# Luolin0826/band

Measured on AMD Instinct MI355X. Metric: multi-DNN inferences/sec + p99 job latency, 4-model int8 mix @1/2/4/8 GPU, higher is better.
Workload: dtype int8

## Files before the change

### band_amd/_abi.py

```python
import ctypes
import os

_HERE = os.path.dirname(os.path.abspath(__file__))
LIB_PATH = os.path.join(_HERE, "libband_hip%s.so" % (
    "_" + os.environ["BAND_HIP_LIB_VARIANT"] if os.environ.get("BAND_HIP_LIB_VARIANT") else ""))

c_int, c_int32, c_void_p, c_size_t = ctypes.c_int, ctypes.c_int32, ctypes.c_void_p, ctypes.c_size_t


class ConvParams(ctypes.Structure):
    _fields_ = [(n, c_int) for n in (
        "batch", "in_h", "in_w", "in_c", "out_h", "out_w", "out_c", "k_h", "k_w",
        "stride_h", "stride_w", "dil_h", "dil_w", "pad_h", "pad_w", "k_pad", "n_pad", "in_xor")] + [
        (n, c_int32) for n in ("in_zp", "w_zp", "out_zp", "act_min", "act_max")] + [
        (n, c_void_p) for n in ("input", "output", "weights", "bias_eff", "mult", "shift", "residual")] + [
        (n, c_int32) for n in ("add_y_off", "add_r_off", "add_o_off", "add_left_shift", "add_y_mult",
                               "add_y_shift", "add_r_mult", "add_r_shift", "add_o_mult", "add_o_shift",
                               "add_act_min", "add_act_max")] + [("out_table", c_void_p), ("requant_fast", c_int32),
                                                                  ("kernel_hint", c_int32),
                                                                  ("out_img_stride", ctypes.c_int64)]


class ConvGroupedParams(ctypes.Structure):
    _fields_ = [("conv", ConvParams), ("groups", c_int32)]


class ConvGroup(ctypes.Structure):
    _fields_ = [("n", c_int), ("blocks", c_int), ("is1x1", c_int), ("table", c_void_p)]


class DwConvParams(ctypes.Structure):
    _fields_ = [(n, c_int) for n in (
        "batch", "in_h", "in_w", "in_c", "out_h", "out_w", "out_c", "depth_multiplier",
        "k_h", "k_w", "stride_h", "stride_w", "dil_h", "dil_w", "pad_h", "pad_w", "in_xor")] + [
        (n, c_int32) for n in ("in_zp", "w_zp", "out_zp", "act_min", "act_max")] + [
        (n, c_void_p) for n in ("input", "output", "weights", "bias", "mult", "shift", "out_table", "taps")] + [
        ("requant_fast", c_int32), ("kernel_hint", c_int32)]


class FcParams(ctypes.Structure):
    _fields_ = [(n, c_int) for n in ("rows", "depth", "depth_pad", "units", "in_xor")] + [
        (n, c_int32) for n in ("in_zp", "w_zp", "out_zp", "act_min", "act_max")] + [
        (n, c_void_p) for n in ("input", "output", "weights", "bias_eff", "mult", "shift", "out_table")]


class EltwiseParams(ctypes.Structure):
    _fields_ = [("kind", c_int), ("in_signed", c_int), ("shape_a", c_int * 4),
                ("shape_b", c_int * 4), ("shape_o", c_int * 4)] + [
        (n, c_int32) for n in ("a_off", "b_off", "o_off", "left_shift", "a_mult", "a_shift",
                               "b_mult", "b_shift", "o_mult", "o_shift", "act_min", "act_max")] + [
        (n, c_void_p) for n in ("a", "b", "out")]


class PoolParams(ctypes.Structure):
    _fields_ = [(n, c_int) for n in (
        "kind", "in_signed", "batch", "in_h", "in_w", "channels", "out_h", "out_w",
        "f_h", "f_w", "stride_h", "stride_w", "pad_h", "pad_w")] + [
        (n, c_int32) for n in ("act_min", "act_max")] + [
        (n, c_void_p) for n in ("input", "output")]


class IrbParams(ctypes.Structure):
    _fields_ = [(n, c_int) for n in (
        "batch", "in_h", "in_w", "in_c", "exp_c", "out_h", "out_w", "out_c", "stride", "pad_h", "pad_w",
        "has_expand", "tile_h", "tile_w")] + [
        ("exp_w", c_void_p), ("exp_k_pad", c_int), ("exp_bias_eff", c_void_p), ("exp_mult", c_void_p),
        ("exp_shift", c_void_p)] + [(n, c_int32) for n in ("x_zp", "e_zp", "e_act_min", "e_act_max")] + [
        ("dw_w", c_void_p), ("dw_bias", c_void_p), ("dw_mult", c_void_p), ("dw_shift", c_void_p)] + [
        (n, c_int32) for n in ("d_zp", "d_act_min", "d_act_max")] + [
        ("proj_w", c_void_p), ("proj_k_pad", c_int), ("proj_bias_eff", c_void_p), ("proj_mult", c_void_p),
        ("proj_shift", c_void_p)] + [(n, c_int32) for n in ("p_zp", "p_act_min", "p_act_max")] + [
        ("has_residual", c_int)] + [(n, c_int32) for n in (
            "add_p_off", "add_x_off", "add_o_off", "add_left_shift", "add_p_mult", "add_p_shift", "add_x_mult",
            "add_x_shift", "add_o_mult", "add_o_shift", "add_act_min", "add_act_max")] + [
        ("input", c_void_p), ("output", c_void_p), ("debug_stamps", c_void_p), ("requant_fast", c_int32)]


class MeanParams(ctypes.Structure):
    _fields_ = [(n, ctypes.c_long) for n in ("outer", "reduce", "inner")] + [("type", c_int)] + [
        (n, c_int32) for n in ("multiplier", "shift", "bias")] + [("input", c_void_p), ("output", c_void_p)]


class MeanRowsParams(ctypes.Structure):
    _fields_ = [("rows", ctypes.c_long), ("depth", c_int), ("type", c_int), ("exact", c_int),
                ("scale", ctypes.c_float), ("bias", ctypes.c_float), ("out_zp", c_int32),
                ("input", c_void_p), ("output", c_void_p)]


class LayerNormParams(ctypes.Structure):
    _fields_ = [("rows", ctypes.c_long), ("depth", c_int), ("mean_x", MeanRowsParams), ("mean_d", MeanRowsParams)] + [
        (n, EltwiseParams) for n in ("sqdiff", "add_eps", "mul_gamma", "mul_x", "mul_m", "sub_beta", "add_out")] + [
        ("eps_q", c_int32)] + [(n, c_void_p) for n in ("rsqrt_table", "input", "gamma", "beta", "output")]


class DetectionParams(ctypes.Structure):
    _fields_ = [(n, c_int) for n in ("batch", "num_boxes", "num_classes", "num_classes_with_background",
                                     "max_detections")] + [
        (n, ctypes.c_float) for n in ("score_threshold", "iou_threshold", "scale_y", "scale_x", "scale_h",
                                      "scale_w")] + [
        ("box_type", c_int), ("score_type", c_int), ("box_scale", ctypes.c_float), ("score_scale", ctypes.c_float),
        ("box_zp", c_int32), ("score_zp", c_int32)] + [
        (n, c_void_p) for n in ("box_encodings", "class_scores", "anchors", "out_boxes", "out_classes",
                                "out_scores", "out_num", "scratch")]


class ChainParams(ctypes.Structure):
    _fields_ = [("dw", DwConvParams), ("pw1", ConvParams), ("pw2", ConvParams), ("has_pw2", c_int),
                ("px_blocks", c_int), ("waves", c_int), ("persist", c_int), ("tile", c_int),
                ("tile_blob", c_void_p), ("debug_stamps", c_void_p), ("deep", c_int), ("c_split", c_int),
                ("stage", c_int), ("dense", c_int)]


CONCAT_MAX_INPUTS = 16


class ConcatParams(ctypes.Structure):
    _fields_ = [("n_inputs", c_int), ("outer", ctypes.c_long),
                ("row", ctypes.c_long * CONCAT_MAX_INPUTS), ("input", c_void_p * CONCAT_MAX_INPUTS),
                ("table", c_void_p * CONCAT_MAX_INPUTS), ("output", c_void_p)]

# ... 55 lines not shown
class SoftmaxParams(ctypes.Structure):
    _fields_ = [("rows", ctypes.c_long), ("depth", c_int), ("is_signed", c_int), ("table", c_void_p),
                ("out_scale", ctypes.c_float), ("out_zp", c_int32), ("input", c_void_p), ("output", c_void_p)]


class ZeroInsertParams(ctypes.Structure):
    _fields_ = [(n, c_int) for n in ("batch", "in_h", "in_w", "channels", "stride_h", "stride_w", "out_h",
                                     "out_w")] + [("fill", ctypes.c_uint32), ("input", c_void_p), ("output", c_void_p)]


class ConvF32Params(ctypes.Structure):
    _fields_ = [(n, c_int) for n in (
        "batch", "in_h", "in_w", "in_c", "out_h", "out_w", "out_c", "k_h", "k_w", "stride_h", "stride_w",
        "dil_h", "dil_w", "pad_h", "pad_w", "depthwise", "depth_multiplier")] + [
        ("act_min", ctypes.c_float), ("act_max", ctypes.c_float)] + [
        (n, c_void_p) for n in ("input", "output", "weights", "bias")]


class FcF32Params(ctypes.Structure):
    _fields_ = [(n, c_int) for n in ("rows", "depth", "units")] + [
        ("act_min", ctypes.c_float), ("act_max", ctypes.c_float)] + [
        (n, c_void_p) for n in ("input", "output", "weights", "bias")]


class EltwiseF32Params(ctypes.Structure):
    _fields_ = [("kind", c_int), ("shape_a", c_int * 4), ("shape_b", c_int * 4), ("shape_o", c_int * 4),
                ("act_min", ctypes.c_float), ("act_max", ctypes.c_float)] + [(n, c_void_p) for n in ("a", "b", "out")]


class PoolF32Params(ctypes.Structure):
    _fields_ = [(n, c_int) for n in (
        "kind", "batch", "in_h", "in_w", "channels", "out_h", "out_w", "f_h", "f_w", "stride_h", "stride_w",
        "pad_h", "pad_w")] + [("act_min", ctypes.c_float), ("act_max", ctypes.c_float)] + [
        (n, c_void_p) for n in ("input", "output")]


KERNEL_SYMBOLS = {
    "bh_device_count": (c_int, [ctypes.POINTER(c_int)]),
    "bh_set_device": (c_int, [c_int]),
    "bh_get_device": (c_int, [ctypes.POINTER(c_int)]),
    "bh_device_arch": (c_int, [c_int, ctypes.c_char_p, c_size_t]),
    "bh_device_pci_bus_id": (c_int, [c_int, ctypes.c_char_p, c_int]),
    "bh_stream_create": (c_int, [ctypes.POINTER(c_void_p)]),
    "bh_stream_destroy": (c_int, [c_void_p]),
    "bh_stream_sync": (c_int, [c_void_p]),
    "bh_stream_query": (c_int, [c_void_p]),
    "bh_malloc": (c_int, [ctypes.POINTER(c_void_p), c_size_t]),
    "bh_free": (c_int, [c_void_p]),
    "bh_host_alloc": (c_int, [ctypes.POINTER(c_void_p), c_size_t]),
    "bh_host_free": (c_int, [c_void_p]),
    "bh_memcpy_h2d_async": (c_int, [c_void_p, c_void_p, c_size_t, c_void_p]),
    "bh_memcpy_d2h_async": (c_int, [c_void_p, c_void_p, c_size_t, c_void_p]),
    "bh_memcpy_d2d_async": (c_int, [c_void_p, c_void_p, c_size_t, c_void_p]),
    "bh_copy_d2d": (c_int, [c_void_p, c_void_p, c_size_t, c_void_p]),
    "bh_memset_async": (c_int, [c_void_p, c_int, c_size_t, c_void_p]),
    "bh_memcpy_h2d": (c_int, [c_void_p, c_void_p, c_size_t]),
    "bh_memcpy_d2h": (c_int, [c_void_p, c_void_p, c_size_t]),
    "bh_capture_begin": (c_int, [c_void_p]),
    "bh_capture_end": (c_int, [c_void_p, ctypes.POINTER(c_void_p)]),
    "bh_graph_launch": (c_int, [c_void_p, c_void_p]),
    "bh_graph_destroy": (c_int, [c_void_p]),
    "bh_event_create": (c_int, [ctypes.POINTER(c_void_p)]),
    "bh_event_create_blocking": (c_int, [ctypes.POINTER(c_void_p)]),
    "bh_capture_end_keep": (c_int, [c_void_p, ctypes.POINTER(c_void_p), ctypes.POINTER(c_void_p)]),
    "bh_graph_free": (c_int, [c_void_p]),
    "bh_graph_memcpy_nodes": (c_int, [c_void_p, ctypes.POINTER(c_void_p), ctypes.POINTER(c_void_p),
                                      ctypes.POINTER(c_void_p), ctypes.POINTER(c_size_t), c_int,
                                      ctypes.POINTER(c_int)]),
    "bh_graph_exec_set_memcpy": (c_int, [c_void_p, c_void_p, c_void_p, c_void_p, c_size_t, c_int]),
    "bh_event_destroy": (c_int, [c_void_p]),
    "bh_event_record": (c_int, [c_void_p, c_void_p]),
    "bh_event_sync": (c_int, [c_void_p]),
    "bh_event_query": (c_int, [c_void_p]),
    "bh_event_create_untimed": (c_int, [ctypes.POINTER(c_void_p)]),
    "bh_event_elapsed_ms": (c_int, [c_void_p, c_void_p, ctypes.POINTER(ctypes.c_float)]),
    "bh_spin_us": (c_int, [c_void_p, c_int]),
    "bh_empty_launch": (c_int, [c_void_p]),
    "bh_profile_events": (c_int, [c_void_p, c_void_p]),
    "bh_pack_conv_weights": (c_int, [c_void_p, c_int, c_int, c_int, c_int, c_int, c_void_p,
                                     c_int32, c_int32, c_void_p, c_void_p]),
    "bh_conv_packed_geometry": (c_int, [c_int, c_int, ctypes.POINTER(c_int), ctypes.POINTER(c_int)]),
    "bh_pack_dw_taps": (c_int, [c_void_p, c_int, c_void_p, c_int32, c_int32, c_void_p]),
    "bh_conv_requant_fast_ok": (c_int, [c_void_p, c_void_p, c_int, c_int, ctypes.c_int64]),
    "bh_conv2d_i8": (c_int, [ctypes.POINTER(ConvParams), c_void_p]),
    "bh_conv_group_ok": (c_int, [ctypes.POINTER(ConvParams)]),
    "bh_conv_group_table_bytes": (ctypes.c_size_t, [c_int]),
    "bh_conv_group_plan": (c_int, [ctypes.POINTER(ConvParams), c_int, c_void_p, ctypes.POINTER(ConvGroup)]),
    "bh_conv_group_i8": (c_int, [ctypes.POINTER(ConvGroup), c_void_p]),
    "bh_conv2d_i8_kernel": (ctypes.c_char_p, [ctypes.POINTER(ConvParams)]),
    "bh_conv2d_grouped_i8": (c_int, [ctypes.POINTER(ConvGroupedParams), c_void_p]),
    "bh_conv2d_grouped_i8_kernel": (ctypes.c_char_p, [ctypes.POINTER(ConvGroupedParams)]),
    "bh_conv_gemm_big_config": (ctypes.c_int, [ctypes.c_long, ctypes.c_int]),
    "bh_dwconv2d_i8_kernel": (ctypes.c_char_p, [ctypes.POINTER(DwConvParams)]),
    "bh_lut_u8": (c_int, [c_void_p, c_void_p, ctypes.c_long, c_void_p, c_void_p]),
    "bh_lut_f32": (c_int, [c_void_p, c_void_p, ctypes.c_long, c_void_p, c_void_p]),
    "bh_quantize_f32": (c_int, [c_void_p, c_void_p, ctypes.c_long, ctypes.c_float, c_int32, c_int, c_void_p]),
    "bh_concat": (c_int, [ctypes.POINTER(ConcatParams), c_void_p]),
    "bh_pad": (c_int, [ctypes.POINTER(PadParams), c_void_p]),
    "bh_resize_nearest": (c_int, [ctypes.POINTER(ResizeNearestParams), c_void_p]),
    "bh_resize_bilinear_i8": (c_int, [ctypes.POINTER(ResizeBilinearParams), c_void_p]),
    "bh_resize_bilinear_u8": (c_int, [ctypes.POINTER(ResizeBilinearU8Params), c_void_p]),
    "bh_argminmax": (c_int, [ctypes.POINTER(ArgMinMaxParams), c_void_p]),
    "bh_argminmax_kernel": (ctypes.c_char_p, [ctypes.POINTER(ArgMinMaxParams)]),
    "bh_resize_bilinear_argminmax_i8": (c_int, [ctypes.POINTER(ResizeArgMinMaxParams), c_void_p]),
    "bh_resize_bilinear_argminmax_i8_ok": (c_int, [ctypes.POINTER(ResizeArgMinMaxParams)]),
    "bh_reindex": (c_int, [ctypes.POINTER(ReindexParams), c_void_p]),
    "bh_reindex_as": (c_int, [ctypes.POINTER(ReindexParams), c_int, c_void_p]),
    "bh_reindex_kernel": (ctypes.c_char_p, [ctypes.POINTER(ReindexParams)]),
    "bh_reindex_canonical": (c_int, [ctypes.POINTER(ReindexParams), ctypes.POINTER(ReindexParams)]),
    "bh_batch_matmul_i8": (c_int, [ctypes.POINTER(BatchMatMulParams), c_void_p]),
    "bh_batch_matmul_i8_kernel": (ctypes.c_char_p, [ctypes.POINTER(BatchMatMulParams)]),
    "bh_batch_matmul_f32": (c_int, [ctypes.POINTER(BatchMatMulParams), c_void_p]),
    "bh_batch_matmul_check": (c_int, [ctypes.POINTER(BatchMatMulParams), c_int]),
    "bh_softmax_i8": (c_int, [ctypes.POINTER(SoftmaxParams), c_void_p]),
    "bh_zero_insert": (c_int, [ctypes.POINTER(ZeroInsertParams), c_void_p]),
    "bh_conv2d_f32": (c_int, [ctypes.POINTER(ConvF32Params), c_void_p]),
    "bh_conv2d_f32_split": (c_int, [ctypes.POINTER(ConvF32Params)]),
    "bh_fc_f32": (c_int, [ctypes.POINTER(FcF32Params), c_void_p]),
    "bh_eltwise_f32": (c_int, [ctypes.POINTER(EltwiseF32Params), c_void_p]),
    "bh_pool_f32": (c_int, [ctypes.POINTER(PoolF32Params), c_void_p]),
    "bh_unary_f32": (c_int, [c_int, c_void_p, c_void_p, ctypes.c_long, ctypes.c_float, ctypes.c_float, c_void_p]),
    "bh_softmax_f32": (c_int, [c_void_p, c_void_p, ctypes.c_long, c_int, ctypes.c_float, c_void_p]),
    "bh_dwconv2d_i8": (c_int, [ctypes.POINTER(DwConvParams), c_void_p]),
    "bh_fc_i8": (c_int, [ctypes.POINTER(FcParams), c_void_p]),
    "bh_eltwise_i8": (c_int, [ctypes.POINTER(EltwiseParams), c_void_p]),
    "bh_pool_i8": (c_int, [ctypes.POINTER(PoolParams), c_void_p]),
    "bh_irb_i8": (c_int, [ctypes.POINTER(IrbParams), c_void_p]),
    "bh_irb_lds_bytes": (c_size_t, [ctypes.POINTER(IrbParams)]),
    "bh_chain_i8": (c_int, [ctypes.POINTER(ChainParams), c_void_p]),
    "bh_mean": (c_int, [ctypes.POINTER(MeanParams), c_void_p]),
    "bh_mean_rows": (c_int, [ctypes.POINTER(MeanRowsParams), c_void_p]),
    "bh_mean_rows_kernel": (ctypes.c_char_p, [ctypes.POINTER(MeanRowsParams)]),
    "bh_mean_rows_check": (c_int, [ctypes.POINTER(MeanRowsParams)]),
    "bh_layernorm_i8": (c_int, [ctypes.POINTER(LayerNormParams), c_void_p]),
    "bh_layernorm_i8_kernel": (ctypes.c_char_p, [ctypes.POINTER(LayerNormParams)]),
    "bh_layernorm_i8_check": (c_int, [ctypes.POINTER(LayerNormParams)]),
    "bh_detection_scratch_bytes": (c_size_t, [c_int, c_int]),
    "bh_detection_postprocess": (c_int, [ctypes.POINTER(DetectionParams), c_void_p]),
    "bh_chain_lds_bytes": (c_size_t, [ctypes.POINTER(ChainParams)]),
    "bh_chain_tile_lds_bytes": (c_size_t, [ctypes.POINTER(ChainParams)]),
    "bh_chain_tile_launch": (c_int, [ctypes.POINTER(ChainParams), c_void_p]),
    "bh_chain_tile_blob_bytes": (c_size_t, [ctypes.POINTER(ChainParams)]),
    "bh_chain_tile_pack": (c_int, [ctypes.POINTER(ChainParams), c_void_p, c_void_p]),
    "bh_chain_stage_lds_bytes": (c_size_t, [ctypes.POINTER(ChainParams)]),
    "bh_chain_stage_launch": (c_int, [ctypes.POINTER(ChainParams), c_void_p]),
    "bh_chain_dense_lds_bytes": (c_size_t, [ctypes.POINTER(ChainParams)]),
    "bh_chain_dense_launch": (c_int, [ctypes.POINTER(ChainParams), c_void_p]),
    "bh_last_error": (ctypes.c_char_p, []),
}

BACKEND_SYMBOLS = {}

_lib = None
_configured = set()


class BandHipError(RuntimeError):
    pass


def load():
    global _lib
    if _lib is None:
        if not os.path.exists(LIB_PATH):
            raise BandHipError(
                "libband_hip.so not built (%s); run __graft_entry__.build() / make -C band_amd/csrc" % LIB_PATH)
# ... 17 lines not shown
```

### band_amd/csrc/backend/hip/lower.cc

```cpp
#include "backend/hip/executor_internal.h"

namespace band {
namespace hip {

using namespace ex;

namespace {

struct ConvQuant {
  std::vector<int32_t> mult, shift;
  int32_t amin, amax, in_zp, w_zp;
  const int32_t* bias;
};

ConvQuant QuantOf(const TflModel& d, const ConvGeometry& g, const TflTensor& out) {
  const TflTensor& in = d.tensors[g.input];
  const TflTensor& w = d.tensors[g.filter];
  const bool i8 = in.type == DataType::kInt8;
  ConvQuant q;
  ConvMultipliers(Scale(in), w.scale, g.out_c, Scale(out), !i8, &q.mult, &q.shift);
  ActivationRangeQuantized(g.act, Scale(out), Zp(out), i8, &q.amin, &q.amax);
  q.in_zp = Dom(in);
  q.w_zp = i8 ? 0 : Dom(w);
  q.bias = g.bias >= 0 ? reinterpret_cast<const int32_t*>(d.tensors[g.bias].data) : nullptr;
// ... 14 lines not shown
  f.in_xor = c.in_xor; f.in_zp = c.in_zp; f.w_zp = c.w_zp; f.out_zp = c.out_zp;
  f.act_min = c.act_min; f.act_max = c.act_max; f.input = c.input; f.output = c.output;
  f.weights = c.weights; f.bias_eff = c.bias_eff; f.mult = c.mult; f.shift = c.shift;
  F.kernel = "fc_kernel";
  F.alg_bytes = L->alg_bytes;
  F.alg_ops = L->alg_ops;
  *L = F;
  return true;
}

template <class Params>
void SetGeometry(const ConvGeometry& g, Params* p) {
  p->batch = g.batch; p->in_h = g.in_h; p->in_w = g.in_w; p->in_c = g.in_c;
  p->out_h = g.out_h; p->out_w = g.out_w; p->out_c = g.out_c; p->k_h = g.k_h; p->k_w = g.k_w;
  p->stride_h = g.stride_h; p->stride_w = g.stride_w; p->dil_h = g.dil_h; p->dil_w = g.dil_w;
  p->pad_h = g.pad_h; p->pad_w = g.pad_w;
}
template <class Params>
void SetGeometry(const PoolGeometry& g, Params* p) {
  p->batch = g.batch; p->in_h = g.in_h; p->in_w = g.in_w; p->channels = g.channels;
  p->out_h = g.out_h; p->out_w = g.out_w; p->f_h = g.f_h; p->f_w = g.f_w;
  p->stride_h = g.stride_h; p->stride_w = g.stride_w; p->pad_h = g.pad_h; p->pad_w = g.pad_w;
}

absl::Status Refused(const TflOperator& op, const char* why) {
  return absl::InternalError(std::string("unsupported ") + TflBuiltinName(op.builtin) + ": " + why);
}

}

absl::Status HipModelExecutor::ConstBlob(const std::string& key, size_t bytes, PreparedSubgraph* sg,
                                         const std::function<absl::Status(uint8_t*)>& fill,
                                         std::shared_ptr<DeviceBlob>* out) {
  auto blob = DeviceRegistry::Get().FindConst(ordinal_, key);
  if (!blob) {
    std::vector<uint8_t> host(bytes, 0);
    RETURN_STATUS_IF(fill(host.data()));
    blob = std::make_shared<DeviceBlob>(ordinal_, bytes);
    if (!blob->ok() || !blob->Upload(0, host.data(), bytes)) return HipErr(1, ("upload constant " + key).c_str());
    DeviceRegistry::Get().PutConst(ordinal_, key, blob);
  }
  sg->consts.push_back(blob);
  *out = blob;
  return absl::OkStatus();
}

absl::Status HipModelExecutor::UploadConst(const std::string& key, const void* data, size_t bytes,
                                           PreparedSubgraph* sg, const void** dev) {
  std::shared_ptr<DeviceBlob> blob;
  RETURN_STATUS_IF(ConstBlob(key, bytes, sg, [&](uint8_t* host) {
    if (bytes) std::memcpy(host, data, bytes);
    return absl::OkStatus();
  }, &blob));
  *dev = blob->ptr();
  return absl::OkStatus();
}

absl::Status HipModelExecutor::DevicePtr(const HipModel& model, int t, PreparedSubgraph* sg, void** ptr) {
  const TflTensor& tt = model.desc().tensors[t];
  if (!tt.is_const()) {
    auto it = sg->offset.find(t);
    if (it == sg->offset.end()) return absl::InternalError("tensor without arena slot");
    *ptr = static_cast<char*>(sg->arena->ptr()) + it->second;
    return absl::OkStatus();
  }
  const void* dev = nullptr;
  RETURN_STATUS_IF(UploadConst("m" + Hex(model.serial()) + "/t" + std::to_string(t), tt.data, tt.data_size, sg, &dev));
  *ptr = const_cast<void*>(dev);
  return absl::OkStatus();
}

absl::Status HipModelExecutor::PackedConv(const HipModel& model, int oi, const ConvGeometry& g, bool flip,
                                          const void* in_ptr, void* out_ptr, const std::string& ckey,
                                          PreparedSubgraph* sg, Launch* L) {
  const TflModel& d = model.desc();
  const TflTensor& w = d.tensors[g.filter];
  const TflTensor& out = d.tensors[d.ops[oi].outputs[0]];
  const bool i8 = w.type == DataType::kInt8;
  const ConvQuant q = QuantOf(d, g, out);
  const int oc = g.out_c, kh = g.k_h, kw = g.k_w, icg = g.in_c / g.groups, K = kh * kw * icg;
  int kp = 0, np = 0;
  bh_conv_packed_geometry(oc, K, &kp, &np);
  const size_t wbytes = static_cast<size_t>(kp) * np;
  std::shared_ptr<DeviceBlob> blob;
  RETURN_STATUS_IF(ConstBlob(ckey, wbytes + 12ull * oc, sg, [&](uint8_t* host) {
    std::vector<uint8_t> flipped(flip ? static_cast<size_t>(oc) * K : 0);
    for (size_t i = 0; i < flipped.size(); ++i) {
      const size_t ci = i % icg, fx = i / icg % kw, fy = i / icg / kw % kh, co = i / K;
      flipped[i] = w.data[((co * kh + (kh - 1 - fy)) * kw + (kw - 1 - fx)) * icg + ci];
    }
    int32_t* tables = reinterpret_cast<int32_t*>(host + wbytes);
    if (bh_pack_conv_weights(flip ? flipped.data() : w.data, i8 ? 1 : 0, oc, K, kp, np, q.bias, q.in_zp, q.w_zp,
                             reinterpret_cast<int8_t*>(host), tables) != 0)
      return absl::InternalError("weight packing failed");
    std::copy(q.mult.begin(), q.mult.end(), tables + oc);
    std::copy(q.shift.begin(), q.shift.end(), tables + 2 * oc);
    return absl::OkStatus();
  }, &blob));
  const int32_t* tab = reinterpret_cast<const int32_t*>(static_cast<char*>(blob->ptr()) + wbytes);
  bh_conv_params& p = L->conv;
  p = bh_conv_params{};
  SetGeometry(g, &p);
  p.k_pad = kp; p.n_pad = np; p.in_xor = i8 ? 0 : 0x80;
  p.in_zp = q.in_zp; p.w_zp = q.w_zp; p.out_zp = Zp(out); p.act_min = q.amin; p.act_max = q.amax;
  p.input = in_ptr; p.output = out_ptr;
  p.weights = static_cast<const int8_t*>(blob->ptr());
  p.bias_eff = tab; p.mult = tab + oc; p.shift = tab + 2 * oc;
  p.requant_fast = bh_conv_requant_fast_ok(q.mult.data(), q.shift.data(), oc, K, MaxAbs(q.bias, oc));
  const double M = static_cast<double>(g.batch) * g.out_h * g.out_w;
  L->alg_ops = 2.0 * M * oc * K;
  L->alg_bytes = static_cast<double>(g.batch) * g.in_h * g.in_w * g.in_c + M * oc + static_cast<double>(oc) * K +
                 12.0 * oc;
  if (g.groups == 1) {
    L->kind = Launch::kConv;
    L->kernel = bh_conv2d_i8_kernel(&p);
    if (GemvAsFc(L)) return absl::OkStatus();
  } else {
    L->kind = Launch::kConvGrouped;
    L->conv_groups = g.groups;
    const bh_conv_grouped_params gp{p, g.groups};
    L->kernel = device_flag_ == DeviceFlag::kCPU ? "conv_grouped_host" : bh_conv2d_grouped_i8_kernel(&gp);
  }
  TryFuseResidualAdd(model, oi, sg, L);
  return absl::OkStatus();
}

absl::Status HipModelExecutor::LowerConv(const HipModel& model, int oi, void* in_ptr, void* out_ptr,
                                         const std::string& ckey, PreparedSubgraph* sg, Launch* L) {
  ConvGeometry g;
  const char* why = "";
  if (!ConvArgs(model.desc(), model.desc().ops[oi], &g, &why)) return Refused(model.desc().ops[oi], why);
  return PackedConv(model, oi, g, false, in_ptr, out_ptr, ckey, sg, L);
}

absl::Status HipModelExecutor::LowerTransposeConv(const HipModel& model, int oi, void* out_ptr,
                                                  const std::string& ckey, PreparedSubgraph* sg, Launch* L) {
  const TflModel& d = model.desc();
  ConvGeometry g;
  const char* why = "";
  if (!ConvArgs(d, d.ops[oi], &g, &why)) return Refused(d.ops[oi], why);
  const TflTensor& x = d.tensors[g.input];
  void* x_ptr = nullptr;
  RETURN_STATUS_IF(DevicePtr(model, g.input, sg, &x_ptr));
  const int uh = (g.in_h - 1) * g.stride_h + 1, uw = (g.in_w - 1) * g.stride_w + 1;
  const size_t ubytes = static_cast<size_t>(g.batch) * uh * uw * g.in_c;
  auto scratch = std::make_shared<DeviceBlob>(ordinal_, ubytes);
  if (!scratch->ok()) return absl::InternalError("HBM scratch allocation failed");
  sg->consts.push_back(scratch);
  Launch Z;
  Z.kind = Launch::kZeroInsert;
  Z.op_index = oi;
  Z.kernel = "zero_insert_kernel";
  Z.zi = bh_zero_insert_params{};
  Z.zi.batch = g.batch; Z.zi.in_h = g.in_h; Z.zi.in_w = g.in_w; Z.zi.channels = g.in_c;
  Z.zi.stride_h = g.stride_h; Z.zi.stride_w = g.stride_w; Z.zi.out_h = uh; Z.zi.out_w = uw;
  Z.zi.fill = static_cast<uint32_t>(Zp(x)) & 0xffu;
  Z.zi.input = x_ptr;
  Z.zi.output = scratch->ptr();
  Z.alg_bytes = static_cast<double>(x.num_elements()) + static_cast<double>(ubytes);
  sg->launches.push_back(Z);
  ConvGeometry u = g;
  u.in_h = uh; u.in_w = uw;
  u.stride_h = u.stride_w = 1;
  u.pad_h = g.k_h - 1 - g.pad_h; u.pad_w = g.k_w - 1 - g.pad_w;
  return PackedConv(model, oi, u, true, scratch->ptr(), out_ptr, ckey, sg, L);
}

absl::Status HipModelExecutor::LowerGlue(const HipModel& model, int oi, void* in_ptr, void* out_ptr,
                                         const std::string& ckey, PreparedSubgraph* sg, Launch* L) {
  const TflModel& d = model.desc();
  const TflOperator& op = d.ops[oi];
  auto T = [&](int i) -> const TflTensor& { return d.tensors[i]; };
  const TflTensor& in = T(op.inputs[0]);
  const TflTensor& out = T(op.outputs[0]);
  const bool i8 = in.type == DataType::kInt8;
  const double in_bytes = static_cast<double>(meta_[op.inputs[0]]->bytes);
  const double out_bytes = static_cast<double>(meta_[op.outputs[0]]->bytes);
  L->alg_bytes = in_bytes + out_bytes;
  switch (op.builtin) {
    case kTflQuantize:
    case kTflRelu:
    case kTflRelu6:
    case kTflReluN1To1:
    case kTflLogistic:
    case kTflHardSwish:
    case kTflRsqrt:
    case kTflGelu: {
      L->src = in_ptr;
      L->dst = out_ptr;
      L->count = static_cast<long>(out.num_elements());
      if (op.builtin == kTflQuantize && in.type == DataType::kFloat32) {
// ... 499 lines not shown
  L->alg_bytes = bytes;
  return absl::OkStatus();
}

absl::Status HipModelExecutor::LowerReindex(const HipModel& model, int oi, PreparedSubgraph* sg) {
  const TflModel& d = model.desc();
  const TflOperator& op = d.ops[oi];
  void* in_ptr = nullptr;
  RETURN_STATUS_IF(DevicePtr(model, op.inputs[op.builtin == kTflSplit ? 1 : 0], sg, &in_ptr));
  for (int k = 0; k < static_cast<int>(op.outputs.size()); ++k) {
    Launch L;
    L.op_index = oi;
    L.out_tensor = op.outputs[k];
    const char* why = "";
    if (!ReindexArgs(d, op, k, &L.reindex, &why))
      return absl::InternalError(std::string("unsupported ") + TflBuiltinName(op.builtin) + ": " + why);
    void* out_ptr = nullptr;
    RETURN_STATUS_IF(DevicePtr(model, op.outputs[k], sg, &out_ptr));
    L.reindex.input = in_ptr;
    L.reindex.output = out_ptr;
    bh_reindex_params c;
    if (bh_reindex_canonical(&L.reindex, &c) != 0)
      return absl::InternalError(std::string(TflBuiltinName(op.builtin)) + ": " + bh_last_error());
    const size_t bytes = meta_[op.outputs[k]]->bytes;
    L.alg_bytes = 2.0 * bytes;
    if (c.rank == 1 && c.in_stride[0] == 1 && c.in_offset == 0) {
      L.kind = Launch::kCopy;
      L.kernel = "copy";
      L.src = in_ptr;
      L.dst = out_ptr;
      L.bytes = bytes;
      if (L.src == L.dst) continue;
    } else {
      L.kind = Launch::kReindex;
      L.kernel = device_flag_ == DeviceFlag::kCPU ? "reindex_host" : bh_reindex_kernel(&L.reindex);
    }
    sg->launches.push_back(L);
  }
  return absl::OkStatus();
}

absl::Status HipModelExecutor::LowerBatchMatMul(const HipModel& model, int oi, void* lhs_ptr, void* out_ptr,
                                                PreparedSubgraph* sg, Launch* L) {
  const TflModel& d = model.desc();
  const TflOperator& op = d.ops[oi];
  const char* why = "";
  bh_batch_matmul_params& p = L->bmm;
  if (!BatchMatMulArgs(d, op, &p, &why)) return absl::InternalError(std::string("unsupported BATCH_MATMUL: ") + why);
  void* rhs_ptr = nullptr;
  RETURN_STATUS_IF(DevicePtr(model, op.inputs[1], sg, &rhs_ptr));
  p.lhs = lhs_ptr;
  p.rhs = rhs_ptr;
  p.out = out_ptr;
  const bool f32 = d.tensors[op.inputs[0]].type == DataType::kFloat32;
  if (bh_batch_matmul_check(&p, f32 ? 4 : 1) != 0) return absl::InternalError(std::string("BATCH_MATMUL: ") + bh_last_error());
  const bool cpu = device_flag_ == DeviceFlag::kCPU;
  L->kind = f32 ? Launch::kBatchMatMulF32 : Launch::kBatchMatMul;
  L->kernel = f32 ? (cpu ? "batch_matmul_f32_host" : "bmm_f32_kernel")
                  : (cpu ? "batch_matmul_host" : bh_batch_matmul_i8_kernel(&p));
  L->alg_ops = 2.0 * p.batch[0] * p.batch[1] * p.m * p.n * p.k;
  L->alg_bytes = static_cast<double>(meta_[op.inputs[0]]->bytes + meta_[op.outputs[0]]->bytes) +
                 static_cast<double>(GetDataTypeBytes(d.tensors[op.inputs[1]].type) * d.tensors[op.inputs[1]].num_elements());
  return absl::OkStatus();
}

absl::Status HipModelExecutor::LowerDepthwise(const HipModel& model, int oi, void* in_ptr, void* out_ptr,
                                              const std::string& ckey, PreparedSubgraph* sg, Launch* L) {
  const TflModel& d = model.desc();
  const TflOperator& op = d.ops[oi];
  ConvGeometry g;
  const char* why = "";
  if (!ConvArgs(d, op, &g, &why)) return Refused(op, why);
  const TflTensor& in = d.tensors[g.input];
  const TflTensor& w = d.tensors[g.filter];
  const TflTensor& out = d.tensors[op.outputs[0]];
  const bool i8 = in.type == DataType::kInt8;
  const ConvQuant q = QuantOf(d, g, out);
  const int oc = g.out_c, kh = g.k_h, kw = g.k_w;
  const size_t wbytes = static_cast<size_t>(kh) * kw * oc;
  const size_t wpad = (wbytes + 15) / 16 * 16;
  const size_t tbytes = 12ull * oc;
  const bool dot = kh == 3 && kw == 3 && g.depth_multiplier == 1 && oc % 4 == 0;
  const size_t pbytes = dot ? 16ull * oc : 0;
  std::shared_ptr<DeviceBlob> blob;
  RETURN_STATUS_IF(ConstBlob(ckey, wpad + tbytes + pbytes, sg, [&](uint8_t* host) {
    for (size_t i = 0; i < wbytes; ++i) host[i] = i8 ? w.data[i] : static_cast<uint8_t>(w.data[i] ^ 0x80);
    int32_t* tables = reinterpret_cast<int32_t*>(host + wpad);
    for (int c = 0; c < oc; ++c) tables[c] = q.bias ? q.bias[c] : 0;
    std::copy(q.mult.begin(), q.mult.end(), tables + oc);
    std::copy(q.shift.begin(), q.shift.end(), tables + 2 * oc);
    if (dot && bh_pack_dw_taps(reinterpret_cast<const int8_t*>(host), oc, tables, q.in_zp, q.w_zp, tables + 3 * oc) != 0)
      return absl::InternalError("depthwise tap packing failed");
    return absl::OkStatus();
  }, &blob));
  const int32_t* tab = reinterpret_cast<const int32_t*>(static_cast<char*>(blob->ptr()) + wpad);
  bh_dwconv_params& p = L->dw;
  p = bh_dwconv_params{};
  SetGeometry(g, &p);
  p.depth_multiplier = g.depth_multiplier;
  p.in_xor = i8 ? 0 : 0x80; p.in_zp = q.in_zp; p.w_zp = q.w_zp; p.out_zp = Zp(out);
  p.act_min = q.amin; p.act_max = q.amax; p.input = in_ptr; p.output = out_ptr;
  p.weights = static_cast<const int8_t*>(blob->ptr());
  p.bias = tab; p.mult = tab + oc; p.shift = tab + 2 * oc;
  if (dot && !blob->host()) p.taps = tab + 3 * oc;
  p.requant_fast = bh_conv_requant_fast_ok(q.mult.data(), q.shift.data(), oc, kh * kw, MaxAbs(q.bias, oc));
  L->kind = Launch::kDwConv;
  L->kernel = bh_dwconv2d_i8_kernel(&p);
  const double M = static_cast<double>(g.batch) * g.out_h * g.out_w;
  L->alg_ops = 2.0 * M * oc * kh * kw;
  L->alg_bytes = static_cast<double>(in.num_elements()) + M * oc + static_cast<double>(wbytes) + 12.0 * oc;
  return absl::OkStatus();
}

absl::Status HipModelExecutor::LowerFc(const HipModel& model, int oi, void* in_ptr, void* out_ptr,
                                       const std::string& ckey, PreparedSubgraph* sg, Launch* L) {
  const TflModel& d = model.desc();
  const TflOperator& op = d.ops[oi];
  FcGeometry g;
  const char* why = "";
  if (!FcArgs(d, op, &g, &why)) return Refused(op, why);
  const TflTensor& in = d.tensors[op.inputs[0]];
  const TflTensor& w = d.tensors[g.filter];
  const TflTensor& out = d.tensors[op.outputs[0]];
  const bool i8 = in.type == DataType::kInt8;
  const int32_t* bias = g.bias >= 0 ? reinterpret_cast<const int32_t*>(d.tensors[g.bias].data) : nullptr;
  const int units = g.units, depth = g.depth, rows = g.rows;
  const int depth_pad = (depth + 15) / 16 * 16;
  int32_t mult, shift, amin, amax;
  FullyConnectedMultiplier(Scale(in), Scale(w), Scale(out), &mult, &shift);
  ActivationRangeQuantized(g.act, Scale(out), Zp(out), i8, &amin, &amax);
  const int32_t in_zp = Dom(in), w_zp = Dom(w);
  const size_t wbytes = static_cast<size_t>(units) * depth_pad;
  std::shared_ptr<DeviceBlob> blob;
  RETURN_STATUS_IF(ConstBlob(ckey, wbytes + 12ull * units, sg, [&](uint8_t* host) {
    int8_t* packed = reinterpret_cast<int8_t*>(host);
    int32_t* tables = reinterpret_cast<int32_t*>(host + wbytes);
    for (int u = 0; u < units; ++u) {
      int64_t s = 0;
      for (int k = 0; k < depth; ++k) {
        const uint8_t raw = w.data[static_cast<size_t>(u) * depth + k];
        const int v = i8 ? static_cast<int>(static_cast<int8_t>(raw)) : static_cast<int>(raw) - 128;
        packed[static_cast<size_t>(u) * depth_pad + k] = static_cast<int8_t>(v);
        s += v;
      }
      tables[u] = static_cast<int32_t>((bias ? bias[u] : 0) - static_cast<int64_t>(in_zp) * s +
                                       static_cast<int64_t>(depth) * in_zp * w_zp);
      tables[units + u] = mult;
      tables[2 * units + u] = shift;
    }
    return absl::OkStatus();
  }, &blob));
  const int32_t* tab = reinterpret_cast<const int32_t*>(static_cast<char*>(blob->ptr()) + wbytes);
  bh_fc_params& p = L->fc;
  p = bh_fc_params{};
  p.rows = rows; p.depth = depth; p.depth_pad = depth_pad; p.units = units;
  p.in_xor = i8 ? 0 : 0x80; p.in_zp = in_zp; p.w_zp = w_zp; p.out_zp = Zp(out);
  p.act_min = amin; p.act_max = amax; p.input = in_ptr; p.output = out_ptr;
  p.weights = static_cast<const int8_t*>(blob->ptr());
  p.bias_eff = tab; p.mult = tab + units; p.shift = tab + 2 * units;
  L->kind = Launch::kFc;
  L->kernel = "fc_kernel";
  L->alg_ops = 2.0 * rows * units * depth;
  L->alg_bytes = static_cast<double>(rows) * depth + static_cast<double>(rows) * units +
                 static_cast<double>(units) * depth + 12.0 * units;
  return absl::OkStatus();
}

absl::Status HipModelExecutor::LowerEltwise(const HipModel& model, int oi, void* in_ptr, void* out_ptr,
                                            PreparedSubgraph* sg, Launch* L) {
  const TflModel& d = model.desc();
  const TflOperator& op = d.ops[oi];
  BroadcastShapes s;
  const char* why = "";
  if (!BroadcastArgs(d, op, &s, &why)) return Refused(op, why);
  const TflTensor& in = d.tensors[op.inputs[0]];
  const TflTensor& b = d.tensors[op.inputs[1]];
  const TflTensor& out = d.tensors[op.outputs[0]];
  const bool i8 = in.type == DataType::kInt8;
  void* b_ptr = nullptr;
  RETURN_STATUS_IF(DevicePtr(model, op.inputs[1], sg, &b_ptr));
  bh_eltwise_params& p = L->elt;
  p = bh_eltwise_params{};
  p.in_signed = i8 ? 1 : 0;
  std::copy_n(s.a, 4, p.shape_a); std::copy_n(s.b, 4, p.shape_b); std::copy_n(s.o, 4, p.shape_o);
  p.a_off = -Zp(in); p.b_off = -Zp(b); p.o_off = Zp(out);
  ActivationRangeQuantized(op.options.Int8(0, 0), Scale(out), Zp(out), i8, &p.act_min, &p.act_max);
  if (op.builtin == kTflSquaredDifference) {
    AddParams ap;
// ... 190 lines not shown
```

### band_amd/csrc/kernels/chain_dense.hip

```cpp
#include <algorithm>
#include <climits>

#include "chain_dw.hpp"
#include "common.hpp"

namespace bh {

struct DenseLds {
  int S1, S2, slab, off_pl, off_add;
  size_t bytes;
};

static DenseLds dense_lds(const bh_chain_params& p) {
  DenseLds L;
  L.S1 = p.pw1.k_pad + 32;
  L.S2 = (p.has_pw2 ? p.pw2.k_pad : (p.pw1.out_c + 15) / 16 * 16) + 32;
  const int dl_row = std::max(L.S1, p.has_pw2 ? (p.pw2.out_c + 15) / 16 * 16 : 0);
  L.off_pl = 16 * dl_row;
  L.slab = L.off_pl + 16 * L.S2;
  L.off_add = 4 * L.slab;
  L.bytes = (size_t)L.off_add + (p.pw1.residual ? 512 * sizeof(int) : 0);
  return L;
}

__device__ __forceinline__ void dense_copy_rows(const unsigned char* src, int stride, uint8_t* dst, int N, int rows,
                                                int lane) {
  const bool v16 = (N & 15) == 0;
  const int u = v16 ? N >> 4 : N >> 2;
  const float rcp = 1.0f / (float)u;
  for (int i = lane; i < rows * u; i += 64) {
    const int r = (int)(((float)i + 0.5f) * rcp);
    const int k = i - r * u;
    if (v16) *(v4i*)(dst + (long)r * N + k * 16) = *(const v4i*)(src + r * stride + k * 16);
    else *(uint32_t*)(dst + (long)r * N + k * 4) = *(const uint32_t*)(src + r * stride + k * 4);
  }
}

struct DenseConv {
  __amdgpu_buffer_rsrc_t w, be, mu, sh;
  int wv, cv;
  int tile_w;
};
__device__ __forceinline__ DenseConv dense_conv(const bh_conv_params& c, int r16, int g) {
  DenseConv d;
  d.w = __builtin_amdgcn_make_buffer_rsrc((void*)c.weights, (short)0, c.n_pad * c.k_pad, 0x00020000);
  d.be = __builtin_amdgcn_make_buffer_rsrc((void*)c.bias_eff, (short)0, c.out_c * 4, 0x00020000);
  d.mu = __builtin_amdgcn_make_buffer_rsrc((void*)c.mult, (short)0, c.out_c * 4, 0x00020000);
  d.sh = __builtin_amdgcn_make_buffer_rsrc((void*)c.shift, (short)0, c.out_c * 4, 0x00020000);
  d.wv = r16 * c.k_pad + g * 16;
  d.cv = r16 * 4;
  d.tile_w = 16 * c.k_pad;
  return d;
}
template <int KX>
struct DenseTile {
  v4i w[KX];
  int be, mu, sh;
};
template <int KX>
__device__ __forceinline__ void dense_filter_load(const DenseConv& c, int t, int k0, int KS, v4i (&w)[KX]) {
  typedef unsigned int v4u __attribute__((ext_vector_type(4)));
#pragma unroll
  for (int u = 0; u < KX; ++u) {
    if (k0 + u < KS) {
      const v4u v = __builtin_amdgcn_raw_buffer_load_b128(c.w, c.wv, t * c.tile_w + (k0 + u) * 64, 0);
      w[u] = (v4i){(int)v.x, (int)v.y, (int)v.z, (int)v.w};
    } else {
      w[u] = (v4i){0, 0, 0, 0};
    }
  }
}
template <int KX>
__device__ __forceinline__ void dense_tile_load(const DenseConv& c, int t, int k0, int KS, DenseTile<KX>& d) {
  dense_filter_load<KX>(c, t, k0, KS, d.w);
  d.be = (int)__builtin_amdgcn_raw_buffer_load_b32(c.be, c.cv, t * 64, 0);
  d.mu = (int)__builtin_amdgcn_raw_buffer_load_b32(c.mu, c.cv, t * 64, 0);
  d.sh = (int)__builtin_amdgcn_raw_buffer_load_b32(c.sh, c.cv, t * 64, 0);
}

template <bool FAST, bool INTERIOR>
__device__ __forceinline__ void dense_dw_groups(const bh_dwconv_params& d, const __amdgpu_buffer_rsrc_t rsrc,
                                                const int (&off)[3], const bool (&ok)[3], bool need, int src4, int r16,
                                                int g, unsigned char* dl, int S1) {
  typedef unsigned int v4u __attribute__((ext_vector_type(4)));
  const int zfill = (int)splat_byte(d.in_zp);
  const int dsel = r16 >> 2;
  const int bsh = 8 * (r16 & 3);
  const int tsel1 = g == 0 ? 0 : 1, tbit1 = g == 0 ? 24 : 8 * (g - 1);
  const int tbit2 = g < 2 ? 8 * (2 + g) : bsh;
  const int G = d.out_c >> 4;
  for (int cg = 0; cg < G; ++cg) {
    const int c0 = cg * 16;
    v4u v[3];
#pragma unroll
    for (int s = 0; s < 3; ++s) asm volatile("" : "=v"(v[s].x), "=v"(v[s].y), "=v"(v[s].z), "=v"(v[s].w));
    if (need) {
#pragma unroll
      for (int s = 0; s < 3; ++s) v[s] = __builtin_amdgcn_raw_buffer_load_b128(rsrc, off[s] + c0, 0, 0);
    }
    const int c = c0 + r16;
    const v4i tw = *(const v4i*)(d.taps + 4 * c);
    const int32_t mu = d.mult[c], sh = d.shift[c];
    v4i xf[3];
#pragma unroll
    for (int s = 0; s < 3; ++s) {
      if (INTERIOR) xf[s] = (v4i){(int)v[s].x, (int)v[s].y, (int)v[s].z, (int)v[s].w};
      else xf[s] = (v4i){ok[s] ? (int)v[s].x : zfill, ok[s] ? (int)v[s].y : zfill, ok[s] ? (int)v[s].z : zfill,
                         ok[s] ? (int)v[s].w : zfill};
#pragma unroll
      for (int j = 0; j < 4; ++j) xf[s][j] = __builtin_amdgcn_ds_bpermute(src4, xf[s][j]);
    }
    const uint32_t t0 = (uint32_t)tw.x, t1 = (uint32_t)tw.y, t2 = (uint32_t)tw.z;
    uint32_t wb[3];
    wb[0] = (t0 >> (8 * g)) & 0xffu;
    wb[1] = ((tsel1 ? t1 : t0) >> tbit1) & 0xffu;
    wb[2] = ((g < 2 ? t1 : t2) >> tbit2) & 0xffu;
    v4i acc = (v4i){tw.w, tw.w, tw.w, tw.w};
#pragma unroll
    for (int s = 0; s < 3; ++s) {
      const int w = g < 3 ? (int)(wb[s] << bsh) : 0;
      const v4i wf = (v4i){dsel == 0 ? w : 0, dsel == 1 ? w : 0, dsel == 2 ? w : 0, dsel == 3 ? w : 0};
      acc = __builtin_amdgcn_mfma_i32_16x16x64_i8(xf[s], wf, acc, 0, 0, 0);
    }
    const ChanQ q = chan_q(mu, sh, d.out_zp);
    int32_t o[4];
#pragma unroll
    for (int r = 0; r < 4; ++r) o[r] = requant_out<FAST>(acc[r], q, d.out_zp, d.act_min, d.act_max);
    stage4(dl, S1, 4 * g, c, o);
  }
}

template <bool FAST>
__device__ __forceinline__ void dense_dw(const bh_dwconv_params& d, const ChainDivs& dv, int m, bool mval, int lane,
                                         int r16, int g, unsigned char* dl, int S1) {
  const int C = d.out_c;
  const int mm = mval ? m : 0;
  const int t = dv.out_w.div(mm);
  const int ox = mm - t * d.out_w;
  const int n = dv.out_h.div(t);
  const int oy = t - n * d.out_h;
  const int iy = oy * d.stride_h, ix = ox * d.stride_w, row0 = n * d.in_h;
  const int gx = g * d.dil_w;
  const int dd = (g == 1 || g == 2) && gx % d.stride_w == 0 ? gx / d.stride_w : 0;
  const bool borrow = dd > 0 && r16 + dd < 16 && ox + dd < d.out_w;
  const bool need = g < 3 && !borrow;
  const int src4 = (borrow ? r16 + dd : lane) << 2;
  int off[3];
  bool ok[3];
#pragma unroll
  for (int s = 0; s < 3; ++s) {
    const int y = iy + s * d.dil_h - d.pad_h, x = ix + gx - d.pad_w;
    ok[s] = mval && g < 3 && y >= 0 && y < d.in_h && x >= 0 && x < d.in_w;
    off[s] = ok[s] ? ((row0 + y) * d.in_w + x) * C : 0;
  }
  const __amdgpu_buffer_rsrc_t rsrc =
      __builtin_amdgcn_make_buffer_rsrc((void*)d.input, (short)0, d.batch * d.in_h * d.in_w * C, 0x00020000);
  const bool interior = __builtin_amdgcn_ballot_w64(g < 3 && !(ok[0] && ok[1] && ok[2])) == 0;
  if (interior) dense_dw_groups<FAST, true>(d, rsrc, off, ok, need, src4, r16, g, dl, S1);
  else dense_dw_groups<FAST, false>(d, rsrc, off, ok, need, src4, r16, g, dl, S1);
}

__device__ __forceinline__ void dense_wave_sync() {
  __builtin_amdgcn_fence(__ATOMIC_RELEASE, "wavefront");
  __builtin_amdgcn_wave_barrier();
  __builtin_amdgcn_fence(__ATOMIC_ACQUIRE, "wavefront");
}

template <bool FAST, int KX, int WPE>
__global__ __launch_bounds__(256, WPE) void chain_dense_kernel(bh_chain_params cp, int P, DenseLds L, ChainDivs dv) {
  extern __shared__ __attribute__((aligned(16))) unsigned char smem[];
  const int lane = threadIdx.x & 63;
  const int pb = threadIdx.x >> 6;
  const int r16 = lane & 15;
  const int g = lane >> 4;
  const int mw = xcd_block(blockIdx.x, gridDim.x) * 64 + pb * 16;
  unsigned char* dl = smem + pb * L.slab;
  unsigned char* pl = dl + L.off_pl;
  const int* add_tab = (const int*)(smem + L.off_add);
  if (cp.pw1.residual) {
    const bh_conv_params& a = cp.pw1;
    int* tab = (int*)(smem + L.off_add);
    for (int i = threadIdx.x; i < 512; i += 256) {
      const int q = (i & 255) - 128;
      tab[i] = i < 256 ? requant_lt1((q + a.add_y_off) * (1 << a.add_left_shift), a.add_y_mult, a.add_y_shift)
                       : requant_lt1((q + a.add_r_off) * (1 << a.add_left_shift), a.add_r_mult, a.add_r_shift);
    }
    __syncthreads();
  }
  if (mw >= P) return;
  const int rows = min(16, P - mw);
  const int orow = 4 * g;

  dense_dw<FAST>(cp.dw, dv, mw + r16, mw + r16 < P, lane, r16, g, dl, L.S1);
  dense_wave_sync();

  {
    const bh_conv_params& a = cp.pw1;
    const int N1 = a.out_c;
    const int T1 = (N1 + 15) >> 4;
    const int KS1 = a.k_pad >> 6;
    const unsigned char* xrow = dl + r16 * L.S1 + g * 16;
    const uint8_t* res = (const uint8_t*)a.residual;
    const DenseConv ac = dense_conv(a, r16, g);
    for (int t = 0; t < T1; ++t) {
      DenseTile<2> cur;
      dense_tile_load<2>(ac, t, 0, KS1, cur);
      v4i acc = (v4i){cur.be, cur.be, cur.be, cur.be};
      const int mu = cur.mu, sh = cur.sh;
      for (int k = 0;;) {
        acc = __builtin_amdgcn_mfma_i32_16x16x64_i8(*(const v4i*)(xrow + k * 64), cur.w[0], acc, 0, 0, 0);
        if (k + 1 < KS1)
          acc = __builtin_amdgcn_mfma_i32_16x16x64_i8(*(const v4i*)(xrow + (k + 1) * 64), cur.w[1], acc, 0, 0, 0);
        k += 2;
        if (k >= KS1) break;
        dense_filter_load<2>(ac, t, k, KS1, cur.w);
      }
      const int n = t * 16 + r16;
      if (n < N1) {
        const ChanQ q = chan_q(mu, sh, a.out_zp);
        int32_t v[4];
#pragma unroll
        for (int r = 0; r < 4; ++r) v[r] = requant_out<FAST>(acc[r], q, a.out_zp, a.act_min, a.act_max);
        if (res) {
          int32_t rq[4];
#pragma unroll
          for (int r = 0; r < 4; ++r)
            rq[r] = (int32_t)(int8_t)res[(uint32_t)(min(mw + orow + r, P - 1) * N1 + n)];
#pragma unroll
          for (int r = 0; r < 4; ++r) {
            const int32_t sy = add_tab[v[r] + 128];
            const int32_t sr = add_tab[256 + rq[r] + 128];
            v[r] = clamp_i32(requant_lt1(sy + sr, a.add_o_mult, a.add_o_shift) + a.add_o_off, a.add_act_min,
                             a.add_act_max);
          }
        }
        stage4(pl, L.S2, orow, n, v);
      }
    }
    dense_wave_sync();
    if (a.output) dense_copy_rows(pl, L.S2, (uint8_t*)a.output + (long)mw * N1, N1, rows, lane);
  }
  if (!cp.has_pw2) return;

  {
    const bh_conv_params& b = cp.pw2;
    const int N2 = b.out_c;
    const int T2 = (N2 + 15) >> 4;
    const int KS2 = b.k_pad >> 6;
    v4i x[KX];
#pragma unroll
    for (int k = 0; k < KX; ++k) x[k] = k < KS2 ? *(const v4i*)(pl + r16 * L.S2 + g * 16 + k * 64) : (v4i){0, 0, 0, 0};
    constexpr bool PF = KX <= 2;
    const DenseConv bc = dense_conv(b, r16, g);
    DenseTile<KX> cur, nxt;
    if (PF) dense_tile_load<KX>(bc, 0, 0, KS2, cur);
    for (int t = 0; t < T2; ++t) {
      if (!PF) dense_tile_load<KX>(bc, t, 0, KS2, cur);
      else if (t + 1 < T2) dense_tile_load<KX>(bc, t + 1, 0, KS2, nxt);
      v4i acc = (v4i){cur.be, cur.be, cur.be, cur.be};
#pragma unroll
      for (int k = 0; k < KX; ++k)
        if (k < KS2) acc = __builtin_amdgcn_mfma_i32_16x16x64_i8(x[k], cur.w[k], acc, 0, 0, 0);
      const int n = t * 16 + r16;
      if (n < N2) {
        const ChanQ q = chan_q(cur.mu, cur.sh, b.out_zp);
        int32_t v[4];
#pragma unroll
        for (int r = 0; r < 4; ++r) v[r] = requant_out<FAST>(acc[r], q, b.out_zp, b.act_min, b.act_max);
        stage4(dl, N2, orow, n, v);
      }
      if (PF && t + 1 < T2) cur = nxt;
    }
    dense_wave_sync();
    dense_copy_rows(dl, N2, (uint8_t*)b.output + (long)mw * N2, N2, rows, lane);
  }
}

#ifndef BH_DENSE_WPE
#define BH_DENSE_WPE 8
#endif

template <bool FAST, int KX, int WPE>
static void launch_dense(const bh_chain_params& p, int P, const DenseLds& L, hipStream_t s) {
  ChainDivs dv;
  dv.out_w = FastDiv(p.dw.out_w);
  dv.out_h = FastDiv(p.dw.out_h);
  BH_LAUNCH((chain_dense_kernel<FAST, KX, WPE>), dim3((P + 63) / 64), dim3(256), L.bytes, s, p, P, L, dv);
}

}

extern "C" size_t bh_chain_dense_lds_bytes(const bh_chain_params* pp) {
  const bh_chain_params& p = *pp;
  if (p.dense != 1 || p.px_blocks != 4 || (p.waves != 0 && p.waves != 4)) return 0;
  if (p.tile || p.persist || p.deep || p.stage || p.c_split > 1) return 0;
  if ((long)p.pw1.n_pad * p.pw1.k_pad >= INT32_MAX || (p.has_pw2 && (long)p.pw2.n_pad * p.pw2.k_pad >= INT32_MAX)) return 0;
  const bh::DenseLds L = bh::dense_lds(p);
  return L.bytes <= 64 * 1024 ? L.bytes : 0;
}

extern "C" int bh_chain_dense_launch(const bh_chain_params* pp, bh_stream_t stream) {
  const bh_chain_params& p = *pp;
  const int P = p.dw.batch * p.dw.out_h * p.dw.out_w;
  const bh::DenseLds L = bh::dense_lds(p);
  const bool fast = p.dw.requant_fast && p.pw1.requant_fast && (!p.has_pw2 || p.pw2.requant_fast);
  hipStream_t s = (hipStream_t)stream;
  const int ks2 = p.has_pw2 ? p.pw2.k_pad >> 6 : 1;
  if (ks2 <= 1) {
    if (fast) bh::launch_dense<true, 1, BH_DENSE_WPE>(p, P, L, s);
    else bh::launch_dense<false, 1, BH_DENSE_WPE>(p, P, L, s);
  } else if (ks2 <= 2) {
    if (fast) bh::launch_dense<true, 2, BH_DENSE_WPE>(p, P, L, s);
    else bh::launch_dense<false, 2, BH_DENSE_WPE>(p, P, L, s);
  } else {
    if (fast) bh::launch_dense<true, 5, BH_DENSE_WPE>(p, P, L, s);
    else bh::launch_dense<false, 5, BH_DENSE_WPE>(p, P, L, s);
  }
  return bh_check_launch("chain_dense_kernel");
}
```

### band_amd/csrc/kernels/chain_dw.hpp

```cpp
#pragma once

#include "common.hpp"

namespace bh {

struct ChainDivs {
  FastDiv out_w, out_h;
};

template <bool FAST, int DA, int WPB>
__device__ __forceinline__ void chain_dw_mfma(const bh_dwconv_params& d, const ChainDivs& dv, int m, bool mval,
                                              int lane, int r16, int g, int wsub, unsigned char* dl, int S1,
                                              int orow) {
  typedef unsigned int v4u __attribute__((ext_vector_type(4)));
  const int C = d.out_c;
  const int mm = mval ? m : 0;
  const int t = dv.out_w.div(mm);
  const int ox = mm - t * d.out_w;
  const int n = dv.out_h.div(t);
  const int oy = t - n * d.out_h;
  const int iy = oy * d.stride_h, ix = ox * d.stride_w, row0 = n * d.in_h;
  const int gx = g * d.dil_w;
  const int dd = (g == 1 || g == 2) && gx % d.stride_w == 0 ? gx / d.stride_w : 0;
  const bool borrow = dd > 0 && r16 + dd < 16 && ox + dd < d.out_w;
  const bool need = g < 3 && !borrow;
  const int src4 = (borrow ? r16 + dd : lane) << 2;
  int off[3];
  bool ok[3];
#pragma unroll
  for (int s = 0; s < 3; ++s) {
    const int y = iy + s * d.dil_h - d.pad_h, x = ix + gx - d.pad_w;
    ok[s] = mval && g < 3 && y >= 0 && y < d.in_h && x >= 0 && x < d.in_w;
    off[s] = ok[s] ? ((row0 + y) * d.in_w + x) * C : 0;
  }
  const __amdgpu_buffer_rsrc_t rsrc =
      __builtin_amdgcn_make_buffer_rsrc((void*)d.input, (short)0, d.batch * d.in_h * d.in_w * C, 0x00020000);
  const int zfill = (int)splat_byte(d.in_zp);
  const int dsel = r16 >> 2;
  const int bsh = 8 * (r16 & 3);
  const int tsel1 = g == 0 ? 0 : 1, tbit1 = g == 0 ? 24 : 8 * (g - 1);
  const int tbit2 = g < 2 ? 8 * (2 + g) : bsh;
  struct DwItem {
    v4i xf[3];
    v4i tw;
    int32_t mu, sh;
  };
  auto dw_load = [&](int cg, DwItem& it) {
    const int c0 = cg * 16;
    v4u v[3] = {};
    if (need) {
#pragma unroll
      for (int s = 0; s < 3; ++s) v[s] = __builtin_amdgcn_raw_buffer_load_b128(rsrc, off[s] + c0, 0, 0);
    }
#pragma unroll
    for (int s = 0; s < 3; ++s)
      it.xf[s] = (v4i){ok[s] ? (int)v[s].x : zfill, ok[s] ? (int)v[s].y : zfill, ok[s] ? (int)v[s].z : zfill,
                       ok[s] ? (int)v[s].w : zfill};
    const int c = c0 + r16;
    it.tw = *(const v4i*)(d.taps + 4 * c);
    it.mu = d.mult[c];
    it.sh = d.shift[c];
  };
  auto dw_finish = [&](int cg, DwItem& it) {
#pragma unroll
    for (int s = 0; s < 3; ++s)
#pragma unroll
      for (int j = 0; j < 4; ++j) it.xf[s][j] = __builtin_amdgcn_ds_bpermute(src4, it.xf[s][j]);
    const uint32_t t0 = (uint32_t)it.tw.x, t1 = (uint32_t)it.tw.y, t2 = (uint32_t)it.tw.z;
    uint32_t wb[3];
    wb[0] = (t0 >> (8 * g)) & 0xffu;
    wb[1] = ((tsel1 ? t1 : t0) >> tbit1) & 0xffu;
    wb[2] = ((g < 2 ? t1 : t2) >> tbit2) & 0xffu;
    v4i acc = (v4i){it.tw.w, it.tw.w, it.tw.w, it.tw.w};
#pragma unroll
    for (int s = 0; s < 3; ++s) {
      const int w = g < 3 ? (int)(wb[s] << bsh) : 0;
      const v4i wf = (v4i){dsel == 0 ? w : 0, dsel == 1 ? w : 0, dsel == 2 ? w : 0, dsel == 3 ? w : 0};
      acc = __builtin_amdgcn_mfma_i32_16x16x64_i8(it.xf[s], wf, acc, 0, 0, 0);
    }
    const ChanQ q = chan_q(it.mu, it.sh, d.out_zp);
    int32_t v[4];
#pragma unroll
    for (int r = 0; r < 4; ++r) v[r] = requant_out<FAST>(acc[r], q, d.out_zp, d.act_min, d.act_max);
    stage4(dl, S1, orow, cg * 16 + r16, v);
  };
  const int G = C >> 4;
  for (int cg = wsub; cg < G; cg += DA * WPB) {
    DwItem it[DA];
#pragma unroll
    for (int u = 0; u < DA; ++u) dw_load(cg + u * WPB < G ? cg + u * WPB : cg, it[u]);
#pragma unroll
    for (int u = 0; u < DA; ++u)
      if (u == 0 || cg + u * WPB < G) dw_finish(cg + u * WPB, it[u]);
  }
}

template <bool FAST, int NB, int NW>
__device__ __forceinline__ void chain_dw_mfma_wg(const bh_dwconv_params& d, const ChainDivs& dv, int m0, int P,
                                                 int lane, int r16, int g, int wave, unsigned char* dl, int S1) {
  typedef unsigned int v4u __attribute__((ext_vector_type(4)));
  const int C = d.out_c;
  const int gx = g * d.dil_w;
  const int dd = (g == 1 || g == 2) && gx % d.stride_w == 0 ? gx / d.stride_w : 0;
  int off[NB][3], src4[NB];
  bool ok[NB][3], need[NB];
#pragma unroll
  for (int b = 0; b < NB; ++b) {
    const int m = m0 + 16 * b + r16;
    const bool mval = m < P;
    const int mm = mval ? m : 0;
    const int t = dv.out_w.div(mm);
    const int ox = mm - t * d.out_w;
    const int n = dv.out_h.div(t);
    const int oy = t - n * d.out_h;
    const int iy = oy * d.stride_h, ix = ox * d.stride_w, row0 = n * d.in_h;
    const bool borrow = dd > 0 && r16 + dd < 16 && ox + dd < d.out_w;
    need[b] = g < 3 && !borrow;
    src4[b] = (borrow ? r16 + dd : lane) << 2;
#pragma unroll
    for (int s = 0; s < 3; ++s) {
      const int y = iy + s * d.dil_h - d.pad_h, x = ix + gx - d.pad_w;
      ok[b][s] = mval && g < 3 && y >= 0 && y < d.in_h && x >= 0 && x < d.in_w;
      off[b][s] = ok[b][s] ? ((row0 + y) * d.in_w + x) * C : 0;
    }
  }
  const __amdgpu_buffer_rsrc_t rsrc =
      __builtin_amdgcn_make_buffer_rsrc((void*)d.input, (short)0, d.batch * d.in_h * d.in_w * C, 0x00020000);
  const int zfill = (int)splat_byte(d.in_zp);
  const int dsel = r16 >> 2;
  const int bsh = 8 * (r16 & 3);
  const int tsel1 = g == 0 ? 0 : 1, tbit1 = g == 0 ? 24 : 8 * (g - 1);
  const int tbit2 = g < 2 ? 8 * (2 + g) : bsh;
  const int G = C >> 4;
  for (int cg = wave; cg < G; cg += NW) {
    const int c0 = cg * 16;
    const int c = c0 + r16;
    v4i xf[NB][3];
#pragma unroll
    for (int b = 0; b < NB; ++b) {
      v4u v[3] = {};
      if (need[b]) {
#pragma unroll
        for (int s = 0; s < 3; ++s) v[s] = __builtin_amdgcn_raw_buffer_load_b128(rsrc, off[b][s] + c0, 0, 0);
      }
#pragma unroll
      for (int s = 0; s < 3; ++s)
        xf[b][s] = (v4i){ok[b][s] ? (int)v[s].x : zfill, ok[b][s] ? (int)v[s].y : zfill,
                         ok[b][s] ? (int)v[s].z : zfill, ok[b][s] ? (int)v[s].w : zfill};
    }
    const v4i tw = *(const v4i*)(d.taps + 4 * c);
    const int32_t mu = d.mult[c], sh = d.shift[c];
    const uint32_t t0 = (uint32_t)tw.x, t1 = (uint32_t)tw.y, t2 = (uint32_t)tw.z;
    uint32_t wb[3];
    wb[0] = (t0 >> (8 * g)) & 0xffu;
    wb[1] = ((tsel1 ? t1 : t0) >> tbit1) & 0xffu;
    wb[2] = ((g < 2 ? t1 : t2) >> tbit2) & 0xffu;
    v4i wf[3];
#pragma unroll
    for (int s = 0; s < 3; ++s) {
      const int w = g < 3 ? (int)(wb[s] << bsh) : 0;
      wf[s] = (v4i){dsel == 0 ? w : 0, dsel == 1 ? w : 0, dsel == 2 ? w : 0, dsel == 3 ? w : 0};
    }
    const ChanQ q = chan_q(mu, sh, d.out_zp);
#pragma unroll
    for (int b = 0; b < NB; ++b) {
#pragma unroll
      for (int s = 0; s < 3; ++s)
#pragma unroll
        for (int j = 0; j < 4; ++j) xf[b][s][j] = __builtin_amdgcn_ds_bpermute(src4[b], xf[b][s][j]);
      v4i acc = (v4i){tw.w, tw.w, tw.w, tw.w};
#pragma unroll
      for (int s = 0; s < 3; ++s) acc = __builtin_amdgcn_mfma_i32_16x16x64_i8(xf[b][s], wf[s], acc, 0, 0, 0);
      int32_t v[4];
#pragma unroll
      for (int r = 0; r < 4; ++r) v[r] = requant_out<FAST>(acc[r], q, d.out_zp, d.act_min, d.act_max);
      stage4(dl, S1, 16 * b + 4 * g, c, v);
    }
  }
}

}
```

### band_amd/csrc/kernels/chain_stage.hip

```cpp
#include <algorithm>

#include "chain_blob.hpp"
#include "chain_dw.hpp"
#include "common.hpp"

namespace bh {

struct StageGeom {
  int S1, S2;
  int TS;
  int w1_bytes;
  int blob_w2, blob_b2, blob_m2, blob_s2;
  int off_w2, off_t2, off_dl, off_pl, off_o1, off_res, off_add, off_out;
  int out_pitch;
  size_t bytes;
};

static size_t up16(size_t v) { return (v + 15) / 16 * 16; }

static StageGeom stage_geom(const bh_chain_params& p) {
  StageGeom G{};
  const TileBlob B = tile_blob(p);
  const int rows = p.px_blocks * 16;
  const int N1 = p.pw1.out_c, N2 = p.pw2.out_c;
  const int T2 = (N2 + 15) / 16;
  const int S = std::max(1, p.c_split);
  G.TS = (T2 + S - 1) / S;
  G.S1 = p.pw1.k_pad + 32;
  G.S2 = p.pw2.k_pad + 32;
  G.w1_bytes = B.w2;
  G.blob_w2 = B.w2;
  G.blob_b2 = B.b2;
  G.blob_m2 = B.m2;
  G.blob_s2 = B.s2;
  size_t o = B.w2;
  G.off_w2 = (int)o;
  o += (size_t)G.TS * 16 * p.pw2.k_pad;
  G.off_t2 = (int)o;
  o += 3 * (size_t)G.TS * 64;
  G.off_dl = (int)o;
  o += (size_t)rows * G.S1;
  G.off_pl = (int)o;
  o += (size_t)rows * G.S2;
  G.off_o1 = (int)o;
  o += p.pw1.output ? up16((size_t)rows * N1) : 0;
  G.off_res = (int)o;
  o += p.pw1.residual ? up16((size_t)rows * N1) : 0;
  G.off_add = (int)o;
  o += p.pw1.residual ? 512 * 4 : 0;
  const int cw = G.TS * 16;
  G.out_pitch = cw % 32 == 0 ? cw + 16 : cw;
  if ((size_t)rows * G.out_pitch <= (size_t)rows * G.S1) {
    G.off_out = G.off_dl;
  } else {
    G.off_out = (int)o;
    o += (size_t)rows * G.out_pitch;
  }
  G.bytes = up16(o);
  return G;
}

__device__ __forceinline__ void stage_copy_rows(const unsigned char* src, uint8_t* dst, int bytes, int tid,
                                                int nthreads) {
  const int n16 = bytes >> 4;
  for (int i = tid; i < n16; i += nthreads) *(v4i*)(dst + i * 16) = *(const v4i*)(src + i * 16);
  const int rem = (bytes - (n16 << 4)) >> 2;
  if (tid < rem) *(uint32_t*)(dst + n16 * 16 + tid * 4) = *(const uint32_t*)(src + n16 * 16 + tid * 4);
}

__device__ __forceinline__ void stage_copy_out(const unsigned char* src, int pitch, uint8_t* dst, int Nc, int c0,
                                               int cw, int rows, int tid, int nthreads) {
  const bool v16 = ((c0 | cw | Nc) & 15) == 0;
  const int u = v16 ? cw >> 4 : cw >> 2;
  const float rcp = 1.0f / (float)u;
  for (int i = tid; i < rows * u; i += nthreads) {
    const int r = (int)(((float)i + 0.5f) * rcp);
    const int k = i - r * u;
    if (v16) *(v4i*)(dst + (long)r * Nc + c0 + k * 16) = *(const v4i*)(src + r * pitch + k * 16);
    else *(uint32_t*)(dst + (long)r * Nc + c0 + k * 4) = *(const uint32_t*)(src + r * pitch + k * 4);
  }
}

template <int RB, bool FAST, int KX, int NW, int LW>
__global__ __launch_bounds__(NW * 64) void chain_stage_kernel(bh_chain_params cp, int P, StageGeom G, ChainDivs dv) {
  extern __shared__ __attribute__((aligned(16))) unsigned char smem[];
  constexpr int WPB = NW / RB;
  constexpr int NA = NW - LW;
  constexpr int NL = LW ? LW : NW;
  static_assert(NA % RB == 0, "phase-A waves cover every pixel block");
  const int tid = threadIdx.x;
  const int lane = tid & 63;
  const int wave = tid >> 6;
  const int r16 = lane & 15;
  const int g = lane >> 4;
  const int pb = wave % RB;
  const int wsub = wave / RB;
  const int blk = xcd_block(blockIdx.x, gridDim.x);
  const int m0 = blk * RB * 16;
  const int rows = min(RB * 16, P - m0);
  const int m = m0 + pb * 16 + r16;
  const int orow = pb * 16 + 4 * g;
  const bh_conv_params& a = cp.pw1;
  const bh_conv_params& b = cp.pw2;
  const int N1 = a.out_c, N2 = b.out_c;
  const int T1 = (N1 + 15) >> 4, T2 = (N2 + 15) >> 4;
  const int t_lo = (int)blockIdx.y * T2 / (int)gridDim.y;
  const int t_hi = ((int)blockIdx.y + 1) * T2 / (int)gridDim.y;
  const int nt = t_hi - t_lo;
  unsigned char* dl = smem + G.off_dl;
  unsigned char* pl = smem + G.off_pl;
  unsigned char* o1 = smem + G.off_o1;
  unsigned char* ol = smem + G.off_out;
  const unsigned char* resl = smem + G.off_res;

  if (LW == 0 || wave >= NA) {
    const int lw = LW ? wave - NA : wave;
    const unsigned char* blob = (const unsigned char*)cp.tile_blob;
    auto run16 = [&](const unsigned char* src, unsigned char* dst, int units) {
      for (int base = lw * 64; base < units; base += NL * 64)
        if (base + lane < units) dma16(src + (base + lane) * 16, dst + base * 16);
    };
    run16(blob, smem, G.w1_bytes >> 4);
    run16(blob + G.blob_w2 + (long)t_lo * 16 * b.k_pad, smem + G.off_w2, nt * b.k_pad);
    run16(blob + G.blob_b2 + 64 * t_lo, smem + G.off_t2, 4 * nt);
    run16(blob + G.blob_m2 + 64 * t_lo, smem + G.off_t2 + G.TS * 64, 4 * nt);
    run16(blob + G.blob_s2 + 64 * t_lo, smem + G.off_t2 + 2 * G.TS * 64, 4 * nt);
    if (a.residual) {
      const uint8_t* res = (const uint8_t*)a.residual + (long)m0 * N1;
      const int units = (rows * N1) >> 2;
      for (int base = lw * 64; base < units; base += NL * 64)
        if (base + lane < units) dma4(res + (base + lane) * 4, smem + G.off_res + base * 4);
    }
  }
  int* add_tab = (int*)(smem + G.off_add);
  if (a.residual) {
    for (int i = tid; i < 512; i += NW * 64) {
      const int q = (i & 255) - 128;
      add_tab[i] = i < 256 ? requant_lt1((q + a.add_y_off) * (1 << a.add_left_shift), a.add_y_mult, a.add_y_shift)
                           : requant_lt1((q + a.add_r_off) * (1 << a.add_left_shift), a.add_r_mult, a.add_r_shift);
    }
  }

  if (LW == 0 || wave < NA) chain_dw_mfma<FAST, 2, NA / RB>(cp.dw, dv, m, m < P, lane, r16, g, wsub, dl, G.S1, orow);
  asm volatile("s_waitcnt vmcnt(0)" ::: "memory");
  __syncthreads();

  {
    const int k1 = a.k_pad;
    const int KS1 = k1 >> 6;
    const int sx1 = swz_mask(r16, k1 >> 4);
    const int* b1 = (const int*)(smem + T1 * 16 * k1);
    const int* m1 = b1 + N1;
    const int* s1 = m1 + N1;
    const unsigned char* xrow = dl + (pb * 16 + r16) * G.S1 + g * 16;
    const bool out1 = a.output != nullptr && blockIdx.y == 0;
    auto epi = [&](int nch, v4i acc) {
      if (nch >= N1) return;
      const ChanQ q = chan_q(m1[nch], s1[nch], a.out_zp);
      int32_t v[4];
#pragma unroll
      for (int r = 0; r < 4; ++r) v[r] = requant_out<FAST>(acc[r], q, a.out_zp, a.act_min, a.act_max);
      if (a.residual) {
#pragma unroll
        for (int r = 0; r < 4; ++r) {
          const int32_t rq = (int32_t)(int8_t)resl[(orow + r) * N1 + nch];
          v[r] = clamp_i32(requant_lt1(add_tab[v[r] + 128] + add_tab[256 + rq + 128], a.add_o_mult, a.add_o_shift) +
                               a.add_o_off,
                           a.add_act_min, a.add_act_max);
        }
      }
      if (out1) stage4(o1, N1, orow, nch, v);
      stage4(pl, G.S2, orow, nch, v);
    };
    for (int t = wsub; t < T1; t += 2 * WPB) {
      const bool two = t + WPB < T1;
      const int ra = t * 16 + r16, rb = (two ? t + WPB : t) * 16 + r16;
      const unsigned char* wa = smem + ra * k1;
      const unsigned char* wb = smem + rb * k1;
      const int ba = b1[ra < N1 ? ra : 0], bb = b1[rb < N1 ? rb : 0];
      v4i acca = (v4i){ba, ba, ba, ba}, accb = (v4i){bb, bb, bb, bb};
      for (int k = 0; k < KS1; ++k) {
        const v4i xv = *(const v4i*)(xrow + k * 64);
        const v4i w0 = *(const v4i*)(wa + 16 * ((4 * k + g) ^ sx1));
        const v4i w1 = *(const v4i*)(wb + 16 * ((4 * k + g) ^ sx1));
        acca = __builtin_amdgcn_mfma_i32_16x16x64_i8(xv, w0, acca, 0, 0, 0);
        accb = __builtin_amdgcn_mfma_i32_16x16x64_i8(xv, w1, accb, 0, 0, 0);
      }
      epi(ra, acca);
      if (two) epi(rb, accb);
    }
  }
  __syncthreads();
  if (a.output && blockIdx.y == 0) stage_copy_rows(o1, (uint8_t*)a.output + (long)m0 * N1, rows * N1, tid, NW * 64);

  {
    const int k2 = b.k_pad;
    const int KS2 = k2 >> 6;
    const int sx2 = swz_mask(r16, k2 >> 4);
    const unsigned char* W2 = smem + G.off_w2;
    const int* b2 = (const int*)(smem + G.off_t2);
    const int* m2 = b2 + G.TS * 16;
    const int* s2 = m2 + G.TS * 16;
    const unsigned char* xrow = pl + (pb * 16 + r16) * G.S2 + g * 16;
    v4i x[KX];
#pragma unroll
    for (int k = 0; k < KX; ++k) x[k] = k < KS2 ? *(const v4i*)(xrow + k * 64) : (v4i){0, 0, 0, 0};
    auto epi = [&](int lc, v4i acc) {
      if (t_lo * 16 + lc >= N2) return;
      const ChanQ q = chan_q(m2[lc], s2[lc], b.out_zp);
      int32_t v[4];
#pragma unroll
      for (int r = 0; r < 4; ++r) v[r] = requant_out<FAST>(acc[r], q, b.out_zp, b.act_min, b.act_max);
      stage4(ol, G.out_pitch, orow, lc, v);
    };
    for (int t = wsub; t < nt; t += 2 * WPB) {
      const bool two = t + WPB < nt;
      const int ra = t * 16 + r16, rb = (two ? t + WPB : t) * 16 + r16;
      const unsigned char* wa = W2 + ra * k2;
      const unsigned char* wb = W2 + rb * k2;
      const int ba = t_lo * 16 + ra < N2 ? b2[ra] : 0, bb = t_lo * 16 + rb < N2 ? b2[rb] : 0;
      v4i acca = (v4i){ba, ba, ba, ba}, accb = (v4i){bb, bb, bb, bb};
#pragma unroll
      for (int k = 0; k < KX; ++k)
        if (k < KS2) {
          const v4i w0 = *(const v4i*)(wa + 16 * ((4 * k + g) ^ sx2));
          const v4i w1 = *(const v4i*)(wb + 16 * ((4 * k + g) ^ sx2));
          acca = __builtin_amdgcn_mfma_i32_16x16x64_i8(x[k], w0, acca, 0, 0, 0);
          accb = __builtin_amdgcn_mfma_i32_16x16x64_i8(x[k], w1, accb, 0, 0, 0);
        }
      epi(ra, acca);
      if (two) epi(rb, accb);
    }
  }
  __syncthreads();
  const int c_lo = t_lo * 16, c_hi = min(N2, t_hi * 16);
  if (c_hi > c_lo)
    stage_copy_out(ol, G.out_pitch, (uint8_t*)b.output + (long)m0 * N2, N2, c_lo, c_hi - c_lo, rows, tid, NW * 64);
}

template <int RB, bool FAST, int KX, int NW, int LW>
static void launch_stage(const bh_chain_params& p, int P, const StageGeom& G, hipStream_t s) {
  if (G.bytes > 64 * 1024) {
    static thread_local int opted_device = -1;
    int dev = 0;
    (void)hipGetDevice(&dev);
    if (opted_device != dev) {
      (void)hipFuncSetAttribute((const void*)chain_stage_kernel<RB, FAST, KX, NW, LW>,
                                hipFuncAttributeMaxDynamicSharedMemorySize, 160 * 1024);
      opted_device = dev;
    }
  }
  ChainDivs dv;
  dv.out_w = FastDiv(p.dw.out_w);
  dv.out_h = FastDiv(p.dw.out_h);
  const int blocks = (P + RB * 16 - 1) / (RB * 16);
  BH_LAUNCH((chain_stage_kernel<RB, FAST, KX, NW, LW>), dim3(blocks, std::max(1, p.c_split)), dim3(NW * 64), G.bytes, s,
            p, P, G, dv);
}

template <bool FAST, int KX>
static void launch_stage_form(const bh_chain_params& p, int P, const StageGeom& G, hipStream_t s) {
  const int nw = p.waves == 8 ? 8 : 4;
  if (p.stage == 2) {
    if (p.px_blocks == 2) {
      if (nw == 8) launch_stage<2, FAST, KX, 8, 4>(p, P, G, s);
      else launch_stage<2, FAST, KX, 4, 2>(p, P, G, s);
    } else {
      if (nw == 8) launch_stage<1, FAST, KX, 8, 4>(p, P, G, s);
      else launch_stage<1, FAST, KX, 4, 2>(p, P, G, s);
    }
    return;
  }
  if (p.px_blocks == 2) {
    if (nw == 8) launch_stage<2, FAST, KX, 8, 0>(p, P, G, s);
    else launch_stage<2, FAST, KX, 4, 0>(p, P, G, s);
  } else {
    if (nw == 8) launch_stage<1, FAST, KX, 8, 0>(p, P, G, s);
    else launch_stage<1, FAST, KX, 4, 0>(p, P, G, s);
  }
}

}

extern "C" size_t bh_chain_stage_lds_bytes(const bh_chain_params* pp) {
  const bh_chain_params& p = *pp;
  if (!p.has_pw2 || p.pw2.k_pad > 64 * 5) return 0;
  if (p.px_blocks != 1 && p.px_blocks != 2) return 0;
  if (p.waves != 0 && p.waves != 4 && p.waves != 8) return 0;
  if (p.tile || p.persist || p.deep || p.stage < 0 || p.stage > 2) return 0;
  if (p.c_split < 0 || p.c_split > 8 || (p.pw2.out_c + 15) / 16 < std::max(1, p.c_split)) return 0;
  const bh::StageGeom G = bh::stage_geom(p);
  return G.bytes <= 160 * 1024 ? G.bytes : 0;
}

extern "C" int bh_chain_stage_launch(const bh_chain_params* pp, bh_stream_t stream) {
  const bh_chain_params& p = *pp;
  if (!p.tile_blob) {
    bh_set_last_error("bh_chain_i8: the stage form needs tile_blob (bh_chain_tile_pack)");
    return BH_EINVAL;
  }
  const int P = p.dw.batch * p.dw.out_h * p.dw.out_w;
  const bh::StageGeom G = bh::stage_geom(p);
  const bool fast = p.dw.requant_fast && p.pw1.requant_fast && p.pw2.requant_fast;
  const bool k2 = p.pw2.k_pad <= 128;
  hipStream_t s = (hipStream_t)stream;
  if (k2) {
    if (fast) bh::launch_stage_form<true, 2>(p, P, G, s);
    else bh::launch_stage_form<false, 2>(p, P, G, s);
  } else {
    if (fast) bh::launch_stage_form<true, 5>(p, P, G, s);
    else bh::launch_stage_form<false, 5>(p, P, G, s);
  }
  return bh_check_launch("chain_stage_kernel");
}
```

### band_amd/csrc/kernels/common.hpp

```cpp
#pragma once

#include <hip/hip_ext.h>
#include <hip/hip_runtime.h>
#include <stdint.h>

#include "band_hip_kernels.h"

namespace bh {

struct ProfEvents {
  hipEvent_t start = nullptr;
  hipEvent_t stop = nullptr;
  int launched = 0;
};
extern thread_local ProfEvents g_prof;

#define BH_LAUNCH(kern, grid, block, shmem, stream, ...)                                            \
  do {                                                                                              \
    if (::bh::g_prof.stop) {                                                                        \
      hipExtLaunchKernelGGL(kern, grid, block, shmem, stream, ::bh::g_prof.start, ::bh::g_prof.stop, 0, \
                            __VA_ARGS__);                                                           \
      ::bh::g_prof.start = nullptr;                                                                 \
      ++::bh::g_prof.launched;                                                                      \
    } else {                                                                                        \
// ... 9 lines not shown
__device__ __forceinline__ int32_t srdhm(int32_t a, int32_t b) {
  return (int32_t)(((int64_t)a * (int64_t)b + (1ll << 30)) >> 31);
}

__device__ __forceinline__ int32_t rdbypot(int32_t x, int e) {
  const int32_t mask = (int32_t)((1u << e) - 1u);
  const int32_t rem = x & mask;
  const int32_t thr = (mask >> 1) + (x < 0 ? 1 : 0);
  return (x >> e) + (rem > thr ? 1 : 0);
}

__device__ __forceinline__ int32_t requant(int32_t x, int32_t m, int32_t shift) {
  const int left = shift > 0 ? shift : 0;
  const int right = shift > 0 ? 0 : -shift;
  return rdbypot(srdhm((int32_t)((uint32_t)x << left), m), right);
}

__device__ __forceinline__ int32_t requant_lt1(int32_t x, int32_t m, int32_t left_shift) {
  return rdbypot(srdhm(x, m), -left_shift);
}

__device__ __forceinline__ int32_t clamp_i32(int32_t v, int32_t lo, int32_t hi) {
  return v < lo ? lo : (v > hi ? hi : v);
}

__device__ __forceinline__ int32_t sbyte(uint32_t w, int b) {
  return (int32_t)(int8_t)((w >> (8 * b)) & 0xff);
}

__device__ __forceinline__ uint32_t splat_byte(int32_t v) {
  return ((uint32_t)v & 0xffu) * 0x01010101u;
}

__device__ __forceinline__ uint32_t pack4_bytes(const int32_t v[4]) {
  const uint32_t lo = __builtin_amdgcn_perm((uint32_t)v[1], (uint32_t)v[0], 0x0c0c0400u);
  const uint32_t hi = __builtin_amdgcn_perm((uint32_t)v[3], (uint32_t)v[2], 0x04000c0cu);
  return lo | hi;
}

__device__ __forceinline__ uint32_t quad_transpose8(uint32_t p) {
  const int i = (int)(threadIdx.x & 3);
  const uint32_t x = (uint32_t)__builtin_amdgcn_mov_dpp((int)p, 0x4e, 0xf, 0xf, false);
  const uint32_t n = __builtin_amdgcn_perm(x, p, (i & 2) ? 0x03020706u : 0x05040100u);
  const uint32_t y = (uint32_t)__builtin_amdgcn_mov_dpp((int)n, 0xb1, 0xf, 0xf, false);
  return __builtin_amdgcn_perm(y, n, (i & 1) ? 0x03070105u : 0x06020400u);
}

__device__ __forceinline__ void stage4(unsigned char* tile, int stride, int row0, int col, const int32_t v[4]) {
  const int r16 = col & 15;
  *(uint32_t*)(tile + (row0 + (r16 & 3)) * stride + col - r16 + (r16 & ~3)) = quad_transpose8(pack4_bytes(v));
}

struct FastDiv {
  uint32_t d = 1, m = 0, s = 0;
  FastDiv() = default;
  __host__ __device__ explicit FastDiv(uint32_t div) : d(div ? div : 1) {
    if (d > 1) {
      uint32_t l = 0;
      while ((1u << l) < d) ++l;
      const uint64_t p = 31 + l;
      m = (uint32_t)(((1ull << p) + d - 1) / d);
      s = (uint32_t)(p - 32);
    }
  }
  __device__ __forceinline__ uint32_t div(uint32_t n) const { return d == 1 ? n : (__umulhi(n, m) >> s); }
  __device__ __forceinline__ uint32_t mod(uint32_t n) const { return n - div(n) * d; }
};

struct ChanQ {
  int32_t mu, sh;
  int32_t e, emask, zpe;
  int64_t c0;
};

__device__ __forceinline__ ChanQ chan_q(int32_t mu, int32_t sh, int32_t zp) {
  ChanQ q;
  q.mu = mu;
  q.sh = sh;
  q.e = -sh;
  q.emask = q.e > 0 ? -1 : 0;
  q.zpe = (int32_t)((uint32_t)zp << (q.e & 31));
  q.c0 = (1ll << 30) + (q.e > 0 ? (1ll << (30 + q.e)) : 0ll);
  return q;
}

__device__ __forceinline__ int32_t med3_clamp(int32_t v, int32_t lo, int32_t hi) {
  int32_t r;
  asm("v_med3_i32 %0, %1, %2, %3" : "=v"(r) : "v"(v), "s"(lo), "v"(hi));
  return r;
}

template <bool FAST>
__device__ __forceinline__ int32_t requant_out(int32_t acc, const ChanQ& q, int32_t zp, int32_t lo, int32_t hi) {
  int32_t v;
  if constexpr (FAST) {
    const int64_t z = (int64_t)acc * q.mu + q.c0;
    const int32_t u = (int32_t)(z >> 31);
    v = (u + ((acc >> 31) & q.emask) + q.zpe) >> q.e;
  } else {
    v = requant(acc, q.mu, q.sh) + zp;
  }
  return med3_clamp(v, lo, hi);
}

__device__ __forceinline__ int32_t requant_clamp(int32_t acc, int32_t mu, int32_t sh, int32_t zp, int32_t lo,
                                                 int32_t hi, bool fast) {
  return fast ? requant_out<true>(acc, chan_q(mu, sh, zp), zp, lo, hi) : clamp_i32(requant(acc, mu, sh) + zp, lo, hi);
}

template <typename T>
using cst_ptr = const T __attribute__((address_space(4)))*;
template <typename T>
__device__ __forceinline__ cst_ptr<T> as_const(const T* p) {
  return (cst_ptr<T>)(uintptr_t)p;
}

__device__ __forceinline__ int xcd_block(int hw, int total) {
  const int per = total >> 3;
  return hw < (per << 3) ? (hw & 7) * per + (hw >> 3) : hw;
}

struct XcdSplit {
  int xb, sub_m, sub_n;
};
__device__ __forceinline__ void xcd_tile(int hw, int total, const XcdSplit& x, int gm, int gn, int& bm, int& bn) {
  if (x.xb == 0) {
    const int l = xcd_block(hw, total);
    bm = l / gn;
    bn = l - bm * gn;
    return;
  }
  const int a = 8 / x.xb;
  const int xcd = hw & 7, j = hw >> 3;
  const int pa = xcd / x.xb, pb = xcd - pa * x.xb;
  const int m_lo = pa * gm / a, sm = (pa + 1) * gm / a - m_lo;
  const int n_lo = pb * gn / x.xb, sn = (pb + 1) * gn / x.xb - n_lo;
  if (j >= sm * sn) {
    bm = gm;
    bn = 0;
    return;
  }
  const int jm = j / sn;
  bm = m_lo + jm;
  bn = n_lo + (j - jm * sn);
}
inline XcdSplit xcd_split(long in_bytes, long w_bytes, int gm, int gn) {
  XcdSplit best{0, gm, gn};
  long cost = -1;
  const long blocks = (long)gm * gn;
  for (int xb = 1; xb <= 8; xb *= 2) {
    const int a = 8 / xb;
    if (xb > gn || a > gm) continue;
    const int sub_m = (gm + a - 1) / a, sub_n = (gn + xb - 1) / xb;
    if (8L * sub_m * sub_n * 8 > blocks * 9) continue;
    const long c = xb * in_bytes + a * w_bytes;
    if (cost < 0 || c < cost) {
      cost = c;
      best = {xb, sub_m, sub_n};
    }
  }
  return best;
}
inline int xcd_grid(const XcdSplit& x) { return x.xb ? 8 * x.sub_m * x.sub_n : x.sub_m * x.sub_n; }

}

// ... 3 lines not shown
```

### band_amd/csrc/kernels/fused_chain.hip

```cpp
#include <algorithm>

#include "chain_dw.hpp"
#include "common.hpp"

namespace bh {

__device__ __forceinline__ uint32_t pack4(const int32_t v[4]) {
  const uint32_t lo = __builtin_amdgcn_perm((uint32_t)v[1], (uint32_t)v[0], 0x0c0c0400u);
  const uint32_t hi = __builtin_amdgcn_perm((uint32_t)v[3], (uint32_t)v[2], 0x04000c0cu);
  return lo | hi;
}

__device__ __forceinline__ v4i gemm_tile(const bh_conv_params& c, const unsigned char* xrow, int t, int KS, int r16,
                                         int g) {
  const int8_t* wrow = c.weights + (long)(t * 16 + r16) * c.k_pad + g * 16;
  const int nb = t * 16 + 4 * g;
  const int nl = nb < c.out_c ? nb : 0;
  v4i acc = *(const v4i*)(c.bias_eff + nl);
  int k = 0;
  for (; k + 8 <= KS; k += 8) {
    v4i w[8], x[8];
#pragma unroll
    for (int u = 0; u < 8; ++u) {
      w[u] = *(const v4i*)(wrow + (k + u) * 64);
// ... 18 lines not shown
    acc = __builtin_amdgcn_mfma_i32_16x16x64_i8(w, x, acc, 0, 0, 0);
  }
  return acc;
}

template <bool FAST>
__device__ __forceinline__ void requant4(const bh_conv_params& c, int nb, v4i acc, int32_t v[4]) {
  const v4i vm = *(const v4i*)(c.mult + nb);
  const v4i vs = *(const v4i*)(c.shift + nb);
#pragma unroll
  for (int r = 0; r < 4; ++r)
    v[r] = requant_out<FAST>(acc[r], chan_q(vm[r], vs[r], c.out_zp), c.out_zp, c.act_min, c.act_max);
}

template <int KMAX, typename Epi>
__device__ __forceinline__ void gemm_xs(const bh_conv_params& c, const unsigned char* xrow, int KS, int t0, int tstep,
                                        int r16, int g, Epi&& epi) {
  v4i x[KMAX];
#pragma unroll
  for (int k = 0; k < KMAX; ++k) x[k] = k < KS ? *(const v4i*)(xrow + k * 64) : (v4i){0, 0, 0, 0};
  const int T = (c.out_c + 15) >> 4;
  for (int t = t0; t < T; t += 2 * tstep) {
    const int tb = t + tstep < T ? t + tstep : t;
    const int8_t* ra = c.weights + (long)(t * 16 + r16) * c.k_pad + g * 16;
    const int8_t* rb = c.weights + (long)(tb * 16 + r16) * c.k_pad + g * 16;
    v4i wa[KMAX], wb[KMAX];
#pragma unroll
    for (int k = 0; k < KMAX; ++k)
      if (k < KS) {
        wa[k] = *(const v4i*)(ra + k * 64);
        wb[k] = *(const v4i*)(rb + k * 64);
      }
    const int na = t * 16 + 4 * g, nb = tb * 16 + 4 * g;
    const int la = na < c.out_c ? na : 0, lb = nb < c.out_c ? nb : 0;
    v4i acca = *(const v4i*)(c.bias_eff + la);
    v4i accb = *(const v4i*)(c.bias_eff + lb);
    const v4i ma = *(const v4i*)(c.mult + la), sa = *(const v4i*)(c.shift + la);
    const v4i mb = *(const v4i*)(c.mult + lb), sb = *(const v4i*)(c.shift + lb);
#pragma unroll
    for (int k = 0; k < KMAX; ++k)
      if (k < KS) {
        acca = __builtin_amdgcn_mfma_i32_16x16x64_i8(wa[k], x[k], acca, 0, 0, 0);
        accb = __builtin_amdgcn_mfma_i32_16x16x64_i8(wb[k], x[k], accb, 0, 0, 0);
      }
    epi(t, na, acca, ma, sa);
    if (tb != t) epi(tb, nb, accb, mb, sb);
  }
}

template <bool FAST>
__device__ __forceinline__ void requant4m(const bh_conv_params& c, v4i acc, v4i vm, v4i vs, int32_t v[4]) {
#pragma unroll
  for (int r = 0; r < 4; ++r)
    v[r] = requant_out<FAST>(acc[r], chan_q(vm[r], vs[r], c.out_zp), c.out_zp, c.act_min, c.act_max);
}

constexpr int kXsMax = 5;

__device__ __forceinline__ void copy_out(const unsigned char* src, uint8_t* dst, int bytes) {
  const int n16 = bytes >> 4;
  for (int i = threadIdx.x; i < n16; i += blockDim.x) *(v4i*)(dst + i * 16) = *(const v4i*)(src + i * 16);
  const int rem = (bytes - (n16 << 4)) >> 2;
  if ((int)threadIdx.x < rem)
    *(uint32_t*)(dst + n16 * 16 + threadIdx.x * 4) = *(const uint32_t*)(src + n16 * 16 + threadIdx.x * 4);
}

__device__ __forceinline__ void copy_out_slice(const unsigned char* src, uint8_t* dst, int Nc, int c0, int cw,
                                               int rows) {
  const bool v16 = ((c0 | cw | Nc) & 15) == 0;
  const int u = v16 ? cw >> 4 : cw >> 2;
  const float rcp = 1.0f / (float)u;
  for (int i = threadIdx.x; i < rows * u; i += blockDim.x) {
    const int r = (int)(((float)i + 0.5f) * rcp);
    const int k = i - r * u;
    const long o = (long)r * Nc + c0;
    if (v16) *(v4i*)(dst + o + k * 16) = *(const v4i*)(src + o + k * 16);
    else *(uint32_t*)(dst + o + k * 4) = *(const uint32_t*)(src + o + k * 4);
  }
}

template <int KB>
struct TileHead {
  v4i w[KB];
  int be, mu, sh;
};
template <int KB>
__device__ __forceinline__ void tile_head_load(const bh_conv_params& c, int t, int KS, int r16, int g,
                                               TileHead<KB>& h) {
  const int8_t* wrow = c.weights + (long)(t * 16 + r16) * c.k_pad + g * 16;
#pragma unroll
  for (int u = 0; u < KB; ++u)
    if (u < KS) h.w[u] = *(const v4i*)(wrow + u * 64);
  const int n = t * 16 + r16;
  const int nl = n < c.out_c ? n : 0;
  h.be = c.bias_eff[nl];
  h.mu = c.mult[nl];
  h.sh = c.shift[nl];
}
template <int KB = 4>
__device__ __forceinline__ v4i gemm_tile_nt(const bh_conv_params& c, const unsigned char* xrow, int t, int KS,
                                            int r16, int g, const TileHead<KB>& h) {
  const int8_t* wrow = c.weights + (long)(t * 16 + r16) * c.k_pad + g * 16;
  v4i acc = (v4i){h.be, h.be, h.be, h.be};
  {
    v4i x[KB];
#pragma unroll
    for (int u = 0; u < KB; ++u)
      if (u < KS) x[u] = *(const v4i*)(xrow + u * 64);
#pragma unroll
    for (int u = 0; u < KB; ++u)
      if (u < KS) acc = __builtin_amdgcn_mfma_i32_16x16x64_i8(x[u], h.w[u], acc, 0, 0, 0);
  }
  for (int k = KB; k < KS; k += KB) {
    v4i w[KB], x[KB];
#pragma unroll
    for (int u = 0; u < KB; ++u)
      if (k + u < KS) {
        w[u] = *(const v4i*)(wrow + (k + u) * 64);
        x[u] = *(const v4i*)(xrow + (k + u) * 64);
      }
#pragma unroll
    for (int u = 0; u < KB; ++u)
      if (k + u < KS) acc = __builtin_amdgcn_mfma_i32_16x16x64_i8(x[u], w[u], acc, 0, 0, 0);
  }
  return acc;
}

template <int KMAX, int TT>
struct XsRound {
  int tt[TT], be[TT], mu[TT], sh[TT];
  v4i w[TT][KMAX];
};
template <int KMAX, int TT>
__device__ __forceinline__ void xs_round_load(const bh_conv_params& c, int KS, int t, int tstep, int T, int r16,
                                              int g, XsRound<KMAX, TT>& rd) {
#pragma unroll
  for (int u = 0; u < TT; ++u) {
    rd.tt[u] = t + u * tstep < T ? t + u * tstep : t;
    const int8_t* r = c.weights + (long)(rd.tt[u] * 16 + r16) * c.k_pad + g * 16;
#pragma unroll
    for (int k = 0; k < KMAX; ++k)
      if (k < KS) rd.w[u][k] = *(const v4i*)(r + k * 64);
    const int n = rd.tt[u] * 16 + r16;
    const int l = n < c.out_c ? n : 0;
    rd.be[u] = c.bias_eff[l];
    rd.mu[u] = c.mult[l];
    rd.sh[u] = c.shift[l];
  }
}
template <int KMAX, int TT, typename Epi>
__device__ __forceinline__ void gemm_xs_nt_from(const bh_conv_params& c, const unsigned char* xrow, int KS, int t0,
                                                int tstep, int T, int r16, int g, XsRound<KMAX, TT>& rd, Epi&& epi) {
  v4i x[KMAX];
#pragma unroll
  for (int k = 0; k < KMAX; ++k) x[k] = k < KS ? *(const v4i*)(xrow + k * 64) : (v4i){0, 0, 0, 0};
  for (int t = t0; t < T; t += TT * tstep) {
    if (t != t0) xs_round_load<KMAX, TT>(c, KS, t, tstep, T, r16, g, rd);
    v4i acc[TT];
#pragma unroll
    for (int u = 0; u < TT; ++u) acc[u] = (v4i){rd.be[u], rd.be[u], rd.be[u], rd.be[u]};
#pragma unroll
    for (int k = 0; k < KMAX; ++k)
      if (k < KS) {
#pragma unroll
        for (int u = 0; u < TT; ++u)
          acc[u] = __builtin_amdgcn_mfma_i32_16x16x64_i8(x[k], rd.w[u][k], acc[u], 0, 0, 0);
      }
#pragma unroll
    for (int u = 0; u < TT; ++u)
      if (u == 0 || rd.tt[u] != t) epi(rd.tt[u], rd.tt[u] * 16 + r16, acc[u], rd.mu[u], rd.sh[u]);
  }
}
template <int KMAX, int TT = 2, typename Epi>
__device__ __forceinline__ void gemm_xs_nt(const bh_conv_params& c, const unsigned char* xrow, int KS, int t0,
                                           int tstep, int r16, int g, Epi&& epi) {
  const int T = (c.out_c + 15) >> 4;
  XsRound<KMAX, TT> rd;
  if (t0 < T) xs_round_load<KMAX, TT>(c, KS, t0, tstep, T, r16, g, rd);
  gemm_xs_nt_from<KMAX, TT>(c, xrow, KS, t0, tstep, T, r16, g, rd, epi);
}

template <int KMAX, typename Epi>
__device__ __forceinline__ void gemm_xs4_nt(const bh_conv_params& c, const unsigned char* base, int stride, int KS,
                                            int wave, int r16, int g, Epi&& epi, int t_begin = 0, int t_end = -1) {
  v4i x[4][KMAX];
#pragma unroll
  for (int pb = 0; pb < 4; ++pb)
#pragma unroll
    for (int k = 0; k < KMAX; ++k)
      x[pb][k] = k < KS ? *(const v4i*)(base + (pb * 16 + r16) * stride + g * 16 + k * 64) : (v4i){0, 0, 0, 0};
  const int T = t_end >= 0 ? t_end : (c.out_c + 15) >> 4;
  for (int t = t_begin + wave; t < T; t += 4) {
    const int n = t * 16 + r16;
    const int nl = n < c.out_c ? n : 0;
    const int8_t* wrow = c.weights + (long)(t * 16 + r16) * c.k_pad + g * 16;
    v4i w[KMAX];
#pragma unroll
    for (int k = 0; k < KMAX; ++k)
      if (k < KS) w[k] = *(const v4i*)(wrow + k * 64);
    const int be = c.bias_eff[nl], mu = c.mult[nl], sh = c.shift[nl];
    v4i acc[4];
#pragma unroll
    for (int pb = 0; pb < 4; ++pb) acc[pb] = (v4i){be, be, be, be};
#pragma unroll
    for (int k = 0; k < KMAX; ++k)
      if (k < KS) {
#pragma unroll
        for (int pb = 0; pb < 4; ++pb) acc[pb] = __builtin_amdgcn_mfma_i32_16x16x64_i8(x[pb][k], w[k], acc[pb], 0, 0, 0);
      }
    epi(n, acc, mu, sh);
  }
}

template <int RB, bool FAST, int KX, int NW, bool AM, int DA = 2, int VAR = 0>
__global__ __launch_bounds__(NW * 64) void chain_kernel(bh_chain_params cp, int P, int S1, int S2, int off_pl, int off_o1,
                                                       int off_add, ChainDivs dv) {
  extern __shared__ __attribute__((aligned(16))) unsigned char smem[];
  const unsigned long long t_entry = __builtin_amdgcn_s_memtime();
  constexpr int WPB = NW / RB;
  constexpr int TTC = DA > 2 ? (KX <= 2 ? 6 : 3) : 2;
  const int lane = threadIdx.x & 63;
  const int wave = threadIdx.x >> 6;
  const int r16 = lane & 15;
  const int g = lane >> 4;
  const int pb = wave % RB;
  const int wsub = wave / RB;
  const int blk = xcd_block(blockIdx.x, gridDim.x);
  const int m0 = blk * RB * 16;
  const int rows = min(RB * 16, P - m0);
  const int m = m0 + pb * 16 + r16;
  unsigned char* dl = smem;
  unsigned char* pl = smem + off_pl;
  unsigned char* o1 = smem + off_o1;
  int* add_tab = (int*)(smem + off_add);
  if (cp.pw1.residual) {
    const bh_conv_params& a = cp.pw1;
    for (int i = threadIdx.x; i < 512; i += NW * 64) {
      const int q = (i & 255) - 128;
      add_tab[i] = i < 256 ? requant_lt1((q + a.add_y_off) * (1 << a.add_left_shift), a.add_y_mult, a.add_y_shift)
                           : requant_lt1((q + a.add_r_off) * (1 << a.add_left_shift), a.add_r_mult, a.add_r_shift);
    }
  }
  const int prow = pb * 16 + r16;
  const int orow = pb * 16 + 4 * g;
  unsigned long long* stamps =
      cp.debug_stamps ? (unsigned long long*)cp.debug_stamps + 8 * (long)blockIdx.x : nullptr;
#define CHAIN_STAMP(k) \
  if (stamps && threadIdx.x == 0) stamps[k] = __builtin_amdgcn_s_memtime();
  CHAIN_STAMP(0)
  if (stamps && threadIdx.x == 0) stamps[7] = t_entry;

  constexpr bool SPLIT = (VAR & 2) != 0;
  constexpr bool PFC = RB == 1 && DA == 2;
  constexpr bool PFB = PFC && NW == 16;
  constexpr int KBB = DA > 2 ? 8 : 4;
  TileHead<KBB> b_head;
  if constexpr (PFB) {
    const int KS1 = cp.pw1.k_pad >> 6;
    if (KS1 > KX && wsub < (cp.pw1.out_c + 15) >> 4) tile_head_load<KBB>(cp.pw1, wsub, KS1, r16, g, b_head);
  }

  if constexpr (RB == 2 && DA == 2) {
    chain_dw_mfma_wg<FAST, RB, NW>(cp.dw, dv, m0, P, lane, r16, g, wave, dl, S1);
  } else {
    chain_dw_mfma<FAST, DA, WPB>(cp.dw, dv, m, m < P, lane, r16, g, wsub, dl, S1, orow);
  }
  __syncthreads();
  CHAIN_STAMP(1)

  {
    const bh_conv_params& a = cp.pw1;
    const int N1 = a.out_c;
    const int T1 = (N1 + 15) >> 4;
    const int KS1 = a.k_pad >> 6;
    const unsigned char* xrow = dl + prow * S1 + g * 16;
    const uint8_t* res = (const uint8_t*)a.residual;
    const bool out1 = a.output != nullptr && (!SPLIT || blockIdx.y == 0);
    auto epi = [&](int t, int n, v4i acc, int mu, int sh) {
      if (n >= N1) return;
      const ChanQ q = chan_q(mu, sh, a.out_zp);
      int32_t v[4];
#pragma unroll
      for (int r = 0; r < 4; ++r) v[r] = requant_out<FAST>(acc[r], q, a.out_zp, a.act_min, a.act_max);
      if (res) {
        int32_t rq[4];
#pragma unroll
        for (int r = 0; r < 4; ++r) {
          const int mr = m0 + orow + r;
          rq[r] = mr < P ? (int32_t)(int8_t)res[(long)mr * N1 + n] : 0;
        }
#pragma unroll
        for (int r = 0; r < 4; ++r) {
          const int32_t sy = add_tab[v[r] + 128];
          const int32_t sr = add_tab[256 + rq[r] + 128];
          v[r] = clamp_i32(requant_lt1(sy + sr, a.add_o_mult, a.add_o_shift) + a.add_o_off, a.add_act_min,
                           a.add_act_max);
        }
      }
      if (out1) stage4(o1, N1, orow, n, v);
      if (cp.has_pw2) stage4(pl, S2, orow, n, v);
    };
    if (AM && KS1 <= KX) {
      gemm_xs4_nt<KX>(a, dl, S1, KS1, wave, r16, g, [&](int n, const v4i* acc, int mu, int sh) {
        if (n >= N1) return;
        const ChanQ q = chan_q(mu, sh, a.out_zp);
#pragma unroll
        for (int pb4 = 0; pb4 < 4; ++pb4) {
          const int rb = pb4 * 16 + 4 * g;
          int32_t v[4];
#pragma unroll
          for (int r = 0; r < 4; ++r) v[r] = requant_out<FAST>(acc[pb4][r], q, a.out_zp, a.act_min, a.act_max);
          if (res) {
#pragma unroll
            for (int r = 0; r < 4; ++r) {
              const int mr = m0 + rb + r;
              const int32_t rq = mr < P ? (int32_t)(int8_t)res[(long)mr * N1 + n] : 0;
              v[r] = clamp_i32(requant_lt1(add_tab[v[r] + 128] + add_tab[256 + rq + 128], a.add_o_mult, a.add_o_shift) +
                                   a.add_o_off,
                               a.add_act_min, a.add_act_max);
            }
          }
          if (out1) stage4(o1, N1, rb, n, v);
          if (cp.has_pw2) stage4(pl, S2, rb, n, v);
        }
      });
    } else if (KS1 <= KX) {
      gemm_xs_nt<KX, TTC>(a, xrow, KS1, wsub, WPB, r16, g, epi);
    } else {
      for (int t = wsub; t < T1; t += WPB) {
        if (!PFB || t != wsub) tile_head_load<KBB>(a, t, KS1, r16, g, b_head);
        const v4i acc = gemm_tile_nt<KBB>(a, xrow, t, KS1, r16, g, b_head);
        epi(t, t * 16 + r16, acc, b_head.mu, b_head.sh);
      }
    }
  }
  struct CTiles {
    int lo, hi;
  };
  auto c_tiles = [&]() {
    const int T2 = (cp.pw2.out_c + 15) >> 4;
    if constexpr (SPLIT)
      return CTiles{(int)blockIdx.y * T2 / (int)gridDim.y, ((int)blockIdx.y + 1) * T2 / (int)gridDim.y};
    else
      return CTiles{0, T2};
  };
  XsRound<KX, TTC> c_first;
  if constexpr (PFC) {
    if (cp.has_pw2) {
      const CTiles ct = c_tiles();
      if (ct.lo + wsub < ct.hi)
        xs_round_load<KX, TTC>(cp.pw2, cp.pw2.k_pad >> 6, ct.lo + wsub, WPB, ct.hi, r16, g, c_first);
    }
  }
  __syncthreads();
  CHAIN_STAMP(2)
  if (cp.pw1.output && (!SPLIT || blockIdx.y == 0))
    copy_out(o1, (uint8_t*)cp.pw1.output + (long)m0 * cp.pw1.out_c, rows * cp.pw1.out_c);
  CHAIN_STAMP(3)
  if (!cp.has_pw2) return;

  {
    const bh_conv_params& b = cp.pw2;
    const int N2 = b.out_c;
    const int KS2 = b.k_pad >> 6;
    const CTiles ct = c_tiles();
    const unsigned char* xrow = pl + prow * S2 + g * 16;
    auto epi4 = [&](int n, const v4i* acc, int mu, int sh) {
      if (n >= N2) return;
      const ChanQ q = chan_q(mu, sh, b.out_zp);
#pragma unroll
      for (int pb4 = 0; pb4 < 4; ++pb4) {
        int32_t v[4];
#pragma unroll
        for (int r = 0; r < 4; ++r) v[r] = requant_out<FAST>(acc[pb4][r], q, b.out_zp, b.act_min, b.act_max);
        stage4(dl, N2, pb4 * 16 + 4 * g, n, v);
      }
    };
    auto epi1 = [&](int t, int n, v4i acc, int mu, int sh) {
      if (n >= N2) return;
      const ChanQ q = chan_q(mu, sh, b.out_zp);
      int32_t v[4];
#pragma unroll
      for (int r = 0; r < 4; ++r) v[r] = requant_out<FAST>(acc[r], q, b.out_zp, b.act_min, b.act_max);
      stage4(dl, N2, orow, n, v);
    };
    if constexpr (AM) {
      gemm_xs4_nt<KX>(b, pl, S2, KS2, wave, r16, g, epi4, ct.lo, ct.hi);
    } else {
      const int tc0 = ct.lo + wsub;
      if (!PFC && tc0 < ct.hi) xs_round_load<KX, TTC>(b, KS2, tc0, WPB, ct.hi, r16, g, c_first);
      gemm_xs_nt_from<KX, TTC>(b, xrow, KS2, tc0, WPB, ct.hi, r16, g, c_first, epi1);
    }
  }
  __syncthreads();
  CHAIN_STAMP(4)
  if constexpr (!SPLIT) {
    copy_out(dl, (uint8_t*)cp.pw2.output + (long)m0 * cp.pw2.out_c, rows * cp.pw2.out_c);
  } else {
    const int N2 = cp.pw2.out_c;
    const int T2 = (N2 + 15) >> 4;
    const int c_lo = (int)blockIdx.y * T2 / (int)gridDim.y * 16;
    const int c_hi = min(N2, ((int)blockIdx.y + 1) * T2 / (int)gridDim.y * 16);
    if (c_hi > c_lo)
      copy_out_slice(dl, (uint8_t*)cp.pw2.output + (long)m0 * N2, N2, c_lo, c_hi - c_lo, rows);
  }
  CHAIN_STAMP(5)
#undef CHAIN_STAMP
}

struct ChainLds {
  int S1, S2, off_pl, off_o1, off_add;
  size_t bytes;
};
static ChainLds chain_lds(const bh_chain_params& p) {
  ChainLds L;
  const int rows = p.px_blocks * 16;
  L.S1 = p.pw1.k_pad + 32;
  L.S2 = p.has_pw2 ? p.pw2.k_pad + 32 : 0;
  const int dl_row = std::max(L.S1, p.has_pw2 ? (p.pw2.out_c + 15) / 16 * 16 : 0);
  L.off_pl = rows * dl_row;
  L.off_o1 = L.off_pl + rows * L.S2;
  L.off_add = L.off_o1 + (p.pw1.output ? rows * ((p.pw1.out_c + 15) / 16 * 16) : 0);
  L.bytes = (size_t)L.off_add + (p.pw1.residual ? 512 * sizeof(int) : 0);
  return L;
}


struct PersistLds {
  int ws1, ws2, S1, S2;
  int off_w2, off_t1, off_t2, off_dwt, off_dww, off_dl, off_pl, off_o1;
  size_t bytes;
};

__host__ __device__ inline PersistLds persist_lds(const bh_chain_params& p) {
  PersistLds L;
  const int T1 = (p.pw1.out_c + 15) / 16;
  const int T2 = p.has_pw2 ? (p.pw2.out_c + 15) / 16 : 0;
  const int C = p.dw.out_c;
  L.ws1 = p.pw1.k_pad + 16;
  L.ws2 = p.has_pw2 ? p.pw2.k_pad + 16 : 0;
  L.S1 = L.ws1;
  L.S2 = L.ws2;
  size_t o = (size_t)T1 * 16 * L.ws1;
  L.off_w2 = (int)o;
  o += (size_t)T2 * 16 * L.ws2;
  L.off_t1 = (int)o;
  o += 12 * (size_t)T1 * 16;
  L.off_t2 = (int)o;
  o += 12 * (size_t)T2 * 16;
  L.off_dwt = (int)o;
  o += 12 * (size_t)C;
  L.off_dww = (int)o;
  o += (9 * (size_t)C + 15) / 16 * 16;
  const int dl_row = L.S1 > (T2 * 16) ? L.S1 : T2 * 16;
  L.off_dl = (int)o;
  o += 64 * (size_t)dl_row;
  L.off_pl = (int)o;
  o += 64 * (size_t)L.S2;
  L.off_o1 = (int)o;
  o += p.pw1.output ? 64 * (size_t)T1 * 16 : 0;
  L.bytes = o;
  return L;
}

template <bool FAST, int KX>
__global__ __launch_bounds__(256) void chain_persist_kernel(bh_chain_params cp, int P, PersistLds L, ChainDivs dv) {
  typedef unsigned int v4u __attribute__((ext_vector_type(4)));
  extern __shared__ __attribute__((aligned(16))) unsigned char smem[];
  const int tid = threadIdx.x;
  const int lane = tid & 63;
  const int wave = tid >> 6;
  const int r16 = lane & 15;
  const int g = lane >> 4;
  const bh_dwconv_params& d = cp.dw;
// ... 138 lines not shown
        v4i acc[4] = {be, be, be, be};
        for (int k = 0; k < KS1; ++k) {
          const v4i w = *(const v4i*)(wrow + k * 64);
#pragma unroll
          for (int pb = 0; pb < 4; ++pb)
            acc[pb] = __builtin_amdgcn_mfma_i32_16x16x64_i8(
                w, *(const v4i*)(dl + (pb * 16 + r16) * L.S1 + g * 16 + k * 64), acc[pb], 0, 0, 0);
        }
        if (nb >= N1) continue;
        const v4i vm = *(const v4i*)(t1 + T1 * 16 + nb);
        const v4i vs = *(const v4i*)(t1 + 2 * T1 * 16 + nb);
        ChanQ q[4];
#pragma unroll
        for (int r = 0; r < 4; ++r) q[r] = chan_q(vm[r], vs[r], a.out_zp);
        uint32_t rq[4];
#pragma unroll
        for (int pb = 0; pb < 4; ++pb) rq[pb] = res && mv[pb] ? *(const uint32_t*)(res + (long)mp[pb] * N1 + nb) : 0u;
#pragma unroll
        for (int pb = 0; pb < 4; ++pb) {
          int32_t v[4];
#pragma unroll
          for (int r = 0; r < 4; ++r) v[r] = requant_out<FAST>(acc[pb][r], q[r], a.out_zp, a.act_min, a.act_max);
          if (res) {
#pragma unroll
            for (int r = 0; r < 4; ++r) {
              const int32_t qv = sbyte(rq[pb], r);
              const int32_t sy =
                  requant_lt1((v[r] + a.add_y_off) * (1 << a.add_left_shift), a.add_y_mult, a.add_y_shift);
              const int32_t sr =
                  requant_lt1((qv + a.add_r_off) * (1 << a.add_left_shift), a.add_r_mult, a.add_r_shift);
              v[r] = clamp_i32(requant_lt1(sy + sr, a.add_o_mult, a.add_o_shift) + a.add_o_off, a.add_act_min,
                               a.add_act_max);
            }
          }
          const uint32_t pk = pack4(v);
          const int row = pb * 16 + r16;
          if (out1) *(uint32_t*)(o1 + row * N1 + nb) = pk;
          if (cp.has_pw2) *(uint32_t*)(pl + row * L.S2 + nb) = pk;
        }
      }
    }
    __syncthreads();
    if (out1) copy_out(o1, out1 + (long)m0 * N1, rows * N1);
    if (cp.has_pw2) {
      v4i x[4][KX];
#pragma unroll
      for (int pb = 0; pb < 4; ++pb)
#pragma unroll
        for (int k = 0; k < KX; ++k)
          x[pb][k] = k < KS2 ? *(const v4i*)(pl + (pb * 16 + r16) * L.S2 + g * 16 + k * 64) : (v4i){0, 0, 0, 0};
      for (int t = wave; t < T2; t += 4) {
        const unsigned char* wrow = W2 + (t * 16 + r16) * L.ws2 + g * 16;
        const int nb = t * 16 + 4 * g;
        const v4i be = *(const v4i*)(t2 + nb);
        v4i acc[4] = {be, be, be, be};
#pragma unroll
        for (int k = 0; k < KX; ++k)
          if (k < KS2) {
            const v4i w = *(const v4i*)(wrow + k * 64);
#pragma unroll
            for (int pb = 0; pb < 4; ++pb) acc[pb] = __builtin_amdgcn_mfma_i32_16x16x64_i8(w, x[pb][k], acc[pb], 0, 0, 0);
          }
        if (nb >= N2) continue;
        const v4i vm = *(const v4i*)(t2 + T2 * 16 + nb);
        const v4i vs = *(const v4i*)(t2 + 2 * T2 * 16 + nb);
        ChanQ q[4];
#pragma unroll
        for (int r = 0; r < 4; ++r) q[r] = chan_q(vm[r], vs[r], b.out_zp);
#pragma unroll
        for (int pb = 0; pb < 4; ++pb) {
          int32_t v[4];
#pragma unroll
          for (int r = 0; r < 4; ++r) v[r] = requant_out<FAST>(acc[pb][r], q[r], b.out_zp, b.act_min, b.act_max);
          *(uint32_t*)(dl + (pb * 16 + r16) * N2 + nb) = pack4(v);
        }
      }
      __syncthreads();
      copy_out(dl, (uint8_t*)b.output + (long)m0 * N2, rows * N2);
    }
    __syncthreads();
  }
}

template <int RB, bool FAST, int KX, int NW, bool AM, int DA, int VAR>
static void launch_chain_v(const bh_chain_params& p, int P, const ChainLds& L, size_t lds, hipStream_t s) {
  if (lds > 64 * 1024) {
    static thread_local int opted_device = -1;
    int dev = 0;
    (void)hipGetDevice(&dev);
    if (opted_device != dev) {
      (void)hipFuncSetAttribute((const void*)chain_kernel<RB, FAST, KX, NW, AM, DA, VAR>, hipFuncAttributeMaxDynamicSharedMemorySize,
                                160 * 1024);
      opted_device = dev;
    }
  }
  ChainDivs dv;
  dv.out_w = FastDiv(p.dw.out_w);
  dv.out_h = FastDiv(p.dw.out_h);
  const int blocks = (P + RB * 16 - 1) / (RB * 16);
  const int split = (VAR & 2) ? p.c_split : 1;
  BH_LAUNCH((chain_kernel<RB, FAST, KX, NW, AM, DA, VAR>), dim3(blocks, split), dim3(NW * 64), lds, s, p, P, L.S1,
            L.S2, L.off_pl, L.off_o1, L.off_add, dv);
}

template <int RB, bool FAST, int KX, int NW = 4, bool AM = false, int DA = 2>
static void launch_chain(const bh_chain_params& p, int P, const ChainLds& L, size_t lds, hipStream_t s) {
  if constexpr (DA == 2 && !AM && RB <= 2) {
    if (p.has_pw2 && p.c_split > 1) return launch_chain_v<RB, FAST, KX, NW, AM, DA, 2>(p, P, L, lds, s);
  }
  launch_chain_v<RB, FAST, KX, NW, AM, DA, 0>(p, P, L, lds, s);
}

template <bool FAST, int KX>
static void launch_persist(const bh_chain_params& p, int P, size_t lds, hipStream_t s) {
  static thread_local int opted_device = -1;
  int dev = 0;
  (void)hipGetDevice(&dev);
  if (opted_device != dev) {
    (void)hipFuncSetAttribute((const void*)chain_persist_kernel<FAST, KX>, hipFuncAttributeMaxDynamicSharedMemorySize,
                              160 * 1024);
    opted_device = dev;
  }
  ChainDivs dv;
  dv.out_w = FastDiv(p.dw.out_w);
  dv.out_h = FastDiv(p.dw.out_h);
  const int nblocks = (P + 63) / 64;
  static thread_local size_t cached_lds = 0;
  static thread_local int cached_per_cu = 1;
  if (cached_lds != lds) {
    int n = 0;
    if (hipOccupancyMaxActiveBlocksPerMultiprocessor(&n, chain_persist_kernel<FAST, KX>, 256, lds) != hipSuccess)
      n = 1;
    cached_per_cu = std::max(1, std::min(4, n));
    cached_lds = lds;
  }
  const int per_cu = cached_per_cu;
  const int grid = std::min(nblocks, 256 * per_cu);
  BH_LAUNCH((chain_persist_kernel<FAST, KX>), dim3(grid), dim3(256), lds, s, p, P, persist_lds(p), dv);
}

static bool conv1x1_ok(const bh_conv_params& c, int in_c) {
  return c.k_h == 1 && c.k_w == 1 && c.stride_h == 1 && c.stride_w == 1 && c.pad_h == 0 && c.pad_w == 0 &&
         c.in_c == in_c && c.k_pad == (in_c + 63) / 64 * 64 && c.n_pad >= (c.out_c + 15) / 16 * 16 &&
         c.in_xor == 0 && c.w_zp == 0 && !c.out_table && c.out_c > 0 && c.out_c % 4 == 0 && c.weights &&
         c.bias_eff && c.mult && c.shift;
}

}

extern "C" size_t bh_chain_lds_bytes(const bh_chain_params* pp) {
  if (!pp) return 0;
  const bh_chain_params& p = *pp;
  const bh_dwconv_params& d = p.dw;
  if (!p.tile && !p.stage) {
    if (p.px_blocks != 1 && p.px_blocks != 2 && p.px_blocks != 4) return 0;
    if (p.waves != 0 && p.waves != 4 && !((p.waves == 8 || p.waves == 16) && p.px_blocks == 1)) return 0;
  }
  if (d.k_h != 3 || d.k_w != 3 || d.depth_multiplier != 1 || d.in_c != d.out_c || d.out_c % 16 || !d.taps ||
      d.in_xor != 0 || d.w_zp != 0 || d.out_table || !d.input || !d.weights || !d.mult || !d.shift ||
      d.batch <= 0 || d.out_h <= 0 || d.out_w <= 0 || d.stride_h <= 0 || d.stride_w <= 0)
    return 0;
  if (!bh::conv1x1_ok(p.pw1, d.out_c)) return 0;
  const long P = (long)d.batch * d.out_h * d.out_w;
  if (p.pw1.batch * p.pw1.out_h * p.pw1.out_w != P) return 0;
  if (p.has_pw2) {
    if (!bh::conv1x1_ok(p.pw2, p.pw1.out_c) || p.pw2.residual || !p.pw2.output ||
        p.pw2.k_pad > 64 * bh::kXsMax)
      return 0;
    if ((long)p.pw2.batch * p.pw2.out_h * p.pw2.out_w != P) return 0;
  } else if (!p.pw1.output) {
    return 0;
  }
  const long widest = std::max<long>(std::max(d.out_c, p.pw1.out_c), p.has_pw2 ? p.pw2.out_c : 0);
  if (P * widest >= INT32_MAX || (long)d.batch * d.in_h * d.in_w * d.in_c >= INT32_MAX) return 0;
  if (p.dense) return bh_chain_dense_lds_bytes(pp);
  if (p.stage) return bh_chain_stage_lds_bytes(pp);
  if (p.c_split < 0 || p.c_split > 4) return 0;
  if (p.c_split > 1 && (p.tile || p.persist || p.deep || p.px_blocks > 2 || !p.has_pw2 ||
                        (p.pw2.out_c + 15) / 16 < p.c_split))
    return 0;
  if (p.tile) return bh_chain_tile_lds_bytes(pp);
  if (p.deep && (p.persist || !((p.px_blocks == 1 && (p.waves == 0 || p.waves == 4 || p.waves == 8)) ||
                                (p.px_blocks == 2 && (p.waves == 0 || p.waves == 4)))))
    return 0;
  if (p.persist) {
// ... 95 lines not shown
```

### include/band_hip_kernels.h

```cpp
#ifndef BAND_HIP_KERNELS_H_
#define BAND_HIP_KERNELS_H_

#include <stddef.h>
#include <stdint.h>

#ifdef __cplusplus
extern "C" {
#endif

#define BH_EINVAL (-1)

typedef void* bh_stream_t;
typedef void* bh_graph_exec_t;
typedef void* bh_event_t;

int bh_device_count(int* count);
int bh_set_device(int ordinal);
int bh_get_device(int* ordinal);
int bh_device_arch(int ordinal, char* buf, size_t cap);
int bh_device_pci_bus_id(int ordinal, char* buf, int cap);
int bh_stream_create(bh_stream_t* stream);
int bh_stream_destroy(bh_stream_t stream);
int bh_stream_sync(bh_stream_t stream);
int bh_stream_query(bh_stream_t stream);
int bh_malloc(void** ptr, size_t bytes);
int bh_free(void* ptr);
int bh_host_alloc(void** ptr, size_t bytes);
int bh_host_free(void* ptr);
int bh_memcpy_h2d_async(void* dst, const void* src, size_t bytes, bh_stream_t s);
int bh_memcpy_d2h_async(void* dst, const void* src, size_t bytes, bh_stream_t s);
int bh_memcpy_d2d_async(void* dst, const void* src, size_t bytes, bh_stream_t s);
int bh_copy_d2d(void* dst, const void* src, size_t bytes, bh_stream_t s);
int bh_memset_async(void* dst, int value, size_t bytes, bh_stream_t s);
int bh_memcpy_h2d(void* dst, const void* src, size_t bytes);
int bh_memcpy_d2h(void* dst, const void* src, size_t bytes);

int bh_capture_begin(bh_stream_t s);
int bh_capture_end(bh_stream_t s, bh_graph_exec_t* exec);
int bh_graph_launch(bh_graph_exec_t exec, bh_stream_t s);
int bh_capture_end_keep(bh_stream_t s, bh_graph_exec_t* exec, void** graph);
int bh_graph_free(void* graph);
int bh_graph_memcpy_nodes(void* graph, void** nodes, void** dsts, const void** srcs, size_t* bytes, int max, int* n);
int bh_graph_exec_set_memcpy(bh_graph_exec_t exec, void* node, void* dst, const void* src, size_t bytes, int h2d);
int bh_graph_destroy(bh_graph_exec_t exec);

int bh_event_create(bh_event_t* ev);
int bh_event_create_blocking(bh_event_t* ev);
int bh_event_create_untimed(bh_event_t* ev);
int bh_event_destroy(bh_event_t ev);
int bh_event_record(bh_event_t ev, bh_stream_t s);
int bh_event_sync(bh_event_t ev);
#define BH_ENOTREADY (-2)
int bh_event_query(bh_event_t ev);
int bh_event_elapsed_ms(bh_event_t start, bh_event_t end, float* ms);
int bh_spin_us(bh_stream_t s, int us);
int bh_empty_launch(bh_stream_t s);
int bh_profile_events(bh_event_t start, bh_event_t stop);


typedef struct bh_conv_params {
  int batch, in_h, in_w, in_c;
  int out_h, out_w, out_c;
  int k_h, k_w;
  int stride_h, stride_w, dil_h, dil_w;
  int pad_h, pad_w;
  int k_pad, n_pad;
  int in_xor;
  int32_t in_zp;
  int32_t w_zp;
  int32_t out_zp;
  int32_t act_min, act_max;
  const void* input;
  void* output;
  const int8_t* weights;
  const int32_t* bias_eff;
  const int32_t* mult;
  const int32_t* shift;
  const void* residual;
  int32_t add_y_off, add_r_off, add_o_off;
  int32_t add_left_shift;
  int32_t add_y_mult, add_y_shift, add_r_mult, add_r_shift, add_o_mult, add_o_shift;
  int32_t add_act_min, add_act_max;
  const void* out_table;
  int32_t requant_fast;
  int32_t kernel_hint;
  int64_t out_img_stride;
} bh_conv_params;

typedef struct bh_conv_group {
  int n, blocks, is1x1;
  const void* table;
} bh_conv_group;
int bh_conv_group_ok(const bh_conv_params* p);
size_t bh_conv_group_table_bytes(int n);
int bh_conv_group_plan(const bh_conv_params* members, int n, void* host_table, bh_conv_group* g);
int bh_conv_group_i8(const bh_conv_group* g, bh_stream_t stream);
#define BH_CONV_AUTO 0
#define BH_CONV_MFMA 1
#define BH_CONV_GEMM 2
#define BH_CONV_GEMM_BIG 3
#define BH_CONV_STEM_VALU 4
#define BH_CONV_STEM_MFMA 5
#define BH_CONV_STEM_SCALAR 6
#define BH_CONV_ROWS 7
int bh_conv_gemm_big_config(long M, int N);

typedef struct bh_conv_grouped_params {
  bh_conv_params conv;
  int32_t groups;
} bh_conv_grouped_params;
#define BH_CONV_GROUPED_AUTO 0
#define BH_CONV_GROUPED_MFMA 1
#define BH_CONV_GROUPED_MFMA_2 2

typedef struct bh_dwconv_params {
  int batch, in_h, in_w, in_c;
  int out_h, out_w, out_c, depth_multiplier;
  int k_h, k_w;
  int stride_h, stride_w, dil_h, dil_w;
  int pad_h, pad_w;
  int in_xor;
  int32_t in_zp, w_zp, out_zp;
  int32_t act_min, act_max;
  const void* input;
  void* output;
  const int8_t* weights;
  const int32_t* bias;
  const int32_t* mult;
  const int32_t* shift;
  const void* out_table;
  const int32_t* taps;
  int32_t requant_fast;
  int32_t kernel_hint;
} bh_dwconv_params;
#define BH_DW_AUTO 0
#define BH_DW_RUN 1
#define BH_DW_DOT 2
#define BH_DW_MFMA 3

typedef struct bh_fc_params {
  int rows, depth, depth_pad, units;
  int in_xor;
  int32_t in_zp, w_zp, out_zp;
  int32_t act_min, act_max;
  const void* input;
  void* output;
  const int8_t* weights;
  const int32_t* bias_eff;
  const int32_t* mult;
  const int32_t* shift;
  const void* out_table;
} bh_fc_params;

#define BH_ELT_ADD 0
#define BH_ELT_MUL 1
#define BH_ELT_SQDIFF 2
typedef struct bh_eltwise_params {
  int kind;
  int in_signed;
  int shape_a[4], shape_b[4], shape_o[4];
  int32_t a_off, b_off, o_off;
  int32_t left_shift;
  int32_t a_mult, a_shift;
  int32_t b_mult, b_shift;
  int32_t o_mult, o_shift;
  int32_t act_min, act_max;
  const void* a;
  const void* b;
  void* out;
} bh_eltwise_params;

#define BH_POOL_AVG 0
#define BH_POOL_MAX 1
typedef struct bh_pool_params {
  int kind;
  int in_signed;
  int batch, in_h, in_w, channels;
  int out_h, out_w;
  int f_h, f_w, stride_h, stride_w, pad_h, pad_w;
  int32_t act_min, act_max;
  const void* input;
  void* output;
} bh_pool_params;

typedef struct bh_irb_params {
  int batch, in_h, in_w, in_c;
  int exp_c;
  int out_h, out_w, out_c;
  int stride, pad_h, pad_w;
  int has_expand;
  int tile_h, tile_w;
  const int8_t* exp_w; int exp_k_pad;
  const int32_t* exp_bias_eff; const int32_t* exp_mult; const int32_t* exp_shift;
  int32_t x_zp;
  int32_t e_zp, e_act_min, e_act_max;
  const int8_t* dw_w;
  const int32_t* dw_bias; const int32_t* dw_mult; const int32_t* dw_shift;
  int32_t d_zp, d_act_min, d_act_max;
  const int8_t* proj_w; int proj_k_pad;
  const int32_t* proj_bias_eff; const int32_t* proj_mult; const int32_t* proj_shift;
  int32_t p_zp, p_act_min, p_act_max;
  int has_residual;
  int32_t add_p_off, add_x_off, add_o_off, add_left_shift;
  int32_t add_p_mult, add_p_shift, add_x_mult, add_x_shift, add_o_mult, add_o_shift;
  int32_t add_act_min, add_act_max;
  const void* input;
  void* output;
  void* debug_stamps;
  int32_t requant_fast;
} bh_irb_params;

size_t bh_irb_lds_bytes(const bh_irb_params* p);
int bh_irb_i8(const bh_irb_params* p, bh_stream_t s);

typedef struct bh_chain_params {
  bh_dwconv_params dw;
  bh_conv_params pw1;
  bh_conv_params pw2;
  int has_pw2;
  int px_blocks;
  int waves;
  int persist;
  int tile;
  const void* tile_blob;
  void* debug_stamps;
  int deep;
  int c_split;
  int stage;
  int dense;
} bh_chain_params;

size_t bh_chain_lds_bytes(const bh_chain_params* p);
size_t bh_chain_stage_lds_bytes(const bh_chain_params* p);
int bh_chain_stage_launch(const bh_chain_params* p, bh_stream_t s);
size_t bh_chain_dense_lds_bytes(const bh_chain_params* p);
int bh_chain_dense_launch(const bh_chain_params* p, bh_stream_t s);
size_t bh_chain_tile_lds_bytes(const bh_chain_params* p);
int bh_chain_tile_launch(const bh_chain_params* p, bh_stream_t s);
size_t bh_chain_tile_blob_bytes(const bh_chain_params* p);
int bh_chain_tile_pack(const bh_chain_params* p, void* blob, bh_stream_t s);
int bh_chain_i8(const bh_chain_params* p, bh_stream_t s);

typedef struct bh_mean_params {
  long outer, reduce, inner;
  int type;
  int32_t multiplier, shift, bias;
  const void* input;
  void* output;
} bh_mean_params;
int bh_mean(const bh_mean_params* p, bh_stream_t s);

typedef struct bh_mean_rows_params {
  long rows;
  int depth;
  int type;
  int exact;
  float scale, bias;
  int32_t out_zp;
  const void* input;
  void* output;
} bh_mean_rows_params;
int bh_mean_rows(const bh_mean_rows_params* p, bh_stream_t s);
const char* bh_mean_rows_kernel(const bh_mean_rows_params* p);
int bh_mean_rows_check(const bh_mean_rows_params* p);

#define BH_LAYERNORM_MAX_DEPTH 1024
typedef struct bh_layernorm_params {
  long rows;
  int depth;
  bh_mean_rows_params mean_x, mean_d;
  bh_eltwise_params sqdiff, add_eps, mul_gamma, mul_x, mul_m, sub_beta, add_out;
  int32_t eps_q;
  const void* rsqrt_table;
  const void* input;
  const void* gamma;
  const void* beta;
  void* output;
} bh_layernorm_params;
int bh_layernorm_i8(const bh_layernorm_params* p, bh_stream_t s);
const char* bh_layernorm_i8_kernel(const bh_layernorm_params* p);
int bh_layernorm_i8_check(const bh_layernorm_params* p);


int bh_pack_conv_weights(const void* w, int w_signed, int out_c, int k,
                         int k_pad, int n_pad, const int32_t* bias,
                         int32_t in_zp, int32_t w_zp, int8_t* packed,
                         int32_t* bias_eff);

int bh_conv_packed_geometry(int out_c, int k, int* k_pad, int* n_pad);
int bh_pack_dw_taps(const int8_t* w, int c, const int32_t* bias, int32_t in_zp, int32_t w_zp, int32_t* taps);
int bh_conv_requant_fast_ok(const int32_t* mult, const int32_t* shift, int n, int k, int64_t max_abs_bias);

int bh_conv2d_i8(const bh_conv_params* p, bh_stream_t s);
const char* bh_conv2d_i8_kernel(const bh_conv_params* p);
int bh_conv2d_grouped_i8(const bh_conv_grouped_params* p, bh_stream_t s);
const char* bh_conv2d_grouped_i8_kernel(const bh_conv_grouped_params* p);
int bh_dwconv2d_i8(const bh_dwconv_params* p, bh_stream_t s);
const char* bh_dwconv2d_i8_kernel(const bh_dwconv_params* p);
int bh_fc_i8(const bh_fc_params* p, bh_stream_t s);
int bh_eltwise_i8(const bh_eltwise_params* p, bh_stream_t s);
int bh_pool_i8(const bh_pool_params* p, bh_stream_t s);


int bh_lut_u8(const void* in, void* out, long n, const void* table, bh_stream_t s);
int bh_lut_f32(const void* in, void* out, long n, const float* table, bh_stream_t s);
int bh_quantize_f32(const float* in, void* out, long n, float scale, int32_t zp, int out_signed,
                    bh_stream_t s);

typedef struct {
  int batch, in_h, in_w, in_c, out_h, out_w, out_c, k_h, k_w;
  int stride_h, stride_w, dil_h, dil_w, pad_h, pad_w;
  int depthwise, depth_multiplier;
  float act_min, act_max;
  const float* input;
  float* output;
  const float* weights;
  const float* bias;
} bh_conv_f32_params;
int bh_conv2d_f32(const bh_conv_f32_params* p, bh_stream_t s);
int bh_conv2d_f32_split(const bh_conv_f32_params* p);

typedef struct {
  int rows, depth, units;
  float act_min, act_max;
  const float* input;
  float* output;
  const float* weights;
  const float* bias;
} bh_fc_f32_params;
int bh_fc_f32(const bh_fc_f32_params* p, bh_stream_t s);

#define BH_ELTF_ADD 0
#define BH_ELTF_SUB 1
#define BH_ELTF_MUL 2
#define BH_ELTF_SQDIFF 3
typedef struct {
  int kind;
  int shape_a[4], shape_b[4], shape_o[4];
  float act_min, act_max;
  const float* a;
  const float* b;
  float* out;
} bh_eltwise_f32_params;
int bh_eltwise_f32(const bh_eltwise_f32_params* p, bh_stream_t s);

typedef struct {
  int kind;
  int batch, in_h, in_w, channels, out_h, out_w, f_h, f_w, stride_h, stride_w, pad_h, pad_w;
  float act_min, act_max;
  const float* input;
  float* output;
} bh_pool_f32_params;
int bh_pool_f32(const bh_pool_f32_params* p, bh_stream_t s);

#define BH_UNARY_CLAMP 0
#define BH_UNARY_LOGISTIC 1
#define BH_UNARY_RSQRT 2
#define BH_UNARY_GELU 3
#define BH_UNARY_GELU_TANH 4
int bh_unary_f32(int kind, const float* in, float* out, long n, float lo, float hi, bh_stream_t s);

int bh_softmax_f32(const float* in, float* out, long rows, int depth, float beta, bh_stream_t s);

#define BH_CONCAT_MAX_INPUTS 16
typedef struct {
  int n_inputs;
  long outer;
  long row[BH_CONCAT_MAX_INPUTS];
  const void* input[BH_CONCAT_MAX_INPUTS];
  const void* table[BH_CONCAT_MAX_INPUTS];
  void* output;
} bh_concat_params;
int bh_concat(const bh_concat_params* p, bh_stream_t s);

// ... 146 lines not shown
```

Measured before the change: 124,900.

## Pack per-channel requant records and depthwise tap fragments for chain kernels

Result: slower. 120,800 (-3.3%).

```diff
diff --git a/band_amd/_abi.py b/band_amd/_abi.py
--- a/band_amd/_abi.py
+++ b/band_amd/_abi.py
@@ -18,7 +18,8 @@
                                "add_y_shift", "add_r_mult", "add_r_shift", "add_o_mult", "add_o_shift",
                                "add_act_min", "add_act_max")] + [("out_table", c_void_p), ("requant_fast", c_int32),
                                                                   ("kernel_hint", c_int32),
-                                                                  ("out_img_stride", ctypes.c_int64)]
+                                                                  ("out_img_stride", ctypes.c_int64),
+                                                                  ("rq", c_void_p)]
 
 
 class ConvGroupedParams(ctypes.Structure):
@@ -35,7 +36,7 @@
         "k_h", "k_w", "stride_h", "stride_w", "dil_h", "dil_w", "pad_h", "pad_w", "in_xor")] + [
         (n, c_int32) for n in ("in_zp", "w_zp", "out_zp", "act_min", "act_max")] + [
         (n, c_void_p) for n in ("input", "output", "weights", "bias", "mult", "shift", "out_table", "taps")] + [
-        ("requant_fast", c_int32), ("kernel_hint", c_int32)]
+        ("requant_fast", c_int32), ("kernel_hint", c_int32), ("rq", c_void_p), ("frags", c_void_p)]
 
 
 class FcParams(ctypes.Structure):
@@ -257,6 +258,9 @@
     "bh_conv_packed_geometry": (c_int, [c_int, c_int, ctypes.POINTER(c_int), ctypes.POINTER(c_int)]),
     "bh_pack_dw_taps": (c_int, [c_void_p, c_int, c_void_p, c_int32, c_int32, c_void_p]),
     "bh_conv_requant_fast_ok": (c_int, [c_void_p, c_void_p, c_int, c_int, ctypes.c_int64]),
+    "bh_rq_records_bytes": (c_size_t, [c_int]),
+    "bh_pack_rq_records": (c_int, [c_void_p, c_void_p, c_void_p, c_int, c_int32, c_void_p]),
+    "bh_pack_dw_frags": (c_int, [c_void_p, c_int, c_void_p]),
     "bh_conv2d_i8": (c_int, [ctypes.POINTER(ConvParams), c_void_p]),
     "bh_conv_group_ok": (c_int, [ctypes.POINTER(ConvParams)]),
     "bh_conv_group_table_bytes": (ctypes.c_size_t, [c_int]),
diff --git a/band_amd/csrc/backend/hip/lower.cc b/band_amd/csrc/backend/hip/lower.cc
--- a/band_amd/csrc/backend/hip/lower.cc
+++ b/band_amd/csrc/backend/hip/lower.cc
@@ -120,8 +120,11 @@
   int kp = 0, np = 0;
   bh_conv_packed_geometry(oc, K, &kp, &np);
   const size_t wbytes = static_cast<size_t>(kp) * np;
+  const bool fast = bh_conv_requant_fast_ok(q.mult.data(), q.shift.data(), oc, K, MaxAbs(q.bias, oc)) != 0;
+  const size_t rq_off = (wbytes + 12ull * oc + 15) / 16 * 16;
+  const size_t rq_bytes = fast ? bh_rq_records_bytes(oc) : 0;
   std::shared_ptr<DeviceBlob> blob;
-  RETURN_STATUS_IF(ConstBlob(ckey, wbytes + 12ull * oc, sg, [&](uint8_t* host) {
+  RETURN_STATUS_IF(ConstBlob(ckey, rq_bytes ? rq_off + rq_bytes : wbytes + 12ull * oc, sg, [&](uint8_t* host) {
     std::vector<uint8_t> flipped(flip ? static_cast<size_t>(oc) * K : 0);
     for (size_t i = 0; i < flipped.size(); ++i) {
       const size_t ci = i % icg, fx = i / icg % kw, fy = i / icg / kw % kh, co = i / K;
@@ -133,6 +136,9 @@
       return absl::InternalError("weight packing failed");
     std::copy(q.mult.begin(), q.mult.end(), tables + oc);
     std::copy(q.shift.begin(), q.shift.end(), tables + 2 * oc);
+    if (rq_bytes && bh_pack_rq_records(tables, q.mult.data(), q.shift.data(), oc, Zp(out),
+                                       reinterpret_cast<int32_t*>(host + rq_off)) != 0)
+      return absl::InternalError("requantisation record packing failed");
     return absl::OkStatus();
   }, &blob));
   const int32_t* tab = reinterpret_cast<const int32_t*>(static_cast<char*>(blob->ptr()) + wbytes);
@@ -144,7 +150,8 @@
   p.input = in_ptr; p.output = out_ptr;
   p.weights = static_cast<const int8_t*>(blob->ptr());
   p.bias_eff = tab; p.mult = tab + oc; p.shift = tab + 2 * oc;
-  p.requant_fast = bh_conv_requant_fast_ok(q.mult.data(), q.shift.data(), oc, K, MaxAbs(q.bias, oc));
+  p.requant_fast = fast ? 1 : 0;
+  if (rq_bytes && !blob->host()) p.rq = reinterpret_cast<const int32_t*>(static_cast<char*>(blob->ptr()) + rq_off);
   const double M = static_cast<double>(g.batch) * g.out_h * g.out_w;
   L->alg_ops = 2.0 * M * oc * K;
   L->alg_bytes = static_cast<double>(g.batch) * g.in_h * g.in_w * g.in_c + M * oc + static_cast<double>(oc) * K +
@@ -810,8 +817,13 @@
   const size_t tbytes = 12ull * oc;
   const bool dot = kh == 3 && kw == 3 && g.depth_multiplier == 1 && oc % 4 == 0;
   const size_t pbytes = dot ? 16ull * oc : 0;
+  const bool fast = bh_conv_requant_fast_ok(q.mult.data(), q.shift.data(), oc, kh * kw, MaxAbs(q.bias, oc)) != 0;
+  const bool chain = dot && oc % 16 == 0;
+  const size_t fr_off = (wpad + tbytes + pbytes + 15) / 16 * 16;
+  const size_t fr_bytes = chain ? 64ull * oc : 0;
+  const size_t rq_bytes = chain && fast ? bh_rq_records_bytes(oc) : 0;
   std::shared_ptr<DeviceBlob> blob;
-  RETURN_STATUS_IF(ConstBlob(ckey, wpad + tbytes + pbytes, sg, [&](uint8_t* host) {
+  RETURN_STATUS_IF(ConstBlob(ckey, chain ? fr_off + fr_bytes + rq_bytes : wpad + tbytes + pbytes, sg, [&](uint8_t* host) {
     for (size_t i = 0; i < wbytes; ++i) host[i] = i8 ? w.data[i] : static_cast<uint8_t>(w.data[i] ^ 0x80);
     int32_t* tables = reinterpret_cast<int32_t*>(host + wpad);
     for (int c = 0; c < oc; ++c) tables[c] = q.bias ? q.bias[c] : 0;
@@ -819,6 +831,17 @@
     std::copy(q.shift.begin(), q.shift.end(), tables + 2 * oc);
     if (dot && bh_pack_dw_taps(reinterpret_cast<const int8_t*>(host), oc, tables, q.in_zp, q.w_zp, tables + 3 * oc) != 0)
       return absl::InternalError("depthwise tap packing failed");
+    if (chain) {
+      const int32_t* taps = tables + 3 * oc;
+      int32_t* frags = reinterpret_cast<int32_t*>(host + fr_off);
+      if (bh_pack_dw_frags(taps, oc, frags) != 0) return absl::InternalError("depthwise fragment packing failed");
+      if (rq_bytes) {
+        std::vector<int32_t> folded(oc);
+        for (int c = 0; c < oc; ++c) folded[c] = taps[4 * c + 3];
+        if (bh_pack_rq_records(folded.data(), q.mult.data(), q.shift.data(), oc, Zp(out), frags + 16 * oc) != 0)
+          return absl::InternalError("requantisation record packing failed");
+      }
+    }
     return absl::OkStatus();
   }, &blob));
   const int32_t* tab = reinterpret_cast<const int32_t*>(static_cast<char*>(blob->ptr()) + wpad);
@@ -831,7 +854,11 @@
   p.weights = static_cast<const int8_t*>(blob->ptr());
   p.bias = tab; p.mult = tab + oc; p.shift = tab + 2 * oc;
   if (dot && !blob->host()) p.taps = tab + 3 * oc;
-  p.requant_fast = bh_conv_requant_fast_ok(q.mult.data(), q.shift.data(), oc, kh * kw, MaxAbs(q.bias, oc));
+  p.requant_fast = fast ? 1 : 0;
+  if (chain && !blob->host()) {
+    p.frags = reinterpret_cast<const int32_t*>(static_cast<char*>(blob->ptr()) + fr_off);
+    if (rq_bytes) p.rq = p.frags + 16 * oc;
+  }
   L->kind = Launch::kDwConv;
   L->kernel = bh_dwconv2d_i8_kernel(&p);
   const double M = static_cast<double>(g.batch) * g.out_h * g.out_w;
diff --git a/band_amd/csrc/backend/hip/requant_records.cc b/band_amd/csrc/backend/hip/requant_records.cc
--- /dev/null
+++ b/band_amd/csrc/backend/hip/requant_records.cc
@@ -0,0 +1,17 @@
+#include "requant_records.h"
+
+#include "band_hip_kernels.h"
+
+extern "C" size_t bh_rq_records_bytes(int n) { return n > 0 ? band::hip::RqRecordCount(n) * 16 : 0; }
+
+extern "C" int bh_pack_rq_records(const int32_t* bias, const int32_t* mult, const int32_t* shift, int n,
+                                  int32_t out_zp, int32_t* rec) {
+  if (!mult || !shift || !rec || n <= 0) return BH_EINVAL;
+  return band::hip::PackRqRecords(bias, mult, shift, n, out_zp, rec) ? 0 : BH_EINVAL;
+}
+
+extern "C" int bh_pack_dw_frags(const int32_t* taps, int c, int32_t* frags) {
+  if (!taps || !frags || c <= 0 || c % 4) return BH_EINVAL;
+  band::hip::PackDwFrags(taps, c, frags);
+  return 0;
+}
diff --git a/band_amd/csrc/backend/hip/requant_records.h b/band_amd/csrc/backend/hip/requant_records.h
--- /dev/null
+++ b/band_amd/csrc/backend/hip/requant_records.h
@@ -0,0 +1,70 @@
+#pragma once
+
+#include <cstddef>
+#include <cstdint>
+
+namespace band {
+namespace hip {
+
+constexpr int kRqMaxE = 22;
+
+inline size_t RqRecordCount(int n) { return static_cast<size_t>((n + 15) / 16) * 16; }
+
+inline int64_t RqConstant(int e, int32_t out_zp) {
+  return (int64_t{1} << 30) + (e > 0 ? (int64_t{1} << (30 + e)) : 0) + static_cast<int64_t>(out_zp) * (int64_t{1} << (31 + e));
+}
+
+inline bool RqChannelOk(int32_t mult, int32_t shift, int32_t out_zp) {
+  return mult > (1 << 30) && shift <= 0 && shift >= -kRqMaxE && out_zp >= -255 && out_zp <= 255;
+}
+
+inline void RqRecord(int32_t bias, int32_t mult, int32_t shift, int32_t out_zp, int32_t rec[4]) {
+  const int e = -shift;
+  const int64_t c = RqConstant(e, out_zp);
+  rec[0] = bias;
+  rec[1] = mult;
+  rec[2] = static_cast<int32_t>(c >> 32);
+  rec[3] = static_cast<int32_t>((static_cast<uint32_t>(c) & 0xC0000000u) | (e > 0 ? 1u << 29 : 0u) | static_cast<uint32_t>(e));
+}
+
+inline int32_t RqApply(int32_t acc, const int32_t rec[4], int32_t lo, int32_t hi) {
+  const uint32_t w = static_cast<uint32_t>(rec[3]);
+  const int e = static_cast<int>(w & 31u);
+  const int32_t emask = (w >> 29) & 1u ? -1 : 0;
+  const int64_t c = static_cast<int64_t>((static_cast<uint64_t>(static_cast<uint32_t>(rec[2])) << 32) | (w & 0xC0000000u));
+  const int64_t z = static_cast<int64_t>(acc) * rec[1] + c;
+  const int32_t u = static_cast<int32_t>(z >> 31);
+  const int32_t v = (u + ((acc >> 31) & emask)) >> e;
+  return v < lo ? lo : (v > hi ? hi : v);
+}
+
+inline bool PackRqRecords(const int32_t* bias, const int32_t* mult, const int32_t* shift, int n, int32_t out_zp,
+                          int32_t* rec) {
+  for (int c = 0; c < n; ++c)
+    if (!RqChannelOk(mult[c], shift[c], out_zp)) return false;
+  const size_t total = RqRecordCount(n);
+  for (size_t c = 0; c < total; ++c) {
+    int32_t* r = rec + 4 * c;
+    if (c < static_cast<size_t>(n)) RqRecord(bias ? bias[c] : 0, mult[c], shift[c], out_zp, r);
+    else r[0] = r[1] = r[2] = r[3] = 0;
+  }
+  return true;
+}
+
+inline void PackDwFrags(const int32_t* taps, int channels, int32_t* frags) {
+  for (int c = 0; c < channels; ++c) {
+    const uint32_t* t = reinterpret_cast<const uint32_t*>(taps) + 4 * static_cast<size_t>(c);
+    const int bsh = 8 * (c & 3);
+    uint32_t tap[9];
+    for (int k = 0; k < 8; ++k) tap[k] = (t[k / 4] >> (8 * (k % 4))) & 0xffu;
+    tap[8] = (t[2] >> bsh) & 0xffu;
+    for (int g = 0; g < 4; ++g) {
+      int32_t* o = frags + (static_cast<size_t>(c) * 4 + g) * 4;
+      for (int s = 0; s < 3; ++s) o[s] = g < 3 ? static_cast<int32_t>(tap[3 * s + g] << bsh) : 0;
+      o[3] = static_cast<int32_t>(t[3]);
+    }
+  }
+}
+
+}
+}
diff --git a/band_amd/csrc/kernels/chain_dense.hip b/band_amd/csrc/kernels/chain_dense.hip
--- a/band_amd/csrc/kernels/chain_dense.hip
+++ b/band_amd/csrc/kernels/chain_dense.hip
@@ -37,12 +37,15 @@
 }
 
 struct DenseConv {
-  __amdgpu_buffer_rsrc_t w, be, mu, sh;
+  __amdgpu_buffer_rsrc_t w, be, mu, sh, rq;
   int wv, cv;
   int tile_w;
 };
+template <bool REC>
 __device__ __forceinline__ DenseConv dense_conv(const bh_conv_params& c, int r16, int g) {
   DenseConv d;
+  if constexpr (REC)
+    d.rq = __builtin_amdgcn_make_buffer_rsrc((void*)c.rq, (short)0, (c.out_c + 15) / 16 * 256, 0x00020000);
   d.w = __builtin_amdgcn_make_buffer_rsrc((void*)c.weights, (short)0, c.n_pad * c.k_pad, 0x00020000);
   d.be = __builtin_amdgcn_make_buffer_rsrc((void*)c.bias_eff, (short)0, c.out_c * 4, 0x00020000);
   d.mu = __builtin_amdgcn_make_buffer_rsrc((void*)c.mult, (short)0, c.out_c * 4, 0x00020000);
@@ -55,7 +58,8 @@
 template <int KX>
 struct DenseTile {
   v4i w[KX];
-  int be, mu, sh;
+  int be;
+  ChanRq rq;
 };
 template <int KX>
 __device__ __forceinline__ void dense_filter_load(const DenseConv& c, int t, int k0, int KS, v4i (&w)[KX]) {
@@ -70,15 +74,22 @@
     }
   }
 }
-template <int KX>
+template <int KX, bool REC>
 __device__ __forceinline__ void dense_tile_load(const DenseConv& c, int t, int k0, int KS, DenseTile<KX>& d) {
   dense_filter_load<KX>(c, t, k0, KS, d.w);
-  d.be = (int)__builtin_amdgcn_raw_buffer_load_b32(c.be, c.cv, t * 64, 0);
-  d.mu = (int)__builtin_amdgcn_raw_buffer_load_b32(c.mu, c.cv, t * 64, 0);
-  d.sh = (int)__builtin_amdgcn_raw_buffer_load_b32(c.sh, c.cv, t * 64, 0);
-}
-
-template <bool FAST, bool INTERIOR>
+  if constexpr (REC) {
+    typedef unsigned int v4u __attribute__((ext_vector_type(4)));
+    const v4u v = __builtin_amdgcn_raw_buffer_load_b128(c.rq, c.cv * 4, t * 256, 0);
+    d.be = (int)v.x;
+    d.rq = {(int)v.y, (int)v.z, (int)v.w};
+  } else {
+    d.be = (int)__builtin_amdgcn_raw_buffer_load_b32(c.be, c.cv, t * 64, 0);
+    d.rq = {(int)__builtin_amdgcn_raw_buffer_load_b32(c.mu, c.cv, t * 64, 0),
+            (int)__builtin_amdgcn_raw_buffer_load_b32(c.sh, c.cv, t * 64, 0), 0};
+  }
+}
+
+template <bool FAST, bool INTERIOR, bool REC, bool FR>
 __device__ __forceinline__ void dense_dw_groups(const bh_dwconv_params& d, const __amdgpu_buffer_rsrc_t rsrc,
                                                 const int (&off)[3], const bool (&ok)[3], bool need, int src4, int r16,
                                                 int g, unsigned char* dl, int S1) {
@@ -86,8 +97,6 @@
   const int zfill = (int)splat_byte(d.in_zp);
   const int dsel = r16 >> 2;
   const int bsh = 8 * (r16 & 3);
-  const int tsel1 = g == 0 ? 0 : 1, tbit1 = g == 0 ? 24 : 8 * (g - 1);
-  const int tbit2 = g < 2 ? 8 * (2 + g) : bsh;
   const int G = d.out_c >> 4;
   for (int cg = 0; cg < G; ++cg) {
     const int c0 = cg * 16;
@@ -99,8 +108,8 @@
       for (int s = 0; s < 3; ++s) v[s] = __builtin_amdgcn_raw_buffer_load_b128(rsrc, off[s] + c0, 0, 0);
     }
     const int c = c0 + r16;
-    const v4i tw = *(const v4i*)(d.taps + 4 * c);
-    const int32_t mu = d.mult[c], sh = d.shift[c];
+    const v4i tw = dw_row_load<FR>(d, c, g);
+    const ChanRq rq = dw_rq_load<REC>(d, c);
     v4i xf[3];
 #pragma unroll
     for (int s = 0; s < 3; ++s) {
@@ -110,19 +119,16 @@
 #pragma unroll
       for (int j = 0; j < 4; ++j) xf[s][j] = __builtin_amdgcn_ds_bpermute(src4, xf[s][j]);
     }
-    const uint32_t t0 = (uint32_t)tw.x, t1 = (uint32_t)tw.y, t2 = (uint32_t)tw.z;
-    uint32_t wb[3];
-    wb[0] = (t0 >> (8 * g)) & 0xffu;
-    wb[1] = ((tsel1 ? t1 : t0) >> tbit1) & 0xffu;
-    wb[2] = ((g < 2 ? t1 : t2) >> tbit2) & 0xffu;
+    int wb[3];
+    dw_lane_bytes<FR>(tw, g, bsh, wb);
     v4i acc = (v4i){tw.w, tw.w, tw.w, tw.w};
 #pragma unroll
     for (int s = 0; s < 3; ++s) {
-      const int w = g < 3 ? (int)(wb[s] << bsh) : 0;
+      const int w = wb[s];
       const v4i wf = (v4i){dsel == 0 ? w : 0, dsel == 1 ? w : 0, dsel == 2 ? w : 0, dsel == 3 ? w : 0};
       acc = __builtin_amdgcn_mfma_i32_16x16x64_i8(xf[s], wf, acc, 0, 0, 0);
     }
-    const ChanQ q = chan_q(mu, sh, d.out_zp);
+    const ChanQ q = chan_q_of<REC>(rq, d.out_zp);
     int32_t o[4];
 #pragma unroll
     for (int r = 0; r < 4; ++r) o[r] = requant_out<FAST>(acc[r], q, d.out_zp, d.act_min, d.act_max);
@@ -130,7 +136,7 @@
   }
 }
 
-template <bool FAST>
+template <bool FAST, bool REC, bool FR>
 __device__ __forceinline__ void dense_dw(const bh_dwconv_params& d, const ChainDivs& dv, int m, bool mval, int lane,
                                          int r16, int g, unsigned char* dl, int S1) {
   const int C = d.out_c;
@@ -156,8 +162,8 @@
   const __amdgpu_buffer_rsrc_t rsrc =
       __builtin_amdgcn_make_buffer_rsrc((void*)d.input, (short)0, d.batch * d.in_h * d.in_w * C, 0x00020000);
   const bool interior = __builtin_amdgcn_ballot_w64(g < 3 && !(ok[0] && ok[1] && ok[2])) == 0;
-  if (interior) dense_dw_groups<FAST, true>(d, rsrc, off, ok, need, src4, r16, g, dl, S1);
-  else dense_dw_groups<FAST, false>(d, rsrc, off, ok, need, src4, r16, g, dl, S1);
+  if (interior) dense_dw_groups<FAST, true, REC, FR>(d, rsrc, off, ok, need, src4, r16, g, dl, S1);
+  else dense_dw_groups<FAST, false, REC, FR>(d, rsrc, off, ok, need, src4, r16, g, dl, S1);
 }
 
 __device__ __forceinline__ void dense_wave_sync() {
@@ -166,8 +172,14 @@
   __builtin_amdgcn_fence(__ATOMIC_ACQUIRE, "wavefront");
 }
 
-template <bool FAST, int KX, int WPE>
+#ifndef BH_TAB_DENSE
+#define BH_TAB_DENSE 3
+#endif
+template <bool FAST, int KX, int WPE, bool TAB = false>
 __global__ __launch_bounds__(256, WPE) void chain_dense_kernel(bh_chain_params cp, int P, DenseLds L, ChainDivs dv) {
+  static_assert(FAST || !TAB, "the records hold the single-step form's constants");
+  constexpr bool REC = TAB && (BH_TAB_DENSE & 1) != 0;
+  constexpr bool FR = TAB && (BH_TAB_DENSE & 2) != 0;
   extern __shared__ __attribute__((aligned(16))) unsigned char smem[];
   const int lane = threadIdx.x & 63;
   const int pb = threadIdx.x >> 6;
@@ -191,7 +203,7 @@
   const int rows = min(16, P - mw);
   const int orow = 4 * g;
 
-  dense_dw<FAST>(cp.dw, dv, mw + r16, mw + r16 < P, lane, r16, g, dl, L.S1);
+  dense_dw<FAST, REC, FR>(cp.dw, dv, mw + r16, mw + r16 < P, lane, r16, g, dl, L.S1);
   dense_wave_sync();
 
   {
@@ -201,12 +213,12 @@
     const int KS1 = a.k_pad >> 6;
     const unsigned char* xrow = dl + r16 * L.S1 + g * 16;
     const uint8_t* res = (const uint8_t*)a.residual;
-    const DenseConv ac = dense_conv(a, r16, g);
+    const DenseConv ac = dense_conv<REC>(a, r16, g);
     for (int t = 0; t < T1; ++t) {
       DenseTile<2> cur;
-      dense_tile_load<2>(ac, t, 0, KS1, cur);
+      dense_tile_load<2, REC>(ac, t, 0, KS1, cur);
       v4i acc = (v4i){cur.be, cur.be, cur.be, cur.be};
-      const int mu = cur.mu, sh = cur.sh;
+      const ChanRq crq = cur.rq;
       for (int k = 0;;) {
         acc = __builtin_amdgcn_mfma_i32_16x16x64_i8(*(const v4i*)(xrow + k * 64), cur.w[0], acc, 0, 0, 0);
         if (k + 1 < KS1)
@@ -217,7 +229,7 @@
       }
       const int n = t * 16 + r16;
       if (n < N1) {
-        const ChanQ q = chan_q(mu, sh, a.out_zp);
+        const ChanQ q = chan_q_of<REC>(crq, a.out_zp);
         int32_t v[4];
 #pragma unroll
         for (int r = 0; r < 4; ++r) v[r] = requant_out<FAST>(acc[r], q, a.out_zp, a.act_min, a.act_max);
@@ -251,19 +263,19 @@
 #pragma unroll
     for (int k = 0; k < KX; ++k) x[k] = k < KS2 ? *(const v4i*)(pl + r16 * L.S2 + g * 16 + k * 64) : (v4i){0, 0, 0, 0};
     constexpr bool PF = KX <= 2;
-    const DenseConv bc = dense_conv(b, r16, g);
+    const DenseConv bc = dense_conv<REC>(b, r16, g);
     DenseTile<KX> cur, nxt;
-    if (PF) dense_tile_load<KX>(bc, 0, 0, KS2, cur);
+    if (PF) dense_tile_load<KX, REC>(bc, 0, 0, KS2, cur);
     for (int t = 0; t < T2; ++t) {
-      if (!PF) dense_tile_load<KX>(bc, t, 0, KS2, cur);
-      else if (t + 1 < T2) dense_tile_load<KX>(bc, t + 1, 0, KS2, nxt);
+      if (!PF) dense_tile_load<KX, REC>(bc, t, 0, KS2, cur);
+      else if (t + 1 < T2) dense_tile_load<KX, REC>(bc, t + 1, 0, KS2, nxt);
       v4i acc = (v4i){cur.be, cur.be, cur.be, cur.be};
 #pragma unroll
       for (int k = 0; k < KX; ++k)
         if (k < KS2) acc = __builtin_amdgcn_mfma_i32_16x16x64_i8(x[k], cur.w[k], acc, 0, 0, 0);
       const int n = t * 16 + r16;
       if (n < N2) {
-        const ChanQ q = chan_q(cur.mu, cur.sh, b.out_zp);
+        const ChanQ q = chan_q_of<REC>(cur.rq, b.out_zp);
         int32_t v[4];
 #pragma unroll
         for (int r = 0; r < 4; ++r) v[r] = requant_out<FAST>(acc[r], q, b.out_zp, b.act_min, b.act_max);
@@ -285,7 +297,13 @@
   ChainDivs dv;
   dv.out_w = FastDiv(p.dw.out_w);
   dv.out_h = FastDiv(p.dw.out_h);
-  BH_LAUNCH((chain_dense_kernel<FAST, KX, WPE>), dim3((P + 63) / 64), dim3(256), L.bytes, s, p, P, L, dv);
+  if constexpr (FAST && BH_TAB_DENSE != 0) {
+    if (chain_has_tables(p)) {
+      BH_LAUNCH((chain_dense_kernel<FAST, KX, WPE, true>), dim3((P + 63) / 64), dim3(256), L.bytes, s, p, P, L, dv);
+      return;
+    }
+  }
+  BH_LAUNCH((chain_dense_kernel<FAST, KX, WPE, false>), dim3((P + 63) / 64), dim3(256), L.bytes, s, p, P, L, dv);
 }
 
 }
diff --git a/band_amd/csrc/kernels/chain_dw.hpp b/band_amd/csrc/kernels/chain_dw.hpp
--- a/band_amd/csrc/kernels/chain_dw.hpp
+++ b/band_amd/csrc/kernels/chain_dw.hpp
@@ -8,7 +8,44 @@
   FastDiv out_w, out_h;
 };
 
-template <bool FAST, int DA, int WPB>
+inline bool chain_has_tables(const bh_chain_params& p) {
+  return p.dw.rq && p.dw.frags && p.pw1.rq && (!p.has_pw2 || p.pw2.rq);
+}
+
+template <bool FR>
+__device__ __forceinline__ v4i dw_row_load(const bh_dwconv_params& d, int c, int g) {
+  if constexpr (FR) return *(const v4i*)(d.frags + 16 * c + 4 * g);
+  else return *(const v4i*)(d.taps + 4 * c);
+}
+template <bool REC>
+__device__ __forceinline__ ChanRq dw_rq_load(const bh_dwconv_params& d, int c) {
+  if constexpr (REC) {
+    const v4i v = *(const v4i*)(d.rq + 4 * c);
+    return {v.y, v.z, v.w};
+  } else {
+    return {d.mult[c], d.shift[c], 0};
+  }
+}
+template <bool FR>
+__device__ __forceinline__ void dw_lane_bytes(const v4i& tw, int g, int bsh, int (&w)[3]) {
+  if constexpr (FR) {
+    w[0] = tw.x;
+    w[1] = tw.y;
+    w[2] = tw.z;
+    return;
+  }
+  const int tsel1 = g == 0 ? 0 : 1, tbit1 = g == 0 ? 24 : 8 * (g - 1);
+  const int tbit2 = g < 2 ? 8 * (2 + g) : bsh;
+  const uint32_t t0 = (uint32_t)tw.x, t1 = (uint32_t)tw.y, t2 = (uint32_t)tw.z;
+  uint32_t wb[3];
+  wb[0] = (t0 >> (8 * g)) & 0xffu;
+  wb[1] = ((tsel1 ? t1 : t0) >> tbit1) & 0xffu;
+  wb[2] = ((g < 2 ? t1 : t2) >> tbit2) & 0xffu;
+#pragma unroll
+  for (int s = 0; s < 3; ++s) w[s] = g < 3 ? (int)(wb[s] << bsh) : 0;
+}
+
+template <bool FAST, int DA, int WPB, bool REC = false, bool FR = false>
 __device__ __forceinline__ void chain_dw_mfma(const bh_dwconv_params& d, const ChainDivs& dv, int m, bool mval,
                                               int lane, int r16, int g, int wsub, unsigned char* dl, int S1,
                                               int orow) {
@@ -38,12 +75,11 @@
   const int zfill = (int)splat_byte(d.in_zp);
   const int dsel = r16 >> 2;
   const int bsh = 8 * (r16 & 3);
-  const int tsel1 = g == 0 ? 0 : 1, tbit1 = g == 0 ? 24 : 8 * (g - 1);
-  const int tbit2 = g < 2 ? 8 * (2 + g) : bsh;
+  static_assert(FAST || !REC, "the records hold the single-step form's constants");
   struct DwItem {
     v4i xf[3];
     v4i tw;
-    int32_t mu, sh;
+    ChanRq rq;
   };
   auto dw_load = [&](int cg, DwItem& it) {
     const int c0 = cg * 16;
@@ -57,28 +93,24 @@
       it.xf[s] = (v4i){ok[s] ? (int)v[s].x : zfill, ok[s] ? (int)v[s].y : zfill, ok[s] ? (int)v[s].z : zfill,
                        ok[s] ? (int)v[s].w : zfill};
     const int c = c0 + r16;
-    it.tw = *(const v4i*)(d.taps + 4 * c);
-    it.mu = d.mult[c];
-    it.sh = d.shift[c];
+    it.tw = dw_row_load<FR>(d, c, g);
+    it.rq = dw_rq_load<REC>(d, c);
   };
   auto dw_finish = [&](int cg, DwItem& it) {
 #pragma unroll
     for (int s = 0; s < 3; ++s)
 #pragma unroll
       for (int j = 0; j < 4; ++j) it.xf[s][j] = __builtin_amdgcn_ds_bpermute(src4, it.xf[s][j]);
-    const uint32_t t0 = (uint32_t)it.tw.x, t1 = (uint32_t)it.tw.y, t2 = (uint32_t)it.tw.z;
-    uint32_t wb[3];
-    wb[0] = (t0 >> (8 * g)) & 0xffu;
-    wb[1] = ((tsel1 ? t1 : t0) >> tbit1) & 0xffu;
-    wb[2] = ((g < 2 ? t1 : t2) >> tbit2) & 0xffu;
+    int wb[3];
+    dw_lane_bytes<FR>(it.tw, g, bsh, wb);
     v4i acc = (v4i){it.tw.w, it.tw.w, it.tw.w, it.tw.w};
 #pragma unroll
     for (int s = 0; s < 3; ++s) {
-      const int w = g < 3 ? (int)(wb[s] << bsh) : 0;
+      const int w = wb[s];
       const v4i wf = (v4i){dsel == 0 ? w : 0, dsel == 1 ? w : 0, dsel == 2 ? w : 0, dsel == 3 ? w : 0};
       acc = __builtin_amdgcn_mfma_i32_16x16x64_i8(it.xf[s], wf, acc, 0, 0, 0);
     }
-    const ChanQ q = chan_q(it.mu, it.sh, d.out_zp);
+    const ChanQ q = chan_q_of<REC>(it.rq, d.out_zp);
     int32_t v[4];
 #pragma unroll
     for (int r = 0; r < 4; ++r) v[r] = requant_out<FAST>(acc[r], q, d.out_zp, d.act_min, d.act_max);
@@ -95,7 +127,7 @@
   }
 }
 
-template <bool FAST, int NB, int NW>
+template <bool FAST, int NB, int NW, bool REC = false, bool FR = false>
 __device__ __forceinline__ void chain_dw_mfma_wg(const bh_dwconv_params& d, const ChainDivs& dv, int m0, int P,
                                                  int lane, int r16, int g, int wave, unsigned char* dl, int S1) {
   typedef unsigned int v4u __attribute__((ext_vector_type(4)));
@@ -129,8 +161,7 @@
   const int zfill = (int)splat_byte(d.in_zp);
   const int dsel = r16 >> 2;
   const int bsh = 8 * (r16 & 3);
-  const int tsel1 = g == 0 ? 0 : 1, tbit1 = g == 0 ? 24 : 8 * (g - 1);
-  const int tbit2 = g < 2 ? 8 * (2 + g) : bsh;
+  static_assert(FAST || !REC, "the records hold the single-step form's constants");
   const int G = C >> 4;
   for (int cg = wave; cg < G; cg += NW) {
     const int c0 = cg * 16;
@@ -148,20 +179,17 @@
         xf[b][s] = (v4i){ok[b][s] ? (int)v[s].x : zfill, ok[b][s] ? (int)v[s].y : zfill,
                          ok[b][s] ? (int)v[s].z : zfill, ok[b][s] ? (int)v[s].w : zfill};
     }
-    const v4i tw = *(const v4i*)(d.taps + 4 * c);
-    const int32_t mu = d.mult[c], sh = d.shift[c];
-    const uint32_t t0 = (uint32_t)tw.x, t1 = (uint32_t)tw.y, t2 = (uint32_t)tw.z;
-    uint32_t wb[3];
-    wb[0] = (t0 >> (8 * g)) & 0xffu;
-    wb[1] = ((tsel1 ? t1 : t0) >> tbit1) & 0xffu;
-    wb[2] = ((g < 2 ? t1 : t2) >> tbit2) & 0xffu;
+    const v4i tw = dw_row_load<FR>(d, c, g);
+    const ChanRq rq = dw_rq_load<REC>(d, c);
+    int wb[3];
+    dw_lane_bytes<FR>(tw, g, bsh, wb);
     v4i wf[3];
 #pragma unroll
     for (int s = 0; s < 3; ++s) {
-      const int w = g < 3 ? (int)(wb[s] << bsh) : 0;
+      const int w = wb[s];
       wf[s] = (v4i){dsel == 0 ? w : 0, dsel == 1 ? w : 0, dsel == 2 ? w : 0, dsel == 3 ? w : 0};
     }
-    const ChanQ q = chan_q(mu, sh, d.out_zp);
+    const ChanQ q = chan_q_of<REC>(rq, d.out_zp);
 #pragma unroll
     for (int b = 0; b < NB; ++b) {
 #pragma unroll
diff --git a/band_amd/csrc/kernels/chain_stage.hip b/band_amd/csrc/kernels/chain_stage.hip
--- a/band_amd/csrc/kernels/chain_stage.hip
+++ b/band_amd/csrc/kernels/chain_stage.hip
@@ -81,7 +81,15 @@
   }
 }
 
-template <int RB, bool FAST, int KX, int NW, int LW>
+template <int LW>
+constexpr int stage_tab_parts() {
+#ifdef BH_TAB_STAGE
+  return BH_TAB_STAGE;
+#else
+  return LW == 0 ? 2 : 0;
+#endif
+}
+template <int RB, bool FAST, int KX, int NW, int LW, bool TAB = false>
 __global__ __launch_bounds__(NW * 64) void chain_stage_kernel(bh_chain_params cp, int P, StageGeom G, ChainDivs dv) {
   extern __shared__ __attribute__((aligned(16))) unsigned char smem[];
   constexpr int WPB = NW / RB;
@@ -141,7 +149,11 @@
     }
   }
 
-  if (LW == 0 || wave < NA) chain_dw_mfma<FAST, 2, NA / RB>(cp.dw, dv, m, m < P, lane, r16, g, wsub, dl, G.S1, orow);
+  static_assert(FAST || !TAB, "the records hold the single-step form's constants");
+  constexpr int PARTS = TAB ? stage_tab_parts<LW>() : 0;
+  constexpr bool REC = (PARTS & 1) != 0;
+  constexpr bool FR = (PARTS & 2) != 0;
+  if (LW == 0 || wave < NA) chain_dw_mfma<FAST, 2, NA / RB, REC, FR>(cp.dw, dv, m, m < P, lane, r16, g, wsub, dl, G.S1, orow);
   asm volatile("s_waitcnt vmcnt(0)" ::: "memory");
   __syncthreads();
 
@@ -238,14 +250,14 @@
     stage_copy_out(ol, G.out_pitch, (uint8_t*)b.output + (long)m0 * N2, N2, c_lo, c_hi - c_lo, rows, tid, NW * 64);
 }
 
-template <int RB, bool FAST, int KX, int NW, int LW>
-static void launch_stage(const bh_chain_params& p, int P, const StageGeom& G, hipStream_t s) {
+template <int RB, bool FAST, int KX, int NW, int LW, bool TAB>
+static void launch_stage_t(const bh_chain_params& p, int P, const StageGeom& G, hipStream_t s) {
   if (G.bytes > 64 * 1024) {
     static thread_local int opted_device = -1;
     int dev = 0;
     (void)hipGetDevice(&dev);
     if (opted_device != dev) {
-      (void)hipFuncSetAttribute((const void*)chain_stage_kernel<RB, FAST, KX, NW, LW>,
+      (void)hipFuncSetAttribute((const void*)chain_stage_kernel<RB, FAST, KX, NW, LW, TAB>,
                                 hipFuncAttributeMaxDynamicSharedMemorySize, 160 * 1024);
       opted_device = dev;
     }
@@ -254,8 +266,16 @@
   dv.out_w = FastDiv(p.dw.out_w);
   dv.out_h = FastDiv(p.dw.out_h);
   const int blocks = (P + RB * 16 - 1) / (RB * 16);
-  BH_LAUNCH((chain_stage_kernel<RB, FAST, KX, NW, LW>), dim3(blocks, std::max(1, p.c_split)), dim3(NW * 64), G.bytes, s,
+  BH_LAUNCH((chain_stage_kernel<RB, FAST, KX, NW, LW, TAB>), dim3(blocks, std::max(1, p.c_split)), dim3(NW * 64), G.bytes, s,
             p, P, G, dv);
+}
+
+template <int RB, bool FAST, int KX, int NW, int LW>
+static void launch_stage(const bh_chain_params& p, int P, const StageGeom& G, hipStream_t s) {
+  if constexpr (FAST && stage_tab_parts<LW>() != 0) {
+    if (p.dw.rq && p.dw.frags) return launch_stage_t<RB, FAST, KX, NW, LW, true>(p, P, G, s);
+  }
+  launch_stage_t<RB, FAST, KX, NW, LW, false>(p, P, G, s);
 }
 
 template <bool FAST, int KX>
diff --git a/band_amd/csrc/kernels/common.hpp b/band_amd/csrc/kernels/common.hpp
--- a/band_amd/csrc/kernels/common.hpp
+++ b/band_amd/csrc/kernels/common.hpp
@@ -115,6 +115,38 @@
   q.zpe = (int32_t)((uint32_t)zp << (q.e & 31));
   q.c0 = (1ll << 30) + (q.e > 0 ? (1ll << (30 + q.e)) : 0ll);
   return q;
+}
+
+__device__ __forceinline__ ChanQ chan_q_rec(int32_t mu, int32_t chi, int32_t w) {
+  ChanQ q;
+  q.mu = mu;
+  q.sh = 0;
+  q.e = w & 31;
+  q.emask = (int32_t)((uint32_t)w << 2) >> 31;
+  q.zpe = 0;
+  q.c0 = (int64_t)(((uint64_t)(uint32_t)chi << 32) | ((uint32_t)w & 0xC0000000u));
+  return q;
+}
+
+struct ChanRq {
+  int32_t mu, a, b;
+};
+template <bool REC>
+__device__ __forceinline__ ChanQ chan_q_of(const ChanRq& r, int32_t zp) {
+  if constexpr (REC) return chan_q_rec(r.mu, r.a, r.b);
+  else return chan_q(r.mu, r.a, zp);
+}
+template <bool REC>
+__device__ __forceinline__ void conv_chan_load(const bh_conv_params& c, int n, int& be, ChanRq& r) {
+  if constexpr (REC) {
+    const v4i v = *(const v4i*)(c.rq + 4 * n);
+    be = v.x;
+    r = {v.y, v.z, v.w};
+  } else {
+    const int nl = n < c.out_c ? n : 0;
+    be = c.bias_eff[nl];
+    r = {c.mult[nl], c.shift[nl], 0};
+  }
 }
 
 __device__ __forceinline__ int32_t med3_clamp(int32_t v, int32_t lo, int32_t hi) {
diff --git a/band_amd/csrc/kernels/fused_chain.hip b/band_amd/csrc/kernels/fused_chain.hip
--- a/band_amd/csrc/kernels/fused_chain.hip
+++ b/band_amd/csrc/kernels/fused_chain.hip
@@ -124,20 +124,17 @@
 template <int KB>
 struct TileHead {
   v4i w[KB];
-  int be, mu, sh;
+  int be;
+  ChanRq rq;
 };
-template <int KB>
+template <int KB, bool REC>
 __device__ __forceinline__ void tile_head_load(const bh_conv_params& c, int t, int KS, int r16, int g,
                                                TileHead<KB>& h) {
   const int8_t* wrow = c.weights + (long)(t * 16 + r16) * c.k_pad + g * 16;
 #pragma unroll
   for (int u = 0; u < KB; ++u)
     if (u < KS) h.w[u] = *(const v4i*)(wrow + u * 64);
-  const int n = t * 16 + r16;
-  const int nl = n < c.out_c ? n : 0;
-  h.be = c.bias_eff[nl];
-  h.mu = c.mult[nl];
-  h.sh = c.shift[nl];
+  conv_chan_load<REC>(c, t * 16 + r16, h.be, h.rq);
 }
 template <int KB = 4>
 __device__ __forceinline__ v4i gemm_tile_nt(const bh_conv_params& c, const unsigned char* xrow, int t, int KS,
@@ -170,10 +167,11 @@
 
 template <int KMAX, int TT>
 struct XsRound {
-  int tt[TT], be[TT], mu[TT], sh[TT];
+  int tt[TT], be[TT];
+  ChanRq rq[TT];
   v4i w[TT][KMAX];
 };
-template <int KMAX, int TT>
+template <int KMAX, int TT, bool REC>
 __device__ __forceinline__ void xs_round_load(const bh_conv_params& c, int KS, int t, int tstep, int T, int r16,
                                               int g, XsRound<KMAX, TT>& rd) {
 #pragma unroll
@@ -183,21 +181,17 @@
 #pragma unroll
     for (int k = 0; k < KMAX; ++k)
       if (k < KS) rd.w[u][k] = *(const v4i*)(r + k * 64);
-    const int n = rd.tt[u] * 16 + r16;
-    const int l = n < c.out_c ? n : 0;
-    rd.be[u] = c.bias_eff[l];
-    rd.mu[u] = c.mult[l];
-    rd.sh[u] = c.shift[l];
-  }
-}
-template <int KMAX, int TT, typename Epi>
+    conv_chan_load<REC>(c, rd.tt[u] * 16 + r16, rd.be[u], rd.rq[u]);
+  }
+}
+template <int KMAX, int TT, bool REC, typename Epi>
 __device__ __forceinline__ void gemm_xs_nt_from(const bh_conv_params& c, const unsigned char* xrow, int KS, int t0,
                                                 int tstep, int T, int r16, int g, XsRound<KMAX, TT>& rd, Epi&& epi) {
   v4i x[KMAX];
 #pragma unroll
   for (int k = 0; k < KMAX; ++k) x[k] = k < KS ? *(const v4i*)(xrow + k * 64) : (v4i){0, 0, 0, 0};
   for (int t = t0; t < T; t += TT * tstep) {
-    if (t != t0) xs_round_load<KMAX, TT>(c, KS, t, tstep, T, r16, g, rd);
+    if (t != t0) xs_round_load<KMAX, TT, REC>(c, KS, t, tstep, T, r16, g, rd);
     v4i acc[TT];
 #pragma unroll
     for (int u = 0; u < TT; ++u) acc[u] = (v4i){rd.be[u], rd.be[u], rd.be[u], rd.be[u]};
@@ -210,19 +204,19 @@
       }
 #pragma unroll
     for (int u = 0; u < TT; ++u)
-      if (u == 0 || rd.tt[u] != t) epi(rd.tt[u], rd.tt[u] * 16 + r16, acc[u], rd.mu[u], rd.sh[u]);
-  }
-}
-template <int KMAX, int TT = 2, typename Epi>
+      if (u == 0 || rd.tt[u] != t) epi(rd.tt[u], rd.tt[u] * 16 + r16, acc[u], rd.rq[u]);
+  }
+}
+template <int KMAX, int TT, bool REC, typename Epi>
 __device__ __forceinline__ void gemm_xs_nt(const bh_conv_params& c, const unsigned char* xrow, int KS, int t0,
                                            int tstep, int r16, int g, Epi&& epi) {
   const int T = (c.out_c + 15) >> 4;
   XsRound<KMAX, TT> rd;
-  if (t0 < T) xs_round_load<KMAX, TT>(c, KS, t0, tstep, T, r16, g, rd);
-  gemm_xs_nt_from<KMAX, TT>(c, xrow, KS, t0, tstep, T, r16, g, rd, epi);
-}
-
-template <int KMAX, typename Epi>
+  if (t0 < T) xs_round_load<KMAX, TT, REC>(c, KS, t0, tstep, T, r16, g, rd);
+  gemm_xs_nt_from<KMAX, TT, REC>(c, xrow, KS, t0, tstep, T, r16, g, rd, epi);
+}
+
+template <int KMAX, bool REC, typename Epi>
 __device__ __forceinline__ void gemm_xs4_nt(const bh_conv_params& c, const unsigned char* base, int stride, int KS,
                                             int wave, int r16, int g, Epi&& epi, int t_begin = 0, int t_end = -1) {
   v4i x[4][KMAX];
@@ -234,13 +228,14 @@
   const int T = t_end >= 0 ? t_end : (c.out_c + 15) >> 4;
   for (int t = t_begin + wave; t < T; t += 4) {
     const int n = t * 16 + r16;
-    const int nl = n < c.out_c ? n : 0;
     const int8_t* wrow = c.weights + (long)(t * 16 + r16) * c.k_pad + g * 16;
     v4i w[KMAX];
 #pragma unroll
     for (int k = 0; k < KMAX; ++k)
       if (k < KS) w[k] = *(const v4i*)(wrow + k * 64);
-    const int be = c.bias_eff[nl], mu = c.mult[nl], sh = c.shift[nl];
+    int be;
+    ChanRq rq;
+    conv_chan_load<REC>(c, n, be, rq);
     v4i acc[4];
 #pragma unroll
     for (int pb = 0; pb < 4; ++pb) acc[pb] = (v4i){be, be, be, be};
@@ -250,11 +245,20 @@
 #pragma unroll
         for (int pb = 0; pb < 4; ++pb) acc[pb] = __builtin_amdgcn_mfma_i32_16x16x64_i8(x[pb][k], w[k], acc[pb], 0, 0, 0);
       }
-    epi(n, acc, mu, sh);
-  }
-}
-
-template <int RB, bool FAST, int KX, int NW, bool AM, int DA = 2, int VAR = 0>
+    epi(n, acc, rq);
+  }
+}
+
+template <int RB, int NW, bool AM, int DA, int VAR>
+constexpr int chain_tab_parts() {
+#ifdef BH_TAB_RASTER
+  return BH_TAB_RASTER;
+#else
+  if (NW != 4 || DA != 2 || (VAR & 2) != 0) return 0;
+  return AM ? 2 : 3;
+#endif
+}
+template <int RB, bool FAST, int KX, int NW, bool AM, int DA = 2, int VAR = 0, bool TAB = false>
 __global__ __launch_bounds__(NW * 64) void chain_kernel(bh_chain_params cp, int P, int S1, int S2, int off_pl, int off_o1,
                                                        int off_add, ChainDivs dv) {
   extern __shared__ __attribute__((aligned(16))) unsigned char smem[];
@@ -293,19 +297,23 @@
   if (stamps && threadIdx.x == 0) stamps[7] = t_entry;
 
   constexpr bool SPLIT = (VAR & 2) != 0;
+  static_assert(FAST || !TAB, "the records hold the single-step form's constants");
+  constexpr int PARTS = TAB ? chain_tab_parts<RB, NW, AM, DA, VAR>() : 0;
+  constexpr bool REC = (PARTS & 1) != 0;
+  constexpr bool FR = (PARTS & 2) != 0;
   constexpr bool PFC = RB == 1 && DA == 2;
   constexpr bool PFB = PFC && NW == 16;
   constexpr int KBB = DA > 2 ? 8 : 4;
   TileHead<KBB> b_head;
   if constexpr (PFB) {
     const int KS1 = cp.pw1.k_pad >> 6;
-    if (KS1 > KX && wsub < (cp.pw1.out_c + 15) >> 4) tile_head_load<KBB>(cp.pw1, wsub, KS1, r16, g, b_head);
+    if (KS1 > KX && wsub < (cp.pw1.out_c + 15) >> 4) tile_head_load<KBB, REC>(cp.pw1, wsub, KS1, r16, g, b_head);
   }
 
   if constexpr (RB == 2 && DA == 2) {
-    chain_dw_mfma_wg<FAST, RB, NW>(cp.dw, dv, m0, P, lane, r16, g, wave, dl, S1);
+    chain_dw_mfma_wg<FAST, RB, NW, REC, FR>(cp.dw, dv, m0, P, lane, r16, g, wave, dl, S1);
   } else {
-    chain_dw_mfma<FAST, DA, WPB>(cp.dw, dv, m, m < P, lane, r16, g, wsub, dl, S1, orow);
+    chain_dw_mfma<FAST, DA, WPB, REC, FR>(cp.dw, dv, m, m < P, lane, r16, g, wsub, dl, S1, orow);
   }
   __syncthreads();
   CHAIN_STAMP(1)
@@ -318,9 +326,9 @@
     const unsigned char* xrow = dl + prow * S1 + g * 16;
     const uint8_t* res = (const uint8_t*)a.residual;
     const bool out1 = a.output != nullptr && (!SPLIT || blockIdx.y == 0);
-    auto epi = [&](int t, int n, v4i acc, int mu, int sh) {
+    auto epi = [&](int t, int n, v4i acc, const ChanRq& rq1) {
       if (n >= N1) return;
-      const ChanQ q = chan_q(mu, sh, a.out_zp);
+      const ChanQ q = chan_q_of<REC>(rq1, a.out_zp);
       int32_t v[4];
 #pragma unroll
       for (int r = 0; r < 4; ++r) v[r] = requant_out<FAST>(acc[r], q, a.out_zp, a.act_min, a.act_max);
@@ -343,9 +351,9 @@
       if (cp.has_pw2) stage4(pl, S2, orow, n, v);
     };
     if (AM && KS1 <= KX) {
-      gemm_xs4_nt<KX>(a, dl, S1, KS1, wave, r16, g, [&](int n, const v4i* acc, int mu, int sh) {
+      gemm_xs4_nt<KX, REC>(a, dl, S1, KS1, wave, r16, g, [&](int n, const v4i* acc, const ChanRq& rq1) {
         if (n >= N1) return;
-        const ChanQ q = chan_q(mu, sh, a.out_zp);
+        const ChanQ q = chan_q_of<REC>(rq1, a.out_zp);
 #pragma unroll
         for (int pb4 = 0; pb4 < 4; ++pb4) {
           const int rb = pb4 * 16 + 4 * g;
@@ -367,12 +375,12 @@
         }
       });
     } else if (KS1 <= KX) {
-      gemm_xs_nt<KX, TTC>(a, xrow, KS1, wsub, WPB, r16, g, epi);
+      gemm_xs_nt<KX, TTC, REC>(a, xrow, KS1, wsub, WPB, r16, g, epi);
     } else {
       for (int t = wsub; t < T1; t += WPB) {
-        if (!PFB || t != wsub) tile_head_load<KBB>(a, t, KS1, r16, g, b_head);
+        if (!PFB || t != wsub) tile_head_load<KBB, REC>(a, t, KS1, r16, g, b_head);
         const v4i acc = gemm_tile_nt<KBB>(a, xrow, t, KS1, r16, g, b_head);
-        epi(t, t * 16 + r16, acc, b_head.mu, b_head.sh);
+        epi(t, t * 16 + r16, acc, b_head.rq);
       }
     }
   }
@@ -391,7 +399,7 @@
     if (cp.has_pw2) {
       const CTiles ct = c_tiles();
       if (ct.lo + wsub < ct.hi)
-        xs_round_load<KX, TTC>(cp.pw2, cp.pw2.k_pad >> 6, ct.lo + wsub, WPB, ct.hi, r16, g, c_first);
+        xs_round_load<KX, TTC, REC>(cp.pw2, cp.pw2.k_pad >> 6, ct.lo + wsub, WPB, ct.hi, r16, g, c_first);
     }
   }
   __syncthreads();
@@ -407,9 +415,9 @@
     const int KS2 = b.k_pad >> 6;
     const CTiles ct = c_tiles();
     const unsigned char* xrow = pl + prow * S2 + g * 16;
-    auto epi4 = [&](int n, const v4i* acc, int mu, int sh) {
+    auto epi4 = [&](int n, const v4i* acc, const ChanRq& rq2) {
       if (n >= N2) return;
-      const ChanQ q = chan_q(mu, sh, b.out_zp);
+      const ChanQ q = chan_q_of<REC>(rq2, b.out_zp);
 #pragma unroll
       for (int pb4 = 0; pb4 < 4; ++pb4) {
         int32_t v[4];
@@ -418,20 +426,20 @@
         stage4(dl, N2, pb4 * 16 + 4 * g, n, v);
       }
     };
-    auto epi1 = [&](int t, int n, v4i acc, int mu, int sh) {
+    auto epi1 = [&](int t, int n, v4i acc, const ChanRq& rq2) {
       if (n >= N2) return;
-      const ChanQ q = chan_q(mu, sh, b.out_zp);
+      const ChanQ q = chan_q_of<REC>(rq2, b.out_zp);
       int32_t v[4];
 #pragma unroll
       for (int r = 0; r < 4; ++r) v[r] = requant_out<FAST>(acc[r], q, b.out_zp, b.act_min, b.act_max);
       stage4(dl, N2, orow, n, v);
     };
     if constexpr (AM) {
-      gemm_xs4_nt<KX>(b, pl, S2, KS2, wave, r16, g, epi4, ct.lo, ct.hi);
+      gemm_xs4_nt<KX, REC>(b, pl, S2, KS2, wave, r16, g, epi4, ct.lo, ct.hi);
     } else {
       const int tc0 = ct.lo + wsub;
-      if (!PFC && tc0 < ct.hi) xs_round_load<KX, TTC>(b, KS2, tc0, WPB, ct.hi, r16, g, c_first);
-      gemm_xs_nt_from<KX, TTC>(b, xrow, KS2, tc0, WPB, ct.hi, r16, g, c_first, epi1);
+      if (!PFC && tc0 < ct.hi) xs_round_load<KX, TTC, REC>(b, KS2, tc0, WPB, ct.hi, r16, g, c_first);
+      gemm_xs_nt_from<KX, TTC, REC>(b, xrow, KS2, tc0, WPB, ct.hi, r16, g, c_first, epi1);
     }
   }
   __syncthreads();
@@ -736,14 +744,14 @@
   }
 }
 
-template <int RB, bool FAST, int KX, int NW, bool AM, int DA, int VAR>
-static void launch_chain_v(const bh_chain_params& p, int P, const ChainLds& L, size_t lds, hipStream_t s) {
+template <int RB, bool FAST, int KX, int NW, bool AM, int DA, int VAR, bool TAB>
+static void launch_chain_t(const bh_chain_params& p, int P, const ChainLds& L, size_t lds, hipStream_t s) {
   if (lds > 64 * 1024) {
     static thread_local int opted_device = -1;
     int dev = 0;
     (void)hipGetDevice(&dev);
     if (opted_device != dev) {
-      (void)hipFuncSetAttribute((const void*)chain_kernel<RB, FAST, KX, NW, AM, DA, VAR>, hipFuncAttributeMaxDynamicSharedMemorySize,
+      (void)hipFuncSetAttribute((const void*)chain_kernel<RB, FAST, KX, NW, AM, DA, VAR, TAB>, hipFuncAttributeMaxDynamicSharedMemorySize,
                                 160 * 1024);
       opted_device = dev;
     }
@@ -753,8 +761,16 @@
   dv.out_h = FastDiv(p.dw.out_h);
   const int blocks = (P + RB * 16 - 1) / (RB * 16);
   const int split = (VAR & 2) ? p.c_split : 1;
-  BH_LAUNCH((chain_kernel<RB, FAST, KX, NW, AM, DA, VAR>), dim3(blocks, split), dim3(NW * 64), lds, s, p, P, L.S1,
+  BH_LAUNCH((chain_kernel<RB, FAST, KX, NW, AM, DA, VAR, TAB>), dim3(blocks, split), dim3(NW * 64), lds, s, p, P, L.S1,
             L.S2, L.off_pl, L.off_o1, L.off_add, dv);
+}
+
+template <int RB, bool FAST, int KX, int NW, bool AM, int DA, int VAR>
+static void launch_chain_v(const bh_chain_params& p, int P, const ChainLds& L, size_t lds, hipStream_t s) {
+  if constexpr (FAST && chain_tab_parts<RB, NW, AM, DA, VAR>() != 0) {
+    if (chain_has_tables(p)) return launch_chain_t<RB, FAST, KX, NW, AM, DA, VAR, true>(p, P, L, lds, s);
+  }
+  launch_chain_t<RB, FAST, KX, NW, AM, DA, VAR, false>(p, P, L, lds, s);
 }
 
 template <int RB, bool FAST, int KX, int NW = 4, bool AM = false, int DA = 2>
diff --git a/include/band_hip_kernels.h b/include/band_hip_kernels.h
--- a/include/band_hip_kernels.h
+++ b/include/band_hip_kernels.h
@@ -85,6 +85,7 @@
   int32_t requant_fast;
   int32_t kernel_hint;
   int64_t out_img_stride;
+  const int32_t* rq;
 } bh_conv_params;
 
 typedef struct bh_conv_group {
@@ -132,6 +133,8 @@
   const int32_t* taps;
   int32_t requant_fast;
   int32_t kernel_hint;
+  const int32_t* rq;
+  const int32_t* frags;
 } bh_dwconv_params;
 #define BH_DW_AUTO 0
 #define BH_DW_RUN 1
@@ -290,6 +293,10 @@
 int bh_conv_packed_geometry(int out_c, int k, int* k_pad, int* n_pad);
 int bh_pack_dw_taps(const int8_t* w, int c, const int32_t* bias, int32_t in_zp, int32_t w_zp, int32_t* taps);
 int bh_conv_requant_fast_ok(const int32_t* mult, const int32_t* shift, int n, int k, int64_t max_abs_bias);
+size_t bh_rq_records_bytes(int n);
+int bh_pack_rq_records(const int32_t* bias, const int32_t* mult, const int32_t* shift, int n, int32_t out_zp,
+                       int32_t* rec);
+int bh_pack_dw_frags(const int32_t* taps, int c, int32_t* frags);
 
 int bh_conv2d_i8(const bh_conv_params* p, bh_stream_t s);
 const char* bh_conv2d_i8_kernel(const bh_conv_params* p);
```
